# tensorlink-lab/tensorlink

Hardware: NVIDIA H100
Metric: generate tokens/sec (higher is better)
Workload: dtype bf16

## Files before the change

### include/tensorlink_b200.h

```cpp
#ifndef TENSORLINK_B200_H
#define TENSORLINK_B200_H

#include <stddef.h>
#include <stdint.h>

#ifdef __cplusplus
extern "C" {
#endif

#define TL_ABI_VERSION 1

typedef enum {
    TL_OK = 0,
    TL_ERR_INVALID = -1,
    TL_ERR_CUDA = -2,
    TL_ERR_NO_DEVICE = -3,
    TL_ERR_WORKSPACE = -4
} tl_status;

#define TL_EPI_BIAS 1
#define TL_EPI_RESIDUAL 2
#define TL_EPI_SWIGLU 4
#define TL_EPI_OUT_F32 8
#define TL_EPI_ACCUM 16
#define TL_A_MN_MAJOR 32
#define TL_B_MN_MAJOR 64

int tl_abi_version(void);
const char* tl_last_error(void);
int tl_device_info(int* sm_count, int* cc_major, int* cc_minor);

int tl_rmsnorm_fwd(const void* x, const void* w, void* y, float* rstd_out, int rows, int H, float eps, void* stream);

int tl_embed_fwd(const int64_t* ids, const void* table, void* out, int n_tokens, int H, int vocab, void* stream);

int tl_gemm_bf16(const void* A, const void* B, void* C, int M, int N, int K, int lda, int ldb, int ldc,
                 const void* bias, const void* residual, int flags, void* stream);

size_t tl_gemm_splitk_ws(int M, int N);
int tl_gemm_bf16_ws(const void* A, const void* B, void* C, int M, int N, int K, int lda, int ldb, int ldc,
                    const void* bias, const void* residual, int flags, void* workspace, size_t ws_bytes, void* stream);
int tl_gemm_bf16_ws_norm(const void* A, const void* B, void* C, int M, int N, int K, int lda, int ldb, int ldc,
                         const void* bias, const void* residual, int flags, void* workspace, size_t ws_bytes,
                         const void* norm_w, float eps, void* H_out, void* stream);

int tl_gemv_bf16(const void* x, const void* W, void* y, int M, int N, int K, const void* bias,
                 const void* residual, const void* norm_w, float eps, int flags, void* stream);
int tl_gemv_bf16_pf(const void* x, const void* W, void* y, int M, int N, int K, const void* bias,
                    const void* residual, const void* norm_w, float eps, int flags, const void* next_W,
                    size_t next_bytes, void* stream);

int tl_rope_table(const float* inv_freq, void* cos_tab, void* sin_tab, int max_pos, int half_dim, void* stream);

int tl_rope_kv_fwd(const void* qkv, void* q_out, void* k_cache, void* v_cache, const int32_t* pos0_dev,
                   const void* cos_tab, const void* sin_tab, const void* q_norm_w, const void* k_norm_w,
                   float eps, int n_tokens, int S, int n_h, int n_kv, int d, int T_max, void* stream);

int tl_attn_prefill_fwd(const void* q, const void* k_cache, const void* v_cache, void* out, float* lse, int B,
                        int S, int past_len, int n_h, int n_kv, int d, int T_max, float scale, void* stream);

size_t tl_attn_decode_ws(int B, int n_h, int d, int T_max);
int tl_attn_decode_fwd(const void* q, const void* k_cache, const void* v_cache, void* out,
                       const int32_t* kv_len_dev, void* workspace, size_t ws_bytes, int B, int n_h, int n_kv,
                       int d, int T_max, float scale, void* stream);

int tl_attn_decode_fused(const void* qkv, void* k_cache, void* v_cache, void* out, const int32_t* pos_dev,
                         const void* cos_tab, const void* sin_tab, const void* q_norm_w, const void* k_norm_w,
                         float eps, int B, int n_h, int n_kv, int d, int T_max, float scale, void* stream);

int tl_rope_kv_fwd_rows(const void* qkv, void* q_out, void* k_cache, void* v_cache, const int32_t* pos0_dev,
                        const void* cos_tab, const void* sin_tab, const void* q_norm_w, const void* k_norm_w,
                        float eps, int n_tokens, int S, int n_h, int n_kv, int d, int T_max,
                        const int32_t* kv_start_dev, void* stream);
int tl_attn_prefill_fwd_rows(const void* q, const void* k_cache, const void* v_cache, void* out, float* lse, int B,
                             int S, int past_len, int n_h, int n_kv, int d, int T_max, float scale,
                             const int32_t* kv_start_dev, void* stream);
int tl_attn_decode_fwd_rows(const void* q, const void* k_cache, const void* v_cache, void* out,
                            const int32_t* kv_len_dev, void* workspace, size_t ws_bytes, int B, int n_h, int n_kv,
                            int d, int T_max, float scale, const int32_t* kv_start_dev, void* stream);
int tl_attn_decode_fused_rows(const void* qkv, void* k_cache, void* v_cache, void* out, const int32_t* pos_dev,
                              const void* cos_tab, const void* sin_tab, const void* q_norm_w, const void* k_norm_w,
                              float eps, int B, int n_h, int n_kv, int d, int T_max, float scale,
                              const int32_t* kv_start_dev, void* stream);
int tl_attn_bwd_rows(const void* q, const void* k_cache, const void* v_cache, const void* out, const void* dout,
                     const float* lse, void* dq, void* dk, void* dv, void* workspace, size_t ws_bytes, int B, int S,
                     int n_h, int n_kv, int d, int T_max, float scale, const int32_t* kv_start_dev, void* stream);

size_t tl_lmhead_ws(int M, int V);
int tl_lmhead_argmax(const void* x, const void* W, const void* norm_w, float eps, int64_t* ids_out,
                     void* logits_out, void* workspace, size_t ws_bytes, int M, int V, int H, void* stream);

int tl_argmax_bf16(const void* logits, int64_t* ids_out, void* workspace, size_t ws_bytes, int M, int V, void* stream);

size_t tl_sample_ws(int M);
int tl_sample(const void* logits, int64_t* ids_out, int M, int V, float temperature, int top_k, float top_p,
              unsigned long long seed, int32_t* counters_dev, void* workspace, size_t ws_bytes, void* stream);

#define TL_LP_PENALTY 0
#define TL_LP_NGRAM 1
#define TL_LP_MIN_NEW 2
#define TL_LP_PROMPT 3
#define TL_LP_N_EOS 4
#define TL_LP_EOS 5
#define TL_LP_MAX_EOS 8
#define TL_LP_PARAMS (TL_LP_EOS + TL_LP_MAX_EOS)
#define TL_LP_BAN 1
size_t tl_logits_proc_ws(int M, int V);
int tl_history_fill(const int64_t* prompt, int32_t* log, int32_t* len, uint32_t* bits, int M, int S, int L, int V,
                    void* stream);
int tl_argmax_proc(const void* logits, int64_t* ids_out, int32_t* log, int32_t* len, uint32_t* bits,
                   const int32_t* params_dev, int flags, void* workspace, size_t ws_bytes, int M, int V, int L, void* stream);
int tl_sample_proc(const void* logits, int64_t* ids_out, int32_t* log, int32_t* len, uint32_t* bits,
                   const int32_t* params_dev, int flags, int M, int V, int L, float temperature, int top_k, float top_p,
                   unsigned long long seed, int32_t* counters_dev, void* workspace, size_t ws_bytes, void* stream);

int tl_advance_pos(int32_t* pos_dev, int32_t* kv_len_dev, int delta, void* stream);
int tl_append_token(const int64_t* ids, int64_t* out_tokens, int32_t* step_dev, int B, int ld, void* stream);

#define TL_JOB_GEMV 0
#define TL_JOB_ATTN 1
#define TL_ATTN_POS_PER_ROW 1
#define TL_DECODE_CHAIN_MAX_JOBS 16
#define TL_DECODE_CHAIN_SYNC_BYTES 1024
typedef struct tl_decode_job {
    int32_t type, N, K, flags;
    int32_t n_h, n_kv, d, T_max;
    float eps, scale;
    const void* W;
    const void* x;
    void* y;
    const void* bias;
    const void* residual;
    const void* norm_w;
    const void* pos_dev;
    const void* cos_tab;
    const void* sin_tab;
    const void* q_norm_w;
    const void* k_norm_w;
    void* k_cache;
    void* v_cache;
} tl_decode_job;
size_t tl_decode_chain_ws(int M, int n_h, int n_kv, int d);
int tl_decode_chain(const tl_decode_job* jobs, int n_jobs, int M, void* sync_slot, void* attn_ws, size_t attn_ws_bytes,
                    const void* pf_ptr, size_t pf_bytes, void* stream);
int tl_decode_chain_trace(void* buf, int n_slots);

int tl_peer_alloc(size_t bytes, void** ptr, unsigned char* handle64);
int tl_peer_open(const unsigned char* handle64, void** ptr);
int tl_peer_close(void* ptr);
int tl_peer_free(void* ptr);
int tl_peer_wait(const uint32_t* flag_local, uint32_t* want_dev, uint32_t* err_dev, uint64_t* wait_ns_dev,
                 uint64_t timeout_ns, int32_t* bump_dev, void* stream);
int tl_peer_signal(uint32_t* flag_peer, uint32_t* sent_dev, int32_t* bump_dev, void* stream);
int tl_peer_put(void* dst_peer, const void* src, size_t bytes, uint32_t* flag_peer, uint32_t* sent_dev, void* stream);

int tl_swiglu_fwd(const void* gu, void* h, int M, int I, void* stream);
int tl_swiglu_bwd(const void* gu, const void* dh, void* dgu, int M, int I, void* stream);
int tl_rmsnorm_bwd(const void* x, const void* w, const void* dy, const float* rstd, const void* dx_add, void* dx,
                   float* dw_accum, int rows, int H, void* stream);
int tl_rope_kv_bwd(const void* dq, const void* dk, const void* dv, void* dqkv, const void* cos_tab,
                   const void* sin_tab, int n_tokens, int S, int n_h, int n_kv, int d, int T_max, void* stream);
int tl_qk_norm_bwd(const void* qkv_pre, void* dqkv, const void* q_norm_w, const void* k_norm_w, float* dqn_accum,
                   float* dkn_accum, float eps, int n_tokens, int n_h, int n_kv, int d, void* stream);
size_t tl_attn_bwd_ws(int B, int S, int n_h);
int tl_attn_bwd(const void* q, const void* k_cache, const void* v_cache, const void* out, const void* dout,
                const float* lse, void* dq, void* dk, void* dv, void* workspace, size_t ws_bytes, int B, int S,
                int n_h, int n_kv, int d, int T_max, float scale, void* stream);
int tl_ce_fwd_bwd(const void* logits, const int64_t* labels, float* loss_sum, int32_t* n_valid, void* dlogits,
                  float grad_scale, int M, int V, void* stream);
int tl_embed_bwd(const int64_t* ids, const void* dout, void* dtable, int n_tokens, int H, int vocab, void* stream);
int tl_colsum(const void* dy, float* db_accum, int M, int N, int ld, void* stream);
int tl_f32_to_bf16_accum(const float* src, void* dst, size_t n, int accumulate, void* stream);
int tl_add_inplace(void* a, const void* b, size_t n, void* stream);
int tl_scale_add_bf16(void* a, const void* b, float scale, int accumulate, size_t n, void* stream);
int tl_scale_add_f32(float* a, const float* b, float scale, int accumulate, size_t n, void* stream);
int tl_adamw_step(void* param, const void* grad, float* exp_avg, float* exp_avg_sq, size_t n, float lr,
                  float beta1, float beta2, float eps, float weight_decay, int step, int decoupled,
                  void* stream);

#ifdef __cplusplus
}
#endif
#endif
```

### tensorlink_b200/csrc/attention.cu

```cuda
#include <stdlib.h>

#include "common.cuh"

namespace tl {

constexpr int FA_BQ = 64, FA_BKV = 64, FA_THREADS = 128;

__device__ __forceinline__ void cp_async16(void* smem_dst, const void* gsrc, bool valid) {
    const uint32_t d = smem_u32(smem_dst);
    const int sz = valid ? 16 : 0;
    asm volatile("cp.async.cg.shared.global [%0], [%1], 16, %2;" ::"r"(d), "l"(gsrc), "r"(sz) : "memory");
}
__device__ __forceinline__ void cp_async_commit() { asm volatile("cp.async.commit_group;" ::: "memory"); }
template <int N>
__device__ __forceinline__ void cp_async_wait() { asm volatile("cp.async.wait_group %0;" ::"n"(N) : "memory"); }

__device__ __forceinline__ void ldmatrix_x4(uint32_t* r, const void* p) {
    asm volatile("ldmatrix.sync.aligned.m8n8.x4.shared.b16 {%0,%1,%2,%3}, [%4];"
                 : "=r"(r[0]), "=r"(r[1]), "=r"(r[2]), "=r"(r[3]) : "r"(smem_u32(p)));
}
__device__ __forceinline__ void ldmatrix_x4_trans(uint32_t* r, const void* p) {
    asm volatile("ldmatrix.sync.aligned.m8n8.x4.trans.shared.b16 {%0,%1,%2,%3}, [%4];"
                 : "=r"(r[0]), "=r"(r[1]), "=r"(r[2]), "=r"(r[3]) : "r"(smem_u32(p)));
}
__device__ __forceinline__ void mma_bf16_16816(float* c, const uint32_t* a, uint32_t b0, uint32_t b1) {
    asm volatile(
        "mma.sync.aligned.m16n8k16.row.col.f32.bf16.bf16.f32 {%0,%1,%2,%3}, {%4,%5,%6,%7}, {%8,%9}, {%0,%1,%2,%3};"
        : "+f"(c[0]), "+f"(c[1]), "+f"(c[2]), "+f"(c[3])
        : "r"(a[0]), "r"(a[1]), "r"(a[2]), "r"(a[3]), "r"(b0), "r"(b1));
}

template <int D, bool ROWS>
__global__ void __launch_bounds__(FA_THREADS) attn_prefill_kernel(const bf16* __restrict__ q,
                                                                   const bf16* __restrict__ k_cache,
                                                                   const bf16* __restrict__ v_cache,
                                                                   bf16* __restrict__ out, float* __restrict__ lse,
                                                                   int S, int past_len, int n_h, int n_kv, int T_max,
                                                                   float scale_log2, const int32_t* __restrict__ kv_start) {
    constexpr int LDS = D + 8;
    extern __shared__ __align__(16) unsigned char smem_raw[];
    bf16* sQ = reinterpret_cast<bf16*>(smem_raw);
    bf16* sK = sQ + FA_BQ * LDS;
    bf16* sV = sK + 2 * FA_BKV * LDS;

    const int tid = threadIdx.x, warp = tid >> 5, lane = tid & 31;
    const int g = lane >> 2, t4 = lane & 3;
    const int qt = gridDim.x - 1 - blockIdx.x;
    const int h = blockIdx.y, b = blockIdx.z;
    const int kvh = h / (n_h / n_kv);
    const int q0 = qt * FA_BQ;
    const int T = past_len + S;
    const bf16* qg = q + ((size_t)b * S) * n_h * D + (size_t)h * D;
    const bf16* kg = k_cache + ((size_t)b * n_kv + kvh) * T_max * D;
    const bf16* vg = v_cache + ((size_t)b * n_kv + kvh) * T_max * D;
    constexpr int CPR = D / 8;
    int k_start = 0, t0 = 0;
    if constexpr (ROWS) {
        k_start = kv_start[b];
        if (min(T, past_len + q0 + FA_BQ) <= k_start) {
#pragma unroll
            for (int r = 0; r < 2; ++r) {
                const int row = q0 + warp * 16 + g + r * 8;
                if (row >= S) continue;
                bf16* dst = out + ((size_t)b * S + row) * n_h * D + (size_t)h * D;
#pragma unroll
                for (int i = 0; i < D / 8; ++i) *reinterpret_cast<uint32_t*>(dst + i * 8 + 2 * t4) = 0u;
                if (lse && t4 == 0) lse[((size_t)b * n_h + h) * S + row] = -INFINITY;
            }
            return;
        }
        t0 = k_start / FA_BKV;
    }

    for (int c = tid; c < FA_BQ * CPR; c += FA_THREADS) {
        const int r = c / CPR, cc = c - r * CPR;
        const bool ok = (q0 + r) < S;
        cp_async16(sQ + r * LDS + cc * 8, qg + (size_t)(ok ? q0 + r : 0) * n_h * D + cc * 8, ok);
    }
    auto load_kv = [&](int buf, int kv0) {
        for (int c = tid; c < FA_BKV * CPR; c += FA_THREADS) {
            const int r = c / CPR, cc = c - r * CPR;
            const bool ok = (kv0 + r) < T && (!ROWS || (kv0 + r) >= k_start);
            const size_t off = (size_t)(ok ? kv0 + r : 0) * D + cc * 8;
            cp_async16(sK + (buf * FA_BKV + r) * LDS + cc * 8, kg + off, ok);
            cp_async16(sV + (buf * FA_BKV + r) * LDS + cc * 8, vg + off, ok);
        }
    };
    const int kv_end = min(T, past_len + q0 + FA_BQ);
    const int n_tiles = (kv_end + FA_BKV - 1) / FA_BKV;
    load_kv(t0 & 1, t0 * FA_BKV);
    cp_async_commit();

    float o[D / 8][4];
#pragma unroll
    for (int i = 0; i < D / 8; ++i) o[i][0] = o[i][1] = o[i][2] = o[i][3] = 0.f;
    float m_run[2] = {-INFINITY, -INFINITY}, l_run[2] = {0.f, 0.f};
    uint32_t qf[D / 16][4];
    const int qrow_abs0 = past_len + q0 + warp * 16 + g;

    for (int it = t0; it < n_tiles; ++it) {
        const int buf = it & 1;
        if (it + 1 < n_tiles) load_kv(buf ^ 1, (it + 1) * FA_BKV);
        cp_async_commit();
        cp_async_wait<1>();
        __syncthreads();
        if (it == t0) {
#pragma unroll
            for (int ks = 0; ks < D / 16; ++ks)
                ldmatrix_x4(qf[ks], sQ + (warp * 16 + (lane & 15)) * LDS + ks * 16 + (lane >> 4) * 8);
        }
        const bf16* sKb = sK + buf * FA_BKV * LDS;
        const bf16* sVb = sV + buf * FA_BKV * LDS;
        float s[FA_BKV / 8][4];
#pragma unroll
        for (int i = 0; i < FA_BKV / 8; ++i) s[i][0] = s[i][1] = s[i][2] = s[i][3] = 0.f;
#pragma unroll
        for (int ks = 0; ks < D / 16; ++ks) {
#pragma unroll
            for (int np = 0; np < FA_BKV / 16; ++np) {
                uint32_t bfr[4];
                const int mi = lane >> 3;
                ldmatrix_x4(bfr, sKb + (np * 16 + (mi >> 1) * 8 + (lane & 7)) * LDS + ks * 16 + (mi & 1) * 8);
                mma_bf16_16816(s[2 * np], qf[ks], bfr[0], bfr[1]);
                mma_bf16_16816(s[2 * np + 1], qf[ks], bfr[2], bfr[3]);
            }
        }
        const int kv0 = it * FA_BKV;
        float mx[2] = {-INFINITY, -INFINITY};
#pragma unroll
        for (int i = 0; i < FA_BKV / 8; ++i) {
#pragma unroll
            for (int e = 0; e < 4; ++e) {
                const int key = kv0 + i * 8 + 2 * t4 + (e & 1);
                const int qpos = qrow_abs0 + ((e >> 1) ? 8 : 0);
                float v = s[i][e] * scale_log2;
                if (key > qpos || key >= T) v = -INFINITY;
                if constexpr (ROWS) if (key < k_start) v = -INFINITY;
                s[i][e] = v;
                mx[e >> 1] = fmaxf(mx[e >> 1], v);
            }
        }
        float alpha[2], msub[2];
#pragma unroll
        for (int r = 0; r < 2; ++r) {
            mx[r] = fmaxf(mx[r], __shfl_xor_sync(0xffffffffu, mx[r], 1));
            mx[r] = fmaxf(mx[r], __shfl_xor_sync(0xffffffffu, mx[r], 2));
            const float m_new = fmaxf(m_run[r], mx[r]);
            msub[r] = (m_new == -INFINITY) ? 0.f : m_new;
            alpha[r] = exp2f(m_run[r] - msub[r]);
            m_run[r] = m_new;
        }
        float rs[2] = {0.f, 0.f};
        uint32_t pf[FA_BKV / 16][4];
#pragma unroll
        for (int i = 0; i < FA_BKV / 8; ++i) {
            const float p0 = exp2f(s[i][0] - msub[0]), p1 = exp2f(s[i][1] - msub[0]);
            const float p2 = exp2f(s[i][2] - msub[1]), p3 = exp2f(s[i][3] - msub[1]);
            rs[0] += p0 + p1;
            rs[1] += p2 + p3;
            pf[i >> 1][(i & 1) * 2] = pack_bf16(p0, p1);
            pf[i >> 1][(i & 1) * 2 + 1] = pack_bf16(p2, p3);
        }
#pragma unroll
        for (int r = 0; r < 2; ++r) {
            rs[r] += __shfl_xor_sync(0xffffffffu, rs[r], 1);
            rs[r] += __shfl_xor_sync(0xffffffffu, rs[r], 2);
            l_run[r] = l_run[r] * alpha[r] + rs[r];
        }
#pragma unroll
        for (int i = 0; i < D / 8; ++i) {
            o[i][0] *= alpha[0];
            o[i][1] *= alpha[0];
            o[i][2] *= alpha[1];
            o[i][3] *= alpha[1];
        }
#pragma unroll
        for (int kk = 0; kk < FA_BKV / 16; ++kk) {
#pragma unroll
            for (int dp = 0; dp < D / 16; ++dp) {
                uint32_t bfr[4];
                const int mi = lane >> 3;
                ldmatrix_x4_trans(bfr, sVb + (kk * 16 + (mi & 1) * 8 + (lane & 7)) * LDS + dp * 16 + (mi >> 1) * 8);
                mma_bf16_16816(o[2 * dp], pf[kk], bfr[0], bfr[1]);
                mma_bf16_16816(o[2 * dp + 1], pf[kk], bfr[2], bfr[3]);
            }
        }
        __syncthreads();
    }
#pragma unroll
    for (int r = 0; r < 2; ++r) {
        const int row = q0 + warp * 16 + g + r * 8;
        if (row >= S) continue;
        const float inv = l_run[r] > 0.f ? 1.0f / l_run[r] : 0.f;
        bf16* dst = out + ((size_t)b * S + row) * n_h * D + (size_t)h * D;
#pragma unroll
        for (int i = 0; i < D / 8; ++i)
            *reinterpret_cast<uint32_t*>(dst + i * 8 + 2 * t4) = pack_bf16(o[i][2 * r] * inv, o[i][2 * r + 1] * inv);
        if (lse && t4 == 0)
            lse[((size_t)b * n_h + h) * S + row] = m_run[r] * 0.6931471805599453f + logf(l_run[r]);
    }
}

constexpr int DEC_CHUNK = 128, DEC_THREADS = 128, DEC_MAX_REP = 8;
constexpr int DEC_CHUNK_MMA = 256;

__host__ __device__ inline size_t dec_rec_floats(int n_rep, int D) { return (size_t)n_rep * (2 + D); }

template <int D, bool ROWS>
__global__ void __launch_bounds__(DEC_THREADS) attn_decode_split_kernel(const bf16* __restrict__ q,
                                                                        const bf16* __restrict__ k_cache,
                                                                        const bf16* __restrict__ v_cache,
                                                                        float* __restrict__ ws,
                                                                        const int32_t* __restrict__ kv_len_dev,
                                                                        int n_h, int n_kv, int T_max, int n_splits,
                                                                        float scale_log2, const int32_t* __restrict__ kv_start) {
    const int split = blockIdx.x, kvh = blockIdx.y, b = blockIdx.z;
    const int kv_len = *kv_len_dev;
    const int c0 = split * DEC_CHUNK;
    if (c0 >= kv_len) return;
    int k_start = 0;
    if constexpr (ROWS) {
        k_start = kv_start[b];
        if (c0 + DEC_CHUNK <= k_start) return;
    }
    const int n_rep = n_h / n_kv;
    const int tid = threadIdx.x, lane = tid & 31, warp = tid >> 5;
    __shared__ __align__(16) float sq[DEC_MAX_REP][D];
    __shared__ float sp[DEC_MAX_REP][DEC_CHUNK];
    __shared__ float sred[DEC_THREADS / 32][DEC_MAX_REP];
    __shared__ float sm[DEC_MAX_REP];
    __shared__ __align__(16) float so[DEC_THREADS / 32][DEC_MAX_REP][D];

    for (int i = tid; i < n_rep * D; i += DEC_THREADS) {
        const int r = i / D, dd = i - r * D;
        sq[r][dd] = bf2f(q[((size_t)b * n_h + kvh * n_rep + r) * D + dd]);
    }
    __syncthreads();
    const int key = c0 + tid;
    const bool valid = key < kv_len && (!ROWS || key >= k_start);
    float sc[DEC_MAX_REP];
#pragma unroll
    for (int r = 0; r < DEC_MAX_REP; ++r) sc[r] = 0.f;
    if (valid) {
        const uint4* kr = reinterpret_cast<const uint4*>(k_cache + (((size_t)b * n_kv + kvh) * T_max + key) * D);
#pragma unroll 4
        for (int c = 0; c < D / 8; ++c) {
            const uint4 kv4 = kr[c];
            const uint32_t* k32 = reinterpret_cast<const uint32_t*>(&kv4);
            float kf[8];
#pragma unroll
            for (int j = 0; j < 4; ++j) {
                kf[2 * j] = bf16_lo(k32[j]);
                kf[2 * j + 1] = bf16_hi(k32[j]);
            }
#pragma unroll
            for (int r = 0; r < DEC_MAX_REP; ++r) {
                if (r < n_rep) {
                    const float4 qa = *reinterpret_cast<const float4*>(&sq[r][c * 8]);
                    const float4 qb = *reinterpret_cast<const float4*>(&sq[r][c * 8 + 4]);
                    sc[r] += kf[0] * qa.x + kf[1] * qa.y + kf[2] * qa.z + kf[3] * qa.w + kf[4] * qb.x + kf[5] * qb.y +
                             kf[6] * qb.z + kf[7] * qb.w;
                }
            }
        }
    }
#pragma unroll
    for (int r = 0; r < DEC_MAX_REP; ++r) {
        sc[r] = valid ? sc[r] * scale_log2 : -INFINITY;
        const float mw = warp_max(sc[r]);
        if (lane == 0) sred[warp][r] = mw;
    }
    __syncthreads();
    if (tid < DEC_MAX_REP) {
        float m = sred[0][tid];
#pragma unroll
        for (int w = 1; w < DEC_THREADS / 32; ++w) m = fmaxf(m, sred[w][tid]);
        sm[tid] = m;
    }
    __syncthreads();
    float lsum[DEC_MAX_REP];
#pragma unroll
    for (int r = 0; r < DEC_MAX_REP; ++r) {
        const float p = (valid && r < n_rep) ? exp2f(sc[r] - sm[r]) : 0.f;
        sp[r][tid] = rbf(p);
        lsum[r] = warp_sum(p);
    }
    __syncthreads();
#pragma unroll
    for (int r = 0; r < DEC_MAX_REP; ++r)
        if (lane == 0) sred[warp][r] = lsum[r];
    constexpr int TPR = D / 8;
    constexpr int KG = DEC_THREADS / TPR;
    const int dd0 = (tid % TPR) * 8, kgi = tid / TPR;
    float acc[DEC_MAX_REP][8];
#pragma unroll
    for (int r = 0; r < DEC_MAX_REP; ++r)
#pragma unroll
        for (int j = 0; j < 8; ++j) acc[r][j] = 0.f;
    const int nk = min(DEC_CHUNK, kv_len - c0);
    const int k_lo = ROWS ? max(k_start - c0, 0) : 0;
    for (int kk = k_lo + kgi; kk < nk; kk += KG) {
        const uint4 vv = *reinterpret_cast<const uint4*>(v_cache + (((size_t)b * n_kv + kvh) * T_max + c0 + kk) * D + dd0);
        const uint32_t* v32 = reinterpret_cast<const uint32_t*>(&vv);
        float vf[8];
#pragma unroll
        for (int j = 0; j < 4; ++j) {
            vf[2 * j] = bf16_lo(v32[j]);
            vf[2 * j + 1] = bf16_hi(v32[j]);
        }
#pragma unroll
        for (int r = 0; r < DEC_MAX_REP; ++r) {
            if (r < n_rep) {
                const float p = sp[r][kk];
#pragma unroll
                for (int j = 0; j < 8; ++j) acc[r][j] = fmaf(p, vf[j], acc[r][j]);
            }
        }
    }
#pragma unroll
    for (int r = 0; r < DEC_MAX_REP; ++r)
#pragma unroll
        for (int j = 0; j < 8; ++j) {
            float v = acc[r][j];
#pragma unroll
            for (int off = TPR; off < 32; off <<= 1) v += __shfl_xor_sync(0xffffffffu, v, off);
            acc[r][j] = v;
        }
    if (lane < TPR) {
#pragma unroll
        for (int r = 0; r < DEC_MAX_REP; ++r)
            if (r < n_rep) {
#pragma unroll
                for (int j = 0; j < 8; ++j) so[warp][r][dd0 + j] = acc[r][j];
            }
    }
    __syncthreads();
    float* rec = ws + (((size_t)b * n_kv + kvh) * n_splits + split) * dec_rec_floats(n_rep, D);
    for (int i = tid; i < n_rep * D; i += DEC_THREADS) {
        const int r = i / D, dd = i - r * D;
        float v = 0.f;
#pragma unroll
        for (int w = 0; w < DEC_THREADS / 32; ++w) v += so[w][r][dd];
        rec[2 * n_rep + i] = v;
    }
    if (tid < n_rep) {
        float l = 0.f;
#pragma unroll
        for (int w = 0; w < DEC_THREADS / 32; ++w) l += sred[w][tid];
        rec[tid] = sm[tid];
        rec[n_rep + tid] = l;
    }
}

template <int D, bool ROWS>
__global__ void __launch_bounds__(FA_THREADS) attn_decode_mma_kernel(const bf16* __restrict__ q, const bf16* __restrict__ k_cache,
                                                                      const bf16* __restrict__ v_cache, float* __restrict__ ws,
                                                                      const int32_t* __restrict__ kv_len_dev, int n_h, int n_kv,
                                                                      int T_max, int n_splits, float scale_log2,
                                                                      const int32_t* __restrict__ kv_start) {
    constexpr int LDS = D + 8;
    constexpr int CPR = D / 8;
    constexpr int NT = 2;
    const int split = blockIdx.x, kvh = blockIdx.y, b = blockIdx.z;
    const int kv_len = *kv_len_dev;
    const int c0 = split * DEC_CHUNK_MMA;
    if (c0 >= kv_len) return;
    int k_start = 0, t0 = 0;
    if constexpr (ROWS) {
        k_start = kv_start[b];
        if (c0 + DEC_CHUNK_MMA <= k_start) return;
        t0 = max(k_start - c0, 0) / FA_BKV;
    }
    const int n_rep = n_h / n_kv;
    extern __shared__ __align__(16) unsigned char smem_raw[];
    bf16* sQ = reinterpret_cast<bf16*>(smem_raw);
    bf16* sK = sQ + 16 * LDS;
    bf16* sV = sK + NT * FA_BKV * LDS;
    const int tid = threadIdx.x, warp = tid >> 5, lane = tid & 31;
    const int g = lane >> 2, t4 = lane & 3;
    const bf16* kg = k_cache + ((size_t)b * n_kv + kvh) * T_max * D;
    const bf16* vg = v_cache + ((size_t)b * n_kv + kvh) * T_max * D;
    const bf16* qg = q + ((size_t)b * n_h + kvh * n_rep) * D;
    for (int c = tid; c < 16 * CPR; c += FA_THREADS) {
        const int r = c / CPR, cc = c - r * CPR;
        cp_async16(sQ + r * LDS + cc * 8, qg + (size_t)(r < n_rep ? r : 0) * D + cc * 8, r < n_rep);
    }
    const int n_tiles = min(DEC_CHUNK_MMA / FA_BKV, (kv_len - c0 + FA_BKV - 1) / FA_BKV);
    auto load_tile = [&](int t) {
        const int kv0 = c0 + t * FA_BKV, buf = t & 1;
        for (int c = tid; c < FA_BKV * CPR; c += FA_THREADS) {
            const int r = c / CPR, cc = c - r * CPR;
            const bool ok = (kv0 + r) < kv_len && (!ROWS || (kv0 + r) >= k_start);
            const size_t off = (size_t)(ok ? kv0 + r : 0) * D + cc * 8;
            cp_async16(sK + (buf * FA_BKV + r) * LDS + cc * 8, kg + off, ok);
            cp_async16(sV + (buf * FA_BKV + r) * LDS + cc * 8, vg + off, ok);
        }
        cp_async_commit();
    };
    load_tile(t0);
    if (t0 + 1 < n_tiles) load_tile(t0 + 1);
    float o[D / 8][4];
#pragma unroll
    for (int i = 0; i < D / 8; ++i) o[i][0] = o[i][1] = o[i][2] = o[i][3] = 0.f;
    float m_run[2] = {-INFINITY, -INFINITY}, l_run[2] = {0.f, 0.f};
    uint32_t qf[D / 16][4];
    for (int t = t0; t < n_tiles; ++t) {
        if (t + 1 < n_tiles) cp_async_wait<1>(); else cp_async_wait<0>();
        __syncthreads();
        if (t == t0) {
#pragma unroll
            for (int ks = 0; ks < D / 16; ++ks)
                ldmatrix_x4(qf[ks], sQ + (lane & 15) * LDS + ks * 16 + (lane >> 4) * 8);
        }
        const bf16* sKb = sK + ((t & 1) * FA_BKV + warp * 16) * LDS;
        const bf16* sVb = sV + ((t & 1) * FA_BKV + warp * 16) * LDS;
        float sc[2][4];
#pragma unroll
        for (int i = 0; i < 2; ++i) sc[i][0] = sc[i][1] = sc[i][2] = sc[i][3] = 0.f;
#pragma unroll
        for (int ks = 0; ks < D / 16; ++ks) {
            uint32_t bfr[4];
            const int mi = lane >> 3;
            ldmatrix_x4(bfr, sKb + ((mi >> 1) * 8 + (lane & 7)) * LDS + ks * 16 + (mi & 1) * 8);
            mma_bf16_16816(sc[0], qf[ks], bfr[0], bfr[1]);
            mma_bf16_16816(sc[1], qf[ks], bfr[2], bfr[3]);
        }
        const int key0 = c0 + t * FA_BKV + warp * 16;
        float mx[2] = {-INFINITY, -INFINITY};
#pragma unroll
        for (int i = 0; i < 2; ++i)
#pragma unroll
            for (int e = 0; e < 4; ++e) {
                const int key = key0 + i * 8 + 2 * t4 + (e & 1);
                const float v = (key < kv_len && (!ROWS || key >= k_start)) ? sc[i][e] * scale_log2 : -INFINITY;
                sc[i][e] = v;
                mx[e >> 1] = fmaxf(mx[e >> 1], v);
            }
        float alpha[2], msub[2];
#pragma unroll
        for (int r = 0; r < 2; ++r) {
            mx[r] = fmaxf(mx[r], __shfl_xor_sync(0xffffffffu, mx[r], 1));
            mx[r] = fmaxf(mx[r], __shfl_xor_sync(0xffffffffu, mx[r], 2));
            const float m_new = fmaxf(m_run[r], mx[r]);
            msub[r] = (m_new == -INFINITY) ? 0.f : m_new;
            alpha[r] = exp2f(m_run[r] - msub[r]);
            m_run[r] = m_new;
        }
        float rs[2] = {0.f, 0.f};
        uint32_t pf[4];
#pragma unroll
        for (int i = 0; i < 2; ++i) {
            const float p0 = exp2f(sc[i][0] - msub[0]), p1 = exp2f(sc[i][1] - msub[0]);
            const float p2 = exp2f(sc[i][2] - msub[1]), p3 = exp2f(sc[i][3] - msub[1]);
            rs[0] += p0 + p1;
            rs[1] += p2 + p3;
            pf[i * 2] = pack_bf16(p0, p1);
            pf[i * 2 + 1] = pack_bf16(p2, p3);
        }
#pragma unroll
        for (int r = 0; r < 2; ++r) {
            rs[r] += __shfl_xor_sync(0xffffffffu, rs[r], 1);
            rs[r] += __shfl_xor_sync(0xffffffffu, rs[r], 2);
            l_run[r] = l_run[r] * alpha[r] + rs[r];
        }
#pragma unroll
        for (int i = 0; i < D / 8; ++i) {
            o[i][0] *= alpha[0];
            o[i][1] *= alpha[0];
            o[i][2] *= alpha[1];
            o[i][3] *= alpha[1];
        }
#pragma unroll
        for (int dp = 0; dp < D / 16; ++dp) {
            uint32_t bfr[4];
            const int mi = lane >> 3;
            ldmatrix_x4_trans(bfr, sVb + ((mi & 1) * 8 + (lane & 7)) * LDS + dp * 16 + (mi >> 1) * 8);
            mma_bf16_16816(o[2 * dp], pf, bfr[0], bfr[1]);
            mma_bf16_16816(o[2 * dp + 1], pf, bfr[2], bfr[3]);
        }
        if (t + 2 < n_tiles) {
            __syncthreads();
            load_tile(t + 2);
        }
    }
    __syncthreads();
    float* sM = reinterpret_cast<float*>(sK);
    float* sL = sM + 64;
    float* sO = sL + 64;
#pragma unroll
    for (int r = 0; r < 2; ++r) {
        const int row = g + r * 8;
        if (t4 == 0) { sM[warp * 16 + row] = m_run[r]; sL[warp * 16 + row] = l_run[r]; }
#pragma unroll
        for (int i = 0; i < D / 8; ++i) {
            sO[(warp * 16 + row) * D + i * 8 + 2 * t4] = o[i][2 * r];
            sO[(warp * 16 + row) * D + i * 8 + 2 * t4 + 1] = o[i][2 * r + 1];
        }
    }
    __syncthreads();
    float* rec = ws + (((size_t)b * n_kv + kvh) * n_splits + split) * dec_rec_floats(n_rep, D);
    for (int i = tid; i < n_rep * D; i += FA_THREADS) {
        const int r = i / D, dd = i - r * D;
        const float m = fmaxf(fmaxf(sM[r], sM[16 + r]), fmaxf(sM[32 + r], sM[48 + r]));
        float v = 0.f;
#pragma unroll
        for (int w = 0; w < 4; ++w) {
            const float mw = sM[w * 16 + r];
            if (mw != -INFINITY) v += sO[(w * 16 + r) * D + dd] * exp2f(mw - m);
        }
        rec[2 * n_rep + i] = v;
    }
    if (tid < n_rep) {
        const int r = tid;
        const float m = fmaxf(fmaxf(sM[r], sM[16 + r]), fmaxf(sM[32 + r], sM[48 + r]));
        float l = 0.f;
#pragma unroll
        for (int w = 0; w < 4; ++w) {
            const float mw = sM[w * 16 + r];
            if (mw != -INFINITY) l += sL[w * 16 + r] * exp2f(mw - m);
        }
        rec[r] = m;
        rec[n_rep + r] = l;
    }
}

template <int D, bool ROWS>
__global__ void attn_decode_reduce_kernel(const float* __restrict__ ws, bf16* __restrict__ out,
                                          const int32_t* __restrict__ kv_len_dev, int n_h, int n_kv, int n_splits, int chunk,
                                          const int32_t* __restrict__ kv_start) {
    const int h = blockIdx.x, b = blockIdx.y, dd = threadIdx.x;
    const int n_rep = n_h / n_kv, kvh = h / n_rep, r = h - kvh * n_rep;
    const int kv_len = *kv_len_dev;
    const int ns = min(n_splits, (kv_len + chunk - 1) / chunk);
    const int s0 = ROWS ? kv_start[b] / chunk : 0;
    const float* base = ws + ((size_t)b * n_kv + kvh) * n_splits * dec_rec_floats(n_rep, D);
    float M = -INFINITY;
    for (int s = s0; s < ns; ++s) M = fmaxf(M, base[s * dec_rec_floats(n_rep, D) + r]);
    float L = 0.f, O = 0.f;
    for (int s = s0; s < ns; ++s) {
        const float* rec = base + s * dec_rec_floats(n_rep, D);
        const float w = exp2f(rec[r] - M);
        L += rec[n_rep + r] * w;
        O += rec[2 * n_rep + r * D + dd] * w;
    }
    out[((size_t)b * n_h + h) * D + dd] = f2bf(L > 0.f ? O / L : 0.f);
}

}

namespace tl {
int attn_prefill_wgmma(const void* q, const void* k_cache, const void* v_cache, void* out, float* lse, int B, int S, int past_len,
                       int n_h, int n_kv, int d, int T_max, float scale, const int32_t* kv_start, cudaStream_t st);

static int attn_prefill_launch(const void* q, const void* k_cache, const void* v_cache, void* out, float* lse, int B, int S,
                               int past_len, int n_h, int n_kv, int d, int T_max, float scale, const int32_t* kv_start,
                               cudaStream_t st, const char* what) {
    TL_REQUIRE(d == 64 || d == 128, TL_ERR_INVALID, "%s: head_dim %d not in {64,128}", what, d);
    TL_REQUIRE(n_kv > 0 && n_h % n_kv == 0, TL_ERR_INVALID, "%s: n_h %% n_kv != 0", what);
    TL_REQUIRE(past_len >= 0 && past_len + S <= T_max, TL_ERR_INVALID,
               "%s: past_len %d + S %d exceeds cache T_max %d", what, past_len, S, T_max);
    if (B == 0 || S == 0) return TL_OK;
    {
        const char* e = getenv("TL_ATTN_IMPL");
        const int impl = !e ? 0 : (e[0] == 'm' ? 1 : (e[0] == 'w' ? 2 : 0));
        if (impl == 2 || (impl == 0 && S >= FA_BQ))
            return attn_prefill_wgmma(q, k_cache, v_cache, out, lse, B, S, past_len, n_h, n_kv, d, T_max, scale, kv_start, st);
    }
    const dim3 grid((S + FA_BQ - 1) / FA_BQ, n_h, B);
    const float sl2 = scale * 1.4426950408889634f;
    const size_t smem = (size_t)(FA_BQ + 4 * FA_BKV) * (d + 8) * sizeof(bf16);
#define TL_FA_FWD(D_, ROWS_)                                                                                                \
    do {                                                                                                                    \
        static bool done = false;                                                                                           \
        if (!done) { cudaFuncSetAttribute(attn_prefill_kernel<D_, ROWS_>, cudaFuncAttributeMaxDynamicSharedMemorySize, (int)smem); done = true; } \
        attn_prefill_kernel<D_, ROWS_><<<grid, FA_THREADS, smem, st>>>((const bf16*)q, (const bf16*)k_cache, (const bf16*)v_cache, \
                                                                        (bf16*)out, lse, S, past_len, n_h, n_kv, T_max, sl2, kv_start); \
    } while (0)
    if (kv_start) {
        if (d == 64) TL_FA_FWD(64, true); else TL_FA_FWD(128, true);
    } else {
        if (d == 64) TL_FA_FWD(64, false); else TL_FA_FWD(128, false);
    }
#undef TL_FA_FWD
    return check_launch(what);
}

static int attn_decode_launch(const void* q, const void* k_cache, const void* v_cache, void* out, const int32_t* kv_len_dev,
                              void* workspace, size_t ws_bytes, int B, int n_h, int n_kv, int d, int T_max, float scale,
                              const int32_t* kv_start, cudaStream_t st, const char* what);
}

extern "C" {

int tl_attn_prefill_fwd(const void* q, const void* k_cache, const void* v_cache, void* out, float* lse, int B, int S,
                        int past_len, int n_h, int n_kv, int d, int T_max, float scale, void* stream) {
    return tl::attn_prefill_launch(q, k_cache, v_cache, out, lse, B, S, past_len, n_h, n_kv, d, T_max, scale, nullptr,
                                   (cudaStream_t)stream, "tl_attn_prefill_fwd");
}

int tl_attn_prefill_fwd_rows(const void* q, const void* k_cache, const void* v_cache, void* out, float* lse, int B, int S,
                             int past_len, int n_h, int n_kv, int d, int T_max, float scale, const int32_t* kv_start_dev,
                             void* stream) {
    using namespace tl;
    TL_REQUIRE(kv_start_dev != nullptr, TL_ERR_INVALID, "tl_attn_prefill_fwd_rows: kv_start_dev is null");
    return attn_prefill_launch(q, k_cache, v_cache, out, lse, B, S, past_len, n_h, n_kv, d, T_max, scale, kv_start_dev,
                               (cudaStream_t)stream, "tl_attn_prefill_fwd_rows");
}

size_t tl_attn_decode_ws(int B, int n_h, int d, int T_max) {
    const size_t n_splits = (size_t)(T_max + tl::DEC_CHUNK - 1) / tl::DEC_CHUNK;
    return (size_t)B * n_splits * (size_t)n_h * (2 + d) * sizeof(float);
}

int tl_attn_decode_fwd(const void* q, const void* k_cache, const void* v_cache, void* out, const int32_t* kv_len_dev,
                       void* workspace, size_t ws_bytes, int B, int n_h, int n_kv, int d, int T_max, float scale,
                       void* stream) {
    return tl::attn_decode_launch(q, k_cache, v_cache, out, kv_len_dev, workspace, ws_bytes, B, n_h, n_kv, d, T_max, scale,
                                  nullptr, (cudaStream_t)stream, "tl_attn_decode_fwd");
}

int tl_attn_decode_fwd_rows(const void* q, const void* k_cache, const void* v_cache, void* out, const int32_t* kv_len_dev,
                            void* workspace, size_t ws_bytes, int B, int n_h, int n_kv, int d, int T_max, float scale,
                            const int32_t* kv_start_dev, void* stream) {
    using namespace tl;
    TL_REQUIRE(kv_start_dev != nullptr, TL_ERR_INVALID, "tl_attn_decode_fwd_rows: kv_start_dev is null");
    return attn_decode_launch(q, k_cache, v_cache, out, kv_len_dev, workspace, ws_bytes, B, n_h, n_kv, d, T_max, scale,
                              kv_start_dev, (cudaStream_t)stream, "tl_attn_decode_fwd_rows");
}

}

namespace tl {
static int attn_decode_launch(const void* q, const void* k_cache, const void* v_cache, void* out, const int32_t* kv_len_dev,
                              void* workspace, size_t ws_bytes, int B, int n_h, int n_kv, int d, int T_max, float scale,
                              const int32_t* kv_start, cudaStream_t st, const char* what) {
    TL_REQUIRE(d == 64 || d == 128, TL_ERR_INVALID, "%s: head_dim %d not in {64,128}", what, d);
    TL_REQUIRE(n_kv > 0 && n_h % n_kv == 0 && n_h / n_kv <= DEC_MAX_REP, TL_ERR_INVALID,
               "%s: GQA group %d/%d unsupported (max %d)", what, n_h, n_kv, DEC_MAX_REP);
    TL_REQUIRE(kv_len_dev != nullptr, TL_ERR_INVALID, "%s: kv_len_dev is null", what);
    TL_REQUIRE(ws_bytes >= tl_attn_decode_ws(B, n_h, d, T_max), TL_ERR_WORKSPACE,
               "%s: workspace %zu < %zu", what, ws_bytes, tl_attn_decode_ws(B, n_h, d, T_max));
    if (B == 0) return TL_OK;
    const int n_splits = (T_max + DEC_CHUNK - 1) / DEC_CHUNK;
    const float sl2 = scale * 1.4426950408889634f;
    const dim3 g1(n_splits, n_kv, B), g2(n_h, B);
    const char* impl = getenv("TL_DECODE_ATTN");
    if (!(impl && impl[0] == 's')) {
        const int ns_m = (T_max + DEC_CHUNK_MMA - 1) / DEC_CHUNK_MMA;
        const dim3 gm(ns_m, n_kv, B);
        const size_t smem = (size_t)(16 + 4 * FA_BKV) * (d + 8) * sizeof(bf16);
#define TL_DEC_MMA(D_, ROWS_)                                                                                               \
        do {                                                                                                                \
            static bool done = false;                                                                                       \
            if (!done) { cudaFuncSetAttribute(attn_decode_mma_kernel<D_, ROWS_>, cudaFuncAttributeMaxDynamicSharedMemorySize, (int)smem); done = true; } \
            attn_decode_mma_kernel<D_, ROWS_><<<gm, FA_THREADS, smem, st>>>((const bf16*)q, (const bf16*)k_cache, (const bf16*)v_cache, \
                                                                             (float*)workspace, kv_len_dev, n_h, n_kv, T_max, ns_m, sl2, kv_start); \
            attn_decode_reduce_kernel<D_, ROWS_><<<g2, D_, 0, st>>>((const float*)workspace, (bf16*)out, kv_len_dev, n_h, n_kv, ns_m, \
                                                                     DEC_CHUNK_MMA, kv_start);                             \
        } while (0)
        if (kv_start) {
            if (d == 64) TL_DEC_MMA(64, true); else TL_DEC_MMA(128, true);
        } else {
            if (d == 64) TL_DEC_MMA(64, false); else TL_DEC_MMA(128, false);
        }
#undef TL_DEC_MMA
        return check_launch(what);
    }
#define TL_DEC_SIMT(D_, ROWS_)                                                                                              \
    do {                                                                                                                    \
        attn_decode_split_kernel<D_, ROWS_><<<g1, DEC_THREADS, 0, st>>>((const bf16*)q, (const bf16*)k_cache, (const bf16*)v_cache, \
                                                                         (float*)workspace, kv_len_dev, n_h, n_kv, T_max, n_splits, sl2, kv_start); \
        attn_decode_reduce_kernel<D_, ROWS_><<<g2, D_, 0, st>>>((const float*)workspace, (bf16*)out, kv_len_dev, n_h, n_kv, n_splits, \
                                                                 DEC_CHUNK, kv_start);                                     \
    } while (0)
    if (kv_start) {
        if (d == 64) TL_DEC_SIMT(64, true); else TL_DEC_SIMT(128, true);
    } else {
        if (d == 64) TL_DEC_SIMT(64, false); else TL_DEC_SIMT(128, false);
    }
#undef TL_DEC_SIMT
    return check_launch(what);
}
}

namespace tl {

constexpr int FD_THREADS = 128, FD_MAX_T = 2048;

template <int D, bool ROWS>
__global__ void __launch_bounds__(FD_THREADS) attn_decode_fused_kernel(
    const bf16* __restrict__ qkv, bf16* __restrict__ k_cache, bf16* __restrict__ v_cache, bf16* __restrict__ out,
    const int32_t* __restrict__ pos_dev, const bf16* __restrict__ cos_tab, const bf16* __restrict__ sin_tab,
    const bf16* __restrict__ q_norm_w, const bf16* __restrict__ k_norm_w, float eps, int n_h, int n_kv, int T_max,
    float scale_log2, const int32_t* __restrict__ kv_start) {
    constexpr int HALF = D / 2;
    asm volatile("griddepcontrol.wait;" ::: "memory");
    asm volatile("griddepcontrol.launch_dependents;");
    const int h = blockIdx.x, b = blockIdx.y, tid = threadIdx.x, lane = tid & 31, warp = tid >> 5;
    const int n_rep = n_h / n_kv, kvh = h / n_rep;
    const int pos = *pos_dev;
    int k_start = 0;
    if constexpr (ROWS) {
        k_start = kv_start[b];
        cos_tab -= (size_t)k_start * HALF;
        sin_tab -= (size_t)k_start * HALF;
    }
    const int heads = n_h + 2 * n_kv;
    __shared__ __align__(16) float sq[D], sk[D], sv[D];
    __shared__ float sscore[FD_MAX_T + 1];
    __shared__ float sred[FD_THREADS / 32];
    __shared__ float s_bc[2];
    __shared__ __align__(16) float so[FD_THREADS / 32][D];

    const bf16* row = qkv + (size_t)b * heads * D;
    float q1 = 0.f, q2 = 0.f, k1 = 0.f, k2 = 0.f;
    if (tid < HALF) {
        q1 = bf2f(row[(size_t)h * D + tid]);
        q2 = bf2f(row[(size_t)h * D + tid + HALF]);
        k1 = bf2f(row[(size_t)(n_h + kvh) * D + tid]);
        k2 = bf2f(row[(size_t)(n_h + kvh) * D + tid + HALF]);
        sv[tid] = bf2f(row[(size_t)(n_h + n_kv + kvh) * D + tid]);
        sv[tid + HALF] = bf2f(row[(size_t)(n_h + n_kv + kvh) * D + tid + HALF]);
    }
    if (q_norm_w) {
        float a = warp_sum(q1 * q1 + q2 * q2), c = warp_sum(k1 * k1 + k2 * k2);
        __shared__ float nr[2][FD_THREADS / 32];
        if (lane == 0) { nr[0][warp] = a; nr[1][warp] = c; }
        __syncthreads();
        a = c = 0.f;
#pragma unroll
        for (int w = 0; w < FD_THREADS / 32; ++w) { a += nr[0][w]; c += nr[1][w]; }
        const float rq = 1.0f / sqrtf(a / (float)D + eps), rk = 1.0f / sqrtf(c / (float)D + eps);
        if (tid < HALF) {
            q1 = rbf(bf2f(q_norm_w[tid]) * rbf(q1 * rq));
            q2 = rbf(bf2f(q_norm_w[tid + HALF]) * rbf(q2 * rq));
            k1 = rbf(bf2f(k_norm_w[tid]) * rbf(k1 * rk));
            k2 = rbf(bf2f(k_norm_w[tid + HALF]) * rbf(k2 * rk));
        }
    }
    if (tid < HALF) {
        const float c = bf2f(cos_tab[(size_t)pos * HALF + tid]), s = bf2f(sin_tab[(size_t)pos * HALF + tid]);
        sq[tid] = rbf(rbf(q1 * c) + rbf(-q2 * s));
        sq[tid + HALF] = rbf(rbf(q2 * c) + rbf(q1 * s));
        sk[tid] = rbf(rbf(k1 * c) + rbf(-k2 * s));
        sk[tid + HALF] = rbf(rbf(k2 * c) + rbf(k1 * s));
    }
    __syncthreads();
    if (h % n_rep == 0 && tid < D) {
        const size_t off = (((size_t)b * n_kv + kvh) * T_max + pos) * D + tid;
        k_cache[off] = f2bf(sk[tid]);
        v_cache[off] = f2bf(sv[tid]);
    }
    const bf16* kb = k_cache + ((size_t)b * n_kv + kvh) * T_max * D;
    const bf16* vb = v_cache + ((size_t)b * n_kv + kvh) * T_max * D;
    float mx = -INFINITY;
    for (int key = tid; key < pos; key += FD_THREADS) {
        if constexpr (ROWS) if (key < k_start) continue;
        const uint4* kr = reinterpret_cast<const uint4*>(kb + (size_t)key * D);
        float acc = 0.f;
#pragma unroll 4
        for (int c = 0; c < D / 8; ++c) {
            const uint4 kv4 = kr[c];
            const uint32_t* k32 = reinterpret_cast<const uint32_t*>(&kv4);
            const float4 qa = *reinterpret_cast<const float4*>(&sq[c * 8]);
            const float4 qb = *reinterpret_cast<const float4*>(&sq[c * 8 + 4]);
            acc += bf16_lo(k32[0]) * qa.x + bf16_hi(k32[0]) * qa.y + bf16_lo(k32[1]) * qa.z + bf16_hi(k32[1]) * qa.w +
                   bf16_lo(k32[2]) * qb.x + bf16_hi(k32[2]) * qb.y + bf16_lo(k32[3]) * qb.z + bf16_hi(k32[3]) * qb.w;
        }
        acc *= scale_log2;
        sscore[key] = acc;
        mx = fmaxf(mx, acc);
    }
    if (warp == 0) {
        float acc = 0.f;
        for (int i = lane; i < D; i += 32) acc += sq[i] * sk[i];
        acc = warp_sum(acc) * scale_log2;
        if (lane == 0) sscore[pos] = acc;
        mx = fmaxf(mx, acc);
    }
    mx = warp_max(mx);
    if (lane == 0) sred[warp] = mx;
    __syncthreads();
    if (tid == 0) {
        float m = sred[0];
#pragma unroll
        for (int w = 1; w < FD_THREADS / 32; ++w) m = fmaxf(m, sred[w]);
        s_bc[0] = m;
    }
    __syncthreads();
    const float m_all = s_bc[0];
    float lsum = 0.f;
    for (int key = tid; key <= pos; key += FD_THREADS) {
        if constexpr (ROWS) if (key < k_start) continue;
        const float p = exp2f(sscore[key] - m_all);
        lsum += p;
        sscore[key] = rbf(p);
    }
    lsum = warp_sum(lsum);
    __syncthreads();
    if (lane == 0) sred[warp] = lsum;
    __syncthreads();
    constexpr int TPR = D / 8, KG = FD_THREADS / TPR;
    const int dd0 = (tid % TPR) * 8, kgi = tid / TPR;
    float acc[8];
#pragma unroll
    for (int j = 0; j < 8; ++j) acc[j] = 0.f;
    for (int key = kgi; key < pos; key += KG) {
        if constexpr (ROWS) if (key < k_start) continue;
        const uint4 vv = *reinterpret_cast<const uint4*>(vb + (size_t)key * D + dd0);
        const uint32_t* v32 = reinterpret_cast<const uint32_t*>(&vv);
        const float p = sscore[key];
#pragma unroll
        for (int j = 0; j < 4; ++j) {
            acc[2 * j] = fmaf(p, bf16_lo(v32[j]), acc[2 * j]);
            acc[2 * j + 1] = fmaf(p, bf16_hi(v32[j]), acc[2 * j + 1]);
        }
    }
    if (kgi == 0) {
        const float p = sscore[pos];
#pragma unroll
        for (int j = 0; j < 8; ++j) acc[j] = fmaf(p, sv[dd0 + j], acc[j]);
    }
#pragma unroll
    for (int j = 0; j < 8; ++j) {
        float v = acc[j];
#pragma unroll
        for (int off = TPR; off < 32; off <<= 1) v += __shfl_xor_sync(0xffffffffu, v, off);
        acc[j] = v;
    }
    if (lane < TPR) {
#pragma unroll
        for (int j = 0; j < 8; ++j) so[warp][dd0 + j] = acc[j];
    }
    __syncthreads();
    if (tid < D) {
        float l = 0.f, o = 0.f;
#pragma unroll
        for (int w = 0; w < FD_THREADS / 32; ++w) { l += sred[w]; o += so[w][tid]; }
        out[((size_t)b * n_h + h) * D + tid] = f2bf(o / l);
    }
}

}

namespace tl {
static int attn_decode_fused_cfg(cudaLaunchConfig_t* cfg, cudaLaunchAttribute* attr, int d, int n_h, int n_kv, int T_max,
                                 const int32_t* pos_dev, int B, void* stream, const char* what) {
    TL_REQUIRE(d == 64 || d == 128, TL_ERR_INVALID, "%s: head_dim %d not in {64,128}", what, d);
    TL_REQUIRE(n_kv > 0 && n_h % n_kv == 0, TL_ERR_INVALID, "%s: n_h %% n_kv != 0", what);
    TL_REQUIRE(T_max <= FD_MAX_T, TL_ERR_INVALID, "%s: T_max %d > %d (use the split-KV path)", what, T_max, FD_MAX_T);
    TL_REQUIRE(pos_dev != nullptr, TL_ERR_INVALID, "%s: pos_dev is null", what);
    *cfg = {};
    cfg->gridDim = dim3(n_h, B);
    cfg->blockDim = dim3(FD_THREADS);
    cfg->dynamicSmemBytes = 0;
    cfg->stream = (cudaStream_t)stream;
    attr[0].id = cudaLaunchAttributeProgrammaticStreamSerialization;
    attr[0].val.programmaticStreamSerializationAllowed = 1;
    static int use_pdl = -1;
    if (use_pdl < 0) {
        const char* e = getenv("TL_PDL");
        const char* e2 = getenv("TL_PDL_ATTN");
        use_pdl = (!(e && e[0] == '0') && (e2 && e2[0] == '1')) ? 1 : 0;
    }
    cfg->attrs = attr;
    cfg->numAttrs = use_pdl ? 1 : 0;
    return TL_OK;
}
}

extern "C" int tl_attn_decode_fused(const void* qkv, void* k_cache, void* v_cache, void* out, const int32_t* pos_dev,
                                    const void* cos_tab, const void* sin_tab, const void* q_norm_w, const void* k_norm_w,
                                    float eps, int B, int n_h, int n_kv, int d, int T_max, float scale, void* stream) {
    using namespace tl;
    cudaLaunchConfig_t cfg;
    cudaLaunchAttribute attr[1];
    const int rc = attn_decode_fused_cfg(&cfg, attr, d, n_h, n_kv, T_max, pos_dev, B, stream, "tl_attn_decode_fused");
    if (rc != TL_OK || B == 0) return rc;
    const float sl2 = scale * 1.4426950408889634f;
    if (d == 64)
        cudaLaunchKernelEx(&cfg, attn_decode_fused_kernel<64, false>, (const bf16*)qkv, (bf16*)k_cache, (bf16*)v_cache, (bf16*)out,
                           pos_dev, (const bf16*)cos_tab, (const bf16*)sin_tab, (const bf16*)q_norm_w, (const bf16*)k_norm_w, eps,
                           n_h, n_kv, T_max, sl2, (const int32_t*)nullptr);
    else
        cudaLaunchKernelEx(&cfg, attn_decode_fused_kernel<128, false>, (const bf16*)qkv, (bf16*)k_cache, (bf16*)v_cache, (bf16*)out,
                           pos_dev, (const bf16*)cos_tab, (const bf16*)sin_tab, (const bf16*)q_norm_w, (const bf16*)k_norm_w, eps,
                           n_h, n_kv, T_max, sl2, (const int32_t*)nullptr);
    return check_launch("tl_attn_decode_fused");
}

extern "C" int tl_attn_decode_fused_rows(const void* qkv, void* k_cache, void* v_cache, void* out, const int32_t* pos_dev,
                                         const void* cos_tab, const void* sin_tab, const void* q_norm_w, const void* k_norm_w,
                                         float eps, int B, int n_h, int n_kv, int d, int T_max, float scale,
                                         const int32_t* kv_start_dev, void* stream) {
    using namespace tl;
    TL_REQUIRE(kv_start_dev != nullptr, TL_ERR_INVALID, "tl_attn_decode_fused_rows: kv_start_dev is null");
    cudaLaunchConfig_t cfg;
    cudaLaunchAttribute attr[1];
    const int rc = attn_decode_fused_cfg(&cfg, attr, d, n_h, n_kv, T_max, pos_dev, B, stream, "tl_attn_decode_fused_rows");
    if (rc != TL_OK || B == 0) return rc;
    const float sl2 = scale * 1.4426950408889634f;
    if (d == 64)
        cudaLaunchKernelEx(&cfg, attn_decode_fused_kernel<64, true>, (const bf16*)qkv, (bf16*)k_cache, (bf16*)v_cache, (bf16*)out,
                           pos_dev, (const bf16*)cos_tab, (const bf16*)sin_tab, (const bf16*)q_norm_w, (const bf16*)k_norm_w, eps,
                           n_h, n_kv, T_max, sl2, kv_start_dev);
    else
        cudaLaunchKernelEx(&cfg, attn_decode_fused_kernel<128, true>, (const bf16*)qkv, (bf16*)k_cache, (bf16*)v_cache, (bf16*)out,
                           pos_dev, (const bf16*)cos_tab, (const bf16*)sin_tab, (const bf16*)q_norm_w, (const bf16*)k_norm_w, eps,
                           n_h, n_kv, T_max, sl2, kv_start_dev);
    return check_launch("tl_attn_decode_fused_rows");
}
```

### tensorlink_b200/csrc/decode_chain.cu

```cuda
#include <stdlib.h>

#include "common.cuh"

namespace tl {

constexpr int DC_CW = 8;
constexpr int DC_CT = DC_CW * 32;
constexpr int DC_THREADS = DC_CT + 32;
constexpr int DC_MAX_STAGES = 24;
constexpr int DC_MAX_JOBS = 16;
constexpr int DC_MAX_M = 4;
constexpr int DC_TILE = 32;
constexpr int DC_MIN_KEYS = 128;
constexpr int DC_KT_MAX = 128 * 2 + 16;
constexpr int DC_ATTN_BYTES = 8 * 128 * 4 + 2 * 128 * 4 + 8 * DC_TILE * 4 + 2 * DC_TILE * DC_KT_MAX;
constexpr int DC_GB = 8;
constexpr int DC_JOBCTR = 64;
constexpr int DC_STAT_OFF = 2 * (DC_MAX_JOBS + 1) * 4 + DC_MAX_JOBS * 160;
constexpr unsigned long long DC_TIMEOUT_NS = 2000000000ull;

struct ChainParams {
    int n_jobs, n_stages, NW, xs_bytes;
    int dynamic, stage_bytes;
    int kc, l2_ahead;
    unsigned* sync;
    float* attn_part;
    const unsigned char* pf_ptr;
    unsigned long long pf_bytes;
    unsigned long long* trace;
    tl_decode_job jobs[DC_MAX_JOBS];
};

__device__ __forceinline__ void dc_bar(int id, int n) { asm volatile("bar.sync %0, %1;" ::"r"(id), "r"(n) : "memory"); }
__device__ __forceinline__ unsigned dc_ld_acquire(const unsigned* p) {
    unsigned v;
    asm volatile("ld.acquire.gpu.global.u32 %0, [%1];" : "=r"(v) : "l"(p) : "memory");
    return v;
}
__device__ __forceinline__ void dc_red_release(unsigned* p, unsigned v) {
    asm volatile("red.release.gpu.global.add.u32 [%0], %1;" ::"l"(p), "r"(v) : "memory");
}
__device__ __forceinline__ unsigned long long dc_timer() {
    unsigned long long t;
    asm volatile("mov.u64 %0, %%globaltimer;" : "=l"(t));
    return t;
}
__device__ __forceinline__ uint4 dc_ldcg_v4(const void* p) {
    uint4 r;
    asm volatile("ld.global.cg.v4.u32 {%0,%1,%2,%3}, [%4];" : "=r"(r.x), "=r"(r.y), "=r"(r.z), "=r"(r.w) : "l"(p));
    return r;
}
__device__ __forceinline__ float dc_ldcg_bf16(const bf16* p) {
    unsigned short v;
    asm volatile("ld.global.cg.u16 %0, [%1];" : "=h"(v) : "l"(p));
    return __uint_as_float(((uint32_t)v) << 16);
}
__device__ __forceinline__ bool dc_mbar_wait(uint64_t* bar, uint32_t parity, volatile int* dead) {
    int it = 0;
    while (!mbar_try_wait(bar, parity)) {
        if (((++it) & 0xfff) == 0 && *dead) return false;
    }
    return true;
}

struct DcGeom {
    int npairs, P, U, u_begin, u_end, KC, n_chunks;
    bool chunked;
};
__device__ __forceinline__ DcGeom dc_geom(int N, int K, int DC_STAGE, int DC_KC) {
    DcGeom g;
    g.npairs = N >> 1;
    g.chunked = K > DC_KC || (size_t)K * 4 > (size_t)DC_STAGE;
    g.P = g.chunked ? 1 : min(8, (int)(DC_STAGE / ((size_t)K * 4)));
    g.U = (g.npairs + g.P - 1) / g.P;
    g.u_begin = (int)((long long)blockIdx.x * g.U / gridDim.x);
    g.u_end = (int)((long long)(blockIdx.x + 1) * g.U / gridDim.x);
    g.KC = g.chunked ? DC_KC : K;
    g.n_chunks = (K + g.KC - 1) / g.KC;
    return g;
}

template <int M>
__global__ void __launch_bounds__(DC_THREADS, 1) decode_chain_kernel(const __grid_constant__ ChainParams p) {
    extern __shared__ __align__(128) unsigned char smem[];
    const int n_stages = p.n_stages, NW = p.NW, DC_STAGE = p.stage_bytes, DC_KC = p.kc;
    unsigned char* ring = smem;
    bf16* xs = reinterpret_cast<bf16*>(smem + (size_t)n_stages * DC_STAGE);
    unsigned char* attn_s = smem + (size_t)n_stages * DC_STAGE + (size_t)p.xs_bytes;
    uint64_t* full_bar = reinterpret_cast<uint64_t*>(attn_s + DC_ATTN_BYTES);
    uint64_t* empty_bar = full_bar + DC_MAX_STAGES;
    __shared__ float s_part[DC_CW][M];
    __shared__ int s_dead, s_last;
    __shared__ int s_gbase[DC_GB];

    const int tid = threadIdx.x, lane = tid & 31, warp = tid >> 5;
    if (tid == 0) {
        for (int s = 0; s < n_stages; ++s) {
            mbar_init(&full_bar[s], 1);
            mbar_init(&empty_bar[s], 1);
        }
        s_dead = 0;
        s_last = 0;
        fence_barrier_init();
    }
    __syncthreads();
    asm volatile("griddepcontrol.launch_dependents;");

    if (warp == DC_CW) {
        if (lane == 0) {
            int stage = 0, gseq = 0;
            uint32_t phase = 0;
            bool alive = true;
            unsigned* const tickets = p.sync + DC_JOBCTR;
            long long loaded = 0, prefetched = 0;
            int pf_job = 0;
            long long pf_off = 0;
            auto pf_range = [&](int j, const unsigned char*& base, long long& len) {
                const tl_decode_job& q = p.jobs[j];
                const DcGeom h = dc_geom(q.N, q.K, DC_STAGE, DC_KC);
                const long long r0 = (long long)h.u_begin * h.P * 2, r1 = min((long long)h.u_end * h.P * 2, (long long)q.N);
                base = reinterpret_cast<const unsigned char*>(q.W) + r0 * q.K * 2;
                len = (r1 - r0) * q.K * 2;
            };
            auto pump = [&](int max_issue) {
                if (p.dynamic || p.l2_ahead <= 0) return;
                while (max_issue-- > 0 && pf_job < p.n_jobs && prefetched < loaded + p.l2_ahead) {
                    if (p.jobs[pf_job].type != TL_JOB_GEMV) { ++pf_job; pf_off = 0; continue; }
                    const unsigned char* base;
                    long long len;
                    pf_range(pf_job, base, len);
                    if (pf_off >= len) { ++pf_job; pf_off = 0; continue; }
                    const uint32_t sz = (uint32_t)min(16384ll, len - pf_off);
                    asm volatile("cp.async.bulk.prefetch.L2.global [%0], %1;" ::"l"(base + pf_off), "r"(sz & ~15u) : "memory");
                    pf_off += sz;
                    prefetched += sz;
                }
            };
            int first_ticket = 0;
            int jn = 0;
            while (jn < p.n_jobs && p.jobs[jn].type != TL_JOB_GEMV) ++jn;
            if (p.dynamic && jn < p.n_jobs) first_ticket = (int)atomicAdd(&tickets[jn], (unsigned)NW);
            for (int j = jn; j < p.n_jobs && alive; j = jn) {
                const tl_decode_job& jb = p.jobs[j];
                jn = j + 1;
                while (jn < p.n_jobs && p.jobs[jn].type != TL_JOB_GEMV) ++jn;
                const DcGeom g = dc_geom(jb.N, jb.K, DC_STAGE, DC_KC);
                const bf16* W = reinterpret_cast<const bf16*>(jb.W);
                const int K = jb.K;
                int base = p.dynamic ? first_ticket : g.u_begin;
                const int u_end = p.dynamic ? g.U : g.u_end;
                long long pwait = 0;
                if (p.dynamic && jn < p.n_jobs) first_ticket = (int)atomicAdd(&tickets[jn], (unsigned)NW);
                for (;;) {
                    const bool term = base >= u_end;
                    int next = base + NW;
                    if (p.dynamic && !term) next = (int)atomicAdd(&tickets[j], (unsigned)NW);
                    const int n_c = term ? 1 : g.n_chunks;
                    for (int c = 0; c < n_c && alive; ++c)
                        for (int w = 0; w < NW; ++w) {
                            const int unit = base + w;
                            const long long tw0 = clock64();
                            pump(2);
                            {
                                int it = 0;
                                while (!mbar_try_wait(&empty_bar[stage], phase ^ 1)) {
                                    pump(1);
                                    if (((++it) & 0xfff) == 0 && s_dead) { alive = false; break; }
                                }
                                if (!alive) break;
                            }
                            pwait += clock64() - tw0;
                            if (c == 0 && w == 0) s_gbase[gseq & (DC_GB - 1)] = term ? -1 : base;
                            unsigned char* dst = ring + (size_t)stage * DC_STAGE;
                            if (term || unit >= u_end) {
                                mbar_expect_tx(&full_bar[stage], 0);
                            } else {
                                const int pair0 = unit * g.P;
                                const int np = min(g.P, g.npairs - pair0);
                                if (!g.chunked) {
                                    const uint32_t bytes = (uint32_t)(2 * np) * (uint32_t)K * 2u;
                                    mbar_expect_tx(&full_bar[stage], bytes);
                                    bulk_load_1d(dst, W + (size_t)(2 * pair0) * K, bytes, &full_bar[stage]);
                                    loaded += bytes;
                                } else {
                                    const int k0 = c * g.KC;
                                    const uint32_t bytes = (uint32_t)min(g.KC, K - k0) * 2u;
                                    mbar_expect_tx(&full_bar[stage], 2 * bytes);
                                    bulk_load_1d(dst, W + (size_t)(2 * pair0) * K + k0, bytes, &full_bar[stage]);
                                    bulk_load_1d(dst + (size_t)g.KC * 2, W + (size_t)(2 * pair0 + 1) * K + k0, bytes, &full_bar[stage]);
                                    loaded += 2 * bytes;
                                }
                            }
                            if (++stage == n_stages) { stage = 0; phase ^= 1; }
                        }
                    ++gseq;
                    if (term || !alive) break;
                    base = next;
                }
                if (p.trace && blockIdx.x == 0) p.trace[DC_STAT_OFF + (size_t)j * 4 + 2] = (unsigned long long)pwait;
            }
            if (alive && p.pf_bytes) {
                const unsigned long long per = ((p.pf_bytes / gridDim.x) + 4095ull) & ~4095ull;
                unsigned long long off = (unsigned long long)blockIdx.x * per;
                const unsigned long long end = off + per < p.pf_bytes ? off + per : p.pf_bytes;
                for (; off < end; off += 16384ull) {
                    const uint32_t sz = (uint32_t)(end - off < 16384ull ? end - off : 16384ull);
                    asm volatile("cp.async.bulk.prefetch.L2.global [%0], %1;" ::"l"(p.pf_ptr + off), "r"(sz) : "memory");
                }
            }
        }
        return;
    }

    unsigned* const bar_ctr = p.sync;
    unsigned* const err_word = p.sync + 2;
    unsigned* const grp_ctr = p.sync + 4;
    unsigned bar_target = 0;
    auto grid_dep = [&](bool arrive, unsigned n_arrivals) -> bool {
        dc_bar(1, DC_CT);
        if (tid == 0) {
            if (arrive) dc_red_release(bar_ctr, 1u);
            bar_target += n_arrivals;
            unsigned long long t0 = 0;
            int it = 0;
            while ((int)(dc_ld_acquire(bar_ctr) - bar_target) < 0) {
                if (((++it) & 0x3ff) == 0) {
                    const unsigned long long now = dc_timer();
                    if (!t0) t0 = now;
                    if (now - t0 > DC_TIMEOUT_NS || dc_ld_acquire(err_word)) {
                        atomicExch(err_word, 1u);
                        s_dead = 1;
                        break;
                    }
                }
            }
        }
        dc_bar(1, DC_CT);
        return s_dead == 0;
    };
    int seq = warp;
    int gseq = 0;
    const int tr_sel = blockIdx.x == 0 ? 0 : (blockIdx.x == gridDim.x - 1 ? 1 : -1);
    auto stamp = [&](int j, int k) {
        if (!p.trace || tid != 0) return;
        const unsigned long long now = dc_timer();
        if (tr_sel >= 0) p.trace[((size_t)tr_sel * (DC_MAX_JOBS + 1) + j) * 4 + k] = now;
        if (k == 2 && j < DC_MAX_JOBS) p.trace[2 * (DC_MAX_JOBS + 1) * 4 + (size_t)j * 160 + blockIdx.x] = now;
    };
    stamp(DC_MAX_JOBS, 0);

    asm volatile("griddepcontrol.wait;" ::: "memory");
    stamp(DC_MAX_JOBS, 1);

    for (int j = 0; j < p.n_jobs; ++j) {
        const tl_decode_job& jb = p.jobs[j];
        const bool last_job = j == p.n_jobs - 1;
        stamp(j, 0);
        if (jb.type == TL_JOB_GEMV) {
            const int N = jb.N, K = jb.K, flags = jb.flags;
            const bf16* x = reinterpret_cast<const bf16*>(jb.x);
            bf16* y = reinterpret_cast<bf16*>(jb.y);
            const bf16* bias = reinterpret_cast<const bf16*>(jb.bias);
            const bf16* residual = reinterpret_cast<const bf16*>(jb.residual);
            const bf16* norm_w = reinterpret_cast<const bf16*>(jb.norm_w);
            const float eps = jb.eps;
            const int nvec = K >> 3;
            if (norm_w) {
                float ss[M];
#pragma unroll
                for (int m = 0; m < M; ++m) ss[m] = 0.f;
                constexpr int TB = M == 1 ? 4 : (M == 2 ? 2 : 1);
                for (int v0 = tid; v0 < nvec; v0 += TB * DC_CT) {
                    uint4 u[M][TB];
#pragma unroll
                    for (int m = 0; m < M; ++m)
#pragma unroll
                        for (int t = 0; t < TB; ++t)
                            if (v0 + t * DC_CT < nvec) u[m][t] = dc_ldcg_v4(x + (size_t)m * K + (size_t)(v0 + t * DC_CT) * 8);
#pragma unroll
                    for (int m = 0; m < M; ++m)
#pragma unroll
                        for (int t = 0; t < TB; ++t) {
                            const int v = v0 + t * DC_CT;
                            if (v < nvec) {
                                reinterpret_cast<uint4*>(xs + (size_t)m * K)[v] = u[m][t];
                                const uint32_t* u32 = reinterpret_cast<const uint32_t*>(&u[m][t]);
#pragma unroll
                                for (int q = 0; q < 4; ++q) {
                                    const float a = bf16_lo(u32[q]), b = bf16_hi(u32[q]);
                                    ss[m] += a * a + b * b;
                                }
                            }
                        }
                }
#pragma unroll
                for (int m = 0; m < M; ++m) {
                    const float t = warp_sum(ss[m]);
                    if (lane == 0) s_part[warp][m] = t;
                }
                dc_bar(1, DC_CT);
                float rstd[M];
#pragma unroll
                for (int m = 0; m < M; ++m) {
                    float t = 0.f;
#pragma unroll
                    for (int w = 0; w < DC_CW; ++w) t += s_part[w][m];
                    rstd[m] = 1.0f / sqrtf(t / (float)K + eps);
                }
                for (int v = tid; v < nvec; v += DC_CT) {
                    const uint4 g = reinterpret_cast<const uint4*>(norm_w)[v];
                    const uint32_t* g32 = reinterpret_cast<const uint32_t*>(&g);
#pragma unroll
                    for (int m = 0; m < M; ++m) {
                        const uint4 u = reinterpret_cast<const uint4*>(xs + (size_t)m * K)[v];
                        uint4 o;
                        const uint32_t* u32 = reinterpret_cast<const uint32_t*>(&u);
                        uint32_t* o32 = reinterpret_cast<uint32_t*>(&o);
#pragma unroll
                        for (int q = 0; q < 4; ++q)
                            o32[q] = pack_bf16(bf16_lo(g32[q]) * rbf(bf16_lo(u32[q]) * rstd[m]),
                                               bf16_hi(g32[q]) * rbf(bf16_hi(u32[q]) * rstd[m]));
                        reinterpret_cast<uint4*>(xs + (size_t)m * K)[v] = o;
                    }
                }
            } else {
                const int tot = nvec * M;
                for (int v0 = tid; v0 < tot; v0 += 4 * DC_CT) {
                    uint4 u[4];
#pragma unroll
                    for (int t = 0; t < 4; ++t)
                        if (v0 + t * DC_CT < tot) u[t] = dc_ldcg_v4(x + (size_t)(v0 + t * DC_CT) * 8);
#pragma unroll
                    for (int t = 0; t < 4; ++t)
                        if (v0 + t * DC_CT < tot) reinterpret_cast<uint4*>(xs)[v0 + t * DC_CT] = u[t];
                }
            }
            dc_bar(1, DC_CT);
            stamp(j, 1);

            const DcGeom g = dc_geom(N, K, DC_STAGE, DC_KC);
            const int u_end = p.dynamic ? g.U : g.u_end;
            const bool swiglu = flags & TL_EPI_SWIGLU;
            const int n_out = swiglu ? g.npairs : N;
            auto preload = [&](int pair, float (&bs)[2], float (&rs)[M][2]) {
                bs[0] = bs[1] = 0.f;
#pragma unroll
                for (int m = 0; m < M; ++m) rs[m][0] = rs[m][1] = 0.f;
                if (lane != 0) return;
                const int r0 = 2 * pair;
                if (flags & TL_EPI_BIAS) {
                    bs[0] = bf2f(bias[r0]);
                    bs[1] = bf2f(bias[r0 + 1]);
                }
                if (flags & TL_EPI_RESIDUAL) {
#pragma unroll
                    for (int m = 0; m < M; ++m) {
                        rs[m][0] = dc_ldcg_bf16(residual + (size_t)m * N + r0);
                        rs[m][1] = dc_ldcg_bf16(residual + (size_t)m * N + r0 + 1);
                    }
                }
            };
            auto finish = [&](int pair, const float (&a0)[M], const float (&a1)[M], const float (&bs)[2], const float (&rs)[M][2]) {
                if (lane != 0) return;
                const int r0 = 2 * pair;
#pragma unroll
                for (int m = 0; m < M; ++m) {
                    float v0 = a0[m], v1 = a1[m];
                    if (flags & TL_EPI_BIAS) {
                        v0 += bs[0];
                        v1 += bs[1];
                    }
                    if (swiglu) {
                        const float gate = rbf(v0), up = rbf(v1);
                        y[(size_t)m * n_out + pair] = f2bf(rbf(silu_f(gate)) * up);
                    } else {
                        float t0 = rbf(v0), t1 = rbf(v1);
                        if (flags & TL_EPI_RESIDUAL) {
                            t0 += rs[m][0];
                            t1 += rs[m][1];
                        }
                        *reinterpret_cast<uint32_t*>(y + (size_t)m * N + r0) = pack_bf16(t0, t1);
                    }
                }
            };
            auto dot2 = [&](const uint4* r0, const uint4* r1, int k0, int vecs, float (&a0)[M], float (&a1)[M]) {
#pragma unroll 4
                for (int v = lane; v < vecs; v += 32) {
                    const uint4 w0 = r0[v], w1 = r1[v];
                    const uint32_t* a32 = reinterpret_cast<const uint32_t*>(&w0);
                    const uint32_t* b32 = reinterpret_cast<const uint32_t*>(&w1);
#pragma unroll
                    for (int m = 0; m < M; ++m) {
                        const uint4 xv = reinterpret_cast<const uint4*>(xs + (size_t)m * K + k0)[v];
                        const uint32_t* x32 = reinterpret_cast<const uint32_t*>(&xv);
#pragma unroll
                        for (int q = 0; q < 4; ++q) {
                            const float xl = bf16_lo(x32[q]), xh = bf16_hi(x32[q]);
                            a0[m] = fmaf(bf16_lo(a32[q]), xl, a0[m]);
                            a0[m] = fmaf(bf16_hi(a32[q]), xh, a0[m]);
                            a1[m] = fmaf(bf16_lo(b32[q]), xl, a1[m]);
                            a1[m] = fmaf(bf16_hi(b32[q]), xh, a1[m]);
                        }
                    }
                }
            };
            long long cwait = 0;
            const long long cjob0 = clock64();
            if (warp < NW) {
                for (;;) {
                    int stage = seq % n_stages;
                    uint32_t phase = (uint32_t)(seq / n_stages) & 1u;
                    long long tw0 = clock64();
                    mbar_wait(&full_bar[stage], phase);
                    cwait += clock64() - tw0;
                    const int base = s_gbase[gseq & (DC_GB - 1)];
                    ++gseq;
                    if (base < 0) {
                        __syncwarp();
                        if (lane == 0) mbar_arrive(&empty_bar[stage]);
                        seq += NW;
                        break;
                    }
                    const int unit = base + warp;
                    const bool valid = unit < u_end;
                    const int pair0 = unit * g.P;
                    float a0[M], a1[M];
                    float bs[2], rs[M][2];
#pragma unroll
                    for (int m = 0; m < M; ++m) a0[m] = a1[m] = 0.f;
                    if (valid) preload(pair0, bs, rs);
                    for (int c = 0; c < g.n_chunks; ++c, seq += NW) {
                        if (c) {
                            stage = seq % n_stages;
                            phase = (uint32_t)(seq / n_stages) & 1u;
                            tw0 = clock64();
                            mbar_wait(&full_bar[stage], phase);
                            cwait += clock64() - tw0;
                        }
                        const unsigned char* src = ring + (size_t)stage * DC_STAGE;
                        if (valid) {
                            if (!g.chunked) {
                                const int np = min(g.P, g.npairs - pair0);
                                for (int pp = 0; pp < np; ++pp) {
                                    float b0[M], b1[M];
                                    float bn[2], rn[M][2];
#pragma unroll
                                    for (int m = 0; m < M; ++m) b0[m] = b1[m] = 0.f;
                                    if (pp + 1 < np) preload(pair0 + pp + 1, bn, rn);
                                    dot2(reinterpret_cast<const uint4*>(src + (size_t)(2 * pp) * K * 2),
                                         reinterpret_cast<const uint4*>(src + (size_t)(2 * pp + 1) * K * 2), 0, nvec, b0, b1);
#pragma unroll
                                    for (int m = 0; m < M; ++m) { b0[m] = warp_sum(b0[m]); b1[m] = warp_sum(b1[m]); }
                                    finish(pair0 + pp, b0, b1, bs, rs);
                                    if (pp + 1 < np) {
                                        bs[0] = bn[0]; bs[1] = bn[1];
#pragma unroll
                                        for (int m = 0; m < M; ++m) { rs[m][0] = rn[m][0]; rs[m][1] = rn[m][1]; }
                                    }
                                }
                            } else {
                                const int k0 = c * g.KC;
                                dot2(reinterpret_cast<const uint4*>(src), reinterpret_cast<const uint4*>(src + (size_t)g.KC * 2), k0,
                                     min(g.KC, K - k0) >> 3, a0, a1);
                            }
                        }
                        __syncwarp();
                        if (lane == 0) mbar_arrive(&empty_bar[stage]);
                    }
                    if (valid && g.chunked) {
#pragma unroll
                        for (int m = 0; m < M; ++m) { a0[m] = warp_sum(a0[m]); a1[m] = warp_sum(a1[m]); }
                        finish(pair0, a0, a1, bs, rs);
                    }
                }
            }
            if (p.trace && blockIdx.x == 0 && tid == 0) {
                p.trace[DC_STAT_OFF + (size_t)j * 4 + 0] = (unsigned long long)cwait;
                p.trace[DC_STAT_OFF + (size_t)j * 4 + 1] = (unsigned long long)(clock64() - cjob0);
            }
            stamp(j, 2);
            if (!last_job && !grid_dep(true, gridDim.x)) break;
            stamp(j, 3);
        } else if (jb.type == TL_JOB_ATTN) {
            const int n_h = jb.n_h, n_kv = jb.n_kv, D = jb.d, T_max = jb.T_max;
            const int HALF = D >> 1, n_rep = n_h / n_kv;
            const int G = n_kv * M;
            const int cpg = (int)gridDim.x / G;
            const int grp = (int)blockIdx.x / cpg, split = (int)blockIdx.x % cpg;
            const bool in_grid = grp < G;
            const int b = in_grid ? grp / n_kv : 0, kvh = in_grid ? grp % n_kv : 0;
            const int pos = reinterpret_cast<const int32_t*>(jb.pos_dev)[(jb.flags & TL_ATTN_POS_PER_ROW) ? b : 0];
            const int n_keys = pos + 1;
            int cpg_eff = min(cpg, (n_keys + DC_MIN_KEYS - 1) / DC_MIN_KEYS);
            const int chunk = (((n_keys + cpg_eff - 1) / cpg_eff) + DC_TILE - 1) / DC_TILE * DC_TILE;
            cpg_eff = (n_keys + chunk - 1) / chunk;
            const bool active = in_grid && split < cpg_eff;
            float* sq = reinterpret_cast<float*>(attn_s);
            float* sk = sq + 8 * 128;
            float* sv = sk + 128;
            float* sp = sv + 128;
            unsigned char* kt = reinterpret_cast<unsigned char*>(sp + 8 * DC_TILE);
            unsigned char* vt = kt + DC_TILE * DC_KT_MAX;
            const int KT = D * 2 + 16;
            if (tid == 0) s_last = 0;
            if (active) {
                const int k0 = split * chunk, k1 = min(n_keys, k0 + chunk);
                const bool owns_pos = k1 == n_keys;
                const int n_tiles = (k1 - k0 + DC_TILE - 1) / DC_TILE;
                const int heads = n_h + 2 * n_kv;
                const bf16* row = reinterpret_cast<const bf16*>(jb.x) + (size_t)b * heads * D;
                const bf16* cos_tab = reinterpret_cast<const bf16*>(jb.cos_tab);
                const bf16* sin_tab = reinterpret_cast<const bf16*>(jb.sin_tab);
                const bf16* qn = reinterpret_cast<const bf16*>(jb.q_norm_w);
                const bf16* kn = reinterpret_cast<const bf16*>(jb.k_norm_w);
                bf16* k_cache = reinterpret_cast<bf16*>(jb.k_cache);
                bf16* v_cache = reinterpret_cast<bf16*>(jb.v_cache);
                const bf16* kb = k_cache + ((size_t)b * n_kv + kvh) * T_max * D;
                const bf16* vb = v_cache + ((size_t)b * n_kv + kvh) * T_max * D;
                const int vpr = D >> 3, rpp = DC_CT / vpr, n_pass = DC_TILE / rpp;
                const int l_row = tid / vpr, l_col = (tid % vpr) * 8;
                uint4 kreg[2], vreg[2];
                auto load_tile = [&](int t0) {
#pragma unroll
                    for (int ps = 0; ps < 2; ++ps) {
                        kreg[ps] = make_uint4(0u, 0u, 0u, 0u);
                        vreg[ps] = make_uint4(0u, 0u, 0u, 0u);
                        const int key = t0 + ps * rpp + l_row;
                        if (ps < n_pass && key < k1 && key < pos) {
                            kreg[ps] = *reinterpret_cast<const uint4*>(kb + (size_t)key * D + l_col);
                            vreg[ps] = *reinterpret_cast<const uint4*>(vb + (size_t)key * D + l_col);
                        }
                    }
                };
                load_tile(k0);
                for (int u = warp; u <= n_rep; u += DC_CW) {
                    const bool is_k = u == n_rep;
                    if (is_k && !owns_pos) continue;
                    const bf16* src = row + (size_t)(is_k ? n_h + kvh : kvh * n_rep + u) * D;
                    const bf16* nw = is_k ? kn : qn;
                    float* dst = is_k ? sk : sq + u * 128;
                    float x1[2], x2[2], cs[2], sn[2];
                    float ssq = 0.f;
#pragma unroll
                    for (int t = 0; t < 2; ++t) {
                        const int i = lane + 32 * t;
                        x1[t] = x2[t] = cs[t] = sn[t] = 0.f;
                        if (i < HALF) {
                            x1[t] = dc_ldcg_bf16(src + i);
                            x2[t] = dc_ldcg_bf16(src + i + HALF);
                            cs[t] = bf2f(cos_tab[(size_t)pos * HALF + i]);
                            sn[t] = bf2f(sin_tab[(size_t)pos * HALF + i]);
                        }
                    }
#pragma unroll
                    for (int t = 0; t < 2; ++t) ssq += x1[t] * x1[t] + x2[t] * x2[t];
                    if (nw) {
                        const float r = 1.0f / sqrtf(warp_sum(ssq) / (float)D + jb.eps);
#pragma unroll
                        for (int t = 0; t < 2; ++t) {
                            const int i = lane + 32 * t;
                            if (i < HALF) {
                                x1[t] = rbf(bf2f(nw[i]) * rbf(x1[t] * r));
                                x2[t] = rbf(bf2f(nw[i + HALF]) * rbf(x2[t] * r));
                            }
                        }
                    }
#pragma unroll
                    for (int t = 0; t < 2; ++t) {
                        const int i = lane + 32 * t;
                        if (i < HALF) {
                            dst[i] = rbf(rbf(x1[t] * cs[t]) + rbf(-x2[t] * sn[t]));
                            dst[i + HALF] = rbf(rbf(x2[t] * cs[t]) + rbf(x1[t] * sn[t]));
                        }
                    }
                }
                if (owns_pos && tid < D) sv[tid] = dc_ldcg_bf16(row + (size_t)(n_h + n_kv + kvh) * D + tid);
                dc_bar(1, DC_CT);
                if (owns_pos && tid < D) {
                    const size_t off = (((size_t)b * n_kv + kvh) * T_max + pos) * D + tid;
                    k_cache[off] = f2bf(sk[tid]);
                    v_cache[off] = f2bf(sv[tid]);
                }
                const float scale_log2 = jb.scale * 1.4426950408889634f;
                float m_run = -INFINITY, l_run = 0.f;
                float o[4] = {0.f, 0.f, 0.f, 0.f};
                for (int t = 0; t < n_tiles; ++t) {
                    const int t0 = k0 + t * DC_TILE;
#pragma unroll
                    for (int ps = 0; ps < 2; ++ps) {
                        if (ps < n_pass) {
                            const int r_ = ps * rpp + l_row, key = t0 + r_;
                            if (key == pos && key < k1) {
                                uint4 kk, vv;
                                uint32_t* k32 = reinterpret_cast<uint32_t*>(&kk);
                                uint32_t* v32 = reinterpret_cast<uint32_t*>(&vv);
#pragma unroll
                                for (int q = 0; q < 4; ++q) {
                                    k32[q] = pack_bf16(sk[l_col + 2 * q], sk[l_col + 2 * q + 1]);
                                    v32[q] = pack_bf16(sv[l_col + 2 * q], sv[l_col + 2 * q + 1]);
                                }
                                kreg[ps] = kk;
                                vreg[ps] = vv;
                            }
                            *reinterpret_cast<uint4*>(kt + (size_t)r_ * KT + l_col * 2) = kreg[ps];
                            *reinterpret_cast<uint4*>(vt + (size_t)r_ * KT + l_col * 2) = vreg[ps];
                        }
                    }
                    if (t + 1 < n_tiles) load_tile(t0 + DC_TILE);
                    dc_bar(1, DC_CT);
                    if (warp < n_rep) {
                        const int r = warp;
                        float acc = 0.f;
                        const unsigned char* krow = kt + (size_t)lane * KT;
                        for (int c = 0; c < (D >> 3); ++c) {
                            const uint4 kv4 = *reinterpret_cast<const uint4*>(krow + c * 16);
                            const uint32_t* k32 = reinterpret_cast<const uint32_t*>(&kv4);
                            const float4 qa = *reinterpret_cast<const float4*>(&sq[r * 128 + c * 8]);
                            const float4 qb = *reinterpret_cast<const float4*>(&sq[r * 128 + c * 8 + 4]);
                            acc += bf16_lo(k32[0]) * qa.x + bf16_hi(k32[0]) * qa.y + bf16_lo(k32[1]) * qa.z + bf16_hi(k32[1]) * qa.w +
                                   bf16_lo(k32[2]) * qb.x + bf16_hi(k32[2]) * qb.y + bf16_lo(k32[3]) * qb.z + bf16_hi(k32[3]) * qb.w;
                        }
                        const bool in_range = t0 + lane < k1;
                        const float sc_ = in_range ? acc * scale_log2 : -INFINITY;
                        const float m_new = fmaxf(m_run, warp_max(sc_));
                        const float pr = in_range ? exp2f(sc_ - m_new) : 0.f;
                        const float alpha = exp2f(m_run - m_new);
                        l_run = l_run * alpha + warp_sum(pr);
                        m_run = m_new;
                        sp[r * DC_TILE + lane] = rbf(pr);
                        __syncwarp();
#pragma unroll
                        for (int q = 0; q < 4; ++q) o[q] *= alpha;
                        if (D == 128) {
#pragma unroll 8
                            for (int key = 0; key < DC_TILE; ++key) {
                                const uint2 vv = *reinterpret_cast<const uint2*>(vt + (size_t)key * KT + lane * 8);
                                const float pk = sp[r * DC_TILE + key];
                                o[0] = fmaf(pk, bf16_lo(vv.x), o[0]);
                                o[1] = fmaf(pk, bf16_hi(vv.x), o[1]);
                                o[2] = fmaf(pk, bf16_lo(vv.y), o[2]);
                                o[3] = fmaf(pk, bf16_hi(vv.y), o[3]);
                            }
                        } else {
#pragma unroll 8
                            for (int key = 0; key < DC_TILE; ++key) {
                                const uint32_t vv = *reinterpret_cast<const uint32_t*>(vt + (size_t)key * KT + lane * 4);
                                const float pk = sp[r * DC_TILE + key];
                                o[0] = fmaf(pk, bf16_lo(vv), o[0]);
                                o[1] = fmaf(pk, bf16_hi(vv), o[1]);
                            }
                        }
                        __syncwarp();
                    }
                    if (t + 1 < n_tiles) dc_bar(1, DC_CT);
                }
                const int EPL = D >> 5;
                if (cpg_eff == 1) {
                    if (warp < n_rep) {
                        bf16* yo = reinterpret_cast<bf16*>(jb.y) + ((size_t)b * n_h + kvh * n_rep + warp) * D + lane * EPL;
                        const float inv = 1.0f / l_run;
                        *reinterpret_cast<uint32_t*>(yo) = pack_bf16(o[0] * inv, o[1] * inv);
                        if (D == 128) *reinterpret_cast<uint32_t*>(yo + 2) = pack_bf16(o[2] * inv, o[3] * inv);
                    }
                    if (tid == 0) s_last = 1;
                } else {
                    if (warp < n_rep) {
                        float* pp = p.attn_part + (((size_t)b * n_h + kvh * n_rep + warp) * cpg + split) * (D + 4);
                        if (D == 128) *reinterpret_cast<float4*>(pp + lane * 4) = make_float4(o[0], o[1], o[2], o[3]);
                        else *reinterpret_cast<float2*>(pp + lane * 2) = make_float2(o[0], o[1]);
                        if (lane == 0) { pp[D] = m_run; pp[D + 1] = l_run; }
                    }
                    dc_bar(1, DC_CT);
                    if (tid == 0) {
                        __threadfence();
                        const unsigned old = atomicAdd(&grp_ctr[grp], 1u);
                        if (old == (unsigned)(cpg_eff - 1)) {
                            __threadfence();
                            s_last = 1;
                        }
                    }
                    dc_bar(1, DC_CT);
                    if (s_last) {
                        if (warp < n_rep) {
                            const int h = kvh * n_rep + warp;
                            const float* base = p.attn_part + ((size_t)b * n_h + h) * cpg * (D + 4);
                            float mc = -INFINITY, L = 0.f, O[4] = {0.f, 0.f, 0.f, 0.f};
                            for (int s0 = 0; s0 < cpg_eff; s0 += 4) {
                                float ms[4], ls[4], os[4][4];
#pragma unroll
                                for (int q = 0; q < 4; ++q) {
                                    const int s_ = min(s0 + q, cpg_eff - 1);
                                    const float* e = base + (size_t)s_ * (D + 4);
                                    ms[q] = __ldcg(e + D);
                                    ls[q] = __ldcg(e + D + 1);
                                    if (D == 128) {
                                        const float4 t4 = __ldcg(reinterpret_cast<const float4*>(e + lane * 4));
                                        os[q][0] = t4.x; os[q][1] = t4.y; os[q][2] = t4.z; os[q][3] = t4.w;
                                    } else {
                                        const float2 t2 = __ldcg(reinterpret_cast<const float2*>(e + lane * 2));
                                        os[q][0] = t2.x; os[q][1] = t2.y; os[q][2] = os[q][3] = 0.f;
                                    }
                                }
#pragma unroll
                                for (int q = 0; q < 4; ++q) {
                                    if (s0 + q < cpg_eff) {
                                        const float mn = fmaxf(mc, ms[q]);
                                        const float a = exp2f(mc - mn), w = exp2f(ms[q] - mn);
                                        L = L * a + w * ls[q];
#pragma unroll
                                        for (int e_ = 0; e_ < 4; ++e_) O[e_] = O[e_] * a + w * os[q][e_];
                                        mc = mn;
                                    }
                                }
                            }
                            bf16* yo = reinterpret_cast<bf16*>(jb.y) + ((size_t)b * n_h + h) * D + lane * EPL;
                            const float inv = 1.0f / L;
                            *reinterpret_cast<uint32_t*>(yo) = pack_bf16(O[0] * inv, O[1] * inv);
                            if (D == 128) *reinterpret_cast<uint32_t*>(yo + 2) = pack_bf16(O[2] * inv, O[3] * inv);
                        }
                        if (tid == 0) grp_ctr[grp] = 0u;
                    }
                }
            }
            stamp(j, 2);
            if (!last_job && !grid_dep(s_last != 0, (unsigned)G)) break;
            stamp(j, 3);
        }
    }
    dc_bar(1, DC_CT);
    stamp(DC_MAX_JOBS, 2);
    if (tid == 0) {
        __threadfence();
        const unsigned prev = atomicAdd(&p.sync[1], 1u);
        if (prev == gridDim.x - 1) {
            p.sync[0] = 0;
            p.sync[1] = 0;
            for (int j = 0; j < p.n_jobs; ++j) p.sync[DC_JOBCTR + j] = 0;
            __threadfence();
        }
    }
}

}

static unsigned long long* g_chain_trace = nullptr;
static int g_chain_trace_slots = 0, g_chain_trace_next = 0;
constexpr int DC_TRACE_WORDS = tl::DC_STAT_OFF + tl::DC_MAX_JOBS * 4;

extern "C" {

int tl_decode_chain_trace(void* buf, int n_slots) {
    g_chain_trace = (unsigned long long*)buf;
    g_chain_trace_slots = buf ? n_slots : 0;
    g_chain_trace_next = 0;
    return TL_OK;
}

size_t tl_decode_chain_ws(int M, int n_h, int n_kv, int d) {
    if (M < 1 || n_h < 1 || n_kv < 1) return 0;
    const int cpg = 160 / (n_kv * M) > 0 ? 160 / (n_kv * M) : 1;
    return (size_t)M * n_h * cpg * (d + 4) * sizeof(float) + 256;
}

int tl_decode_chain(const tl_decode_job* jobs, int n_jobs, int M, void* sync_slot, void* attn_ws, size_t attn_ws_bytes,
                    const void* pf_ptr, size_t pf_bytes, void* stream) {
    using namespace tl;
    TL_REQUIRE(M >= 1 && M <= DC_MAX_M, TL_ERR_INVALID, "tl_decode_chain: M=%d outside 1..%d", M, DC_MAX_M);
    TL_REQUIRE(jobs && n_jobs > 0 && n_jobs <= DC_MAX_JOBS && sync_slot, TL_ERR_INVALID, "tl_decode_chain: bad job list (n=%d, max %d)",
               n_jobs, DC_MAX_JOBS);
    const int grid = sm_count();
    int k_max = 0, n_attn = 0;
    for (int j = 0; j < n_jobs; ++j) {
        const tl_decode_job& jb = jobs[j];
        if (jb.type == TL_JOB_GEMV) {
            TL_REQUIRE(jb.K % 8 == 0 && jb.N % 2 == 0 && jb.N > 0 && (((uintptr_t)jb.W) & 15) == 0, TL_ERR_INVALID,
                       "tl_decode_chain: job %d bad GEMV shape / alignment", j);
            if (jb.K > k_max) k_max = jb.K;
        } else if (jb.type == TL_JOB_ATTN) {
            TL_REQUIRE((jb.d == 64 || jb.d == 128) && jb.n_kv > 0 && jb.n_h % jb.n_kv == 0 && jb.n_h / jb.n_kv <= 8, TL_ERR_INVALID,
                       "tl_decode_chain: job %d attention shape unsupported (d=%d n_h=%d n_kv=%d)", j, jb.d, jb.n_h, jb.n_kv);
            const int G = jb.n_kv * M;
            TL_REQUIRE(G <= grid && G <= 60, TL_ERR_INVALID, "tl_decode_chain: %d (row, kv head) groups do not fit", G);
            const int cpg = grid / G;
            TL_REQUIRE(attn_ws && attn_ws_bytes >= (size_t)M * jb.n_h * cpg * (jb.d + 4) * sizeof(float), TL_ERR_INVALID,
                       "tl_decode_chain: attention workspace too small");
            ++n_attn;
        } else {
            TL_REQUIRE(false, TL_ERR_INVALID, "tl_decode_chain: job %d has unsupported type %d", j, jb.type);
        }
    }
    (void)n_attn;
    constexpr int SMEM_CAP = 227 * 1024 - 1024;
    const size_t xs_bytes = (((size_t)M * k_max * 2) + 127) & ~(size_t)127;
    const size_t attn_bytes = (size_t)DC_ATTN_BYTES;
    const size_t fixed = xs_bytes + attn_bytes + 2 * DC_MAX_STAGES * sizeof(uint64_t);
    static int forced_kb = -1;
    if (forced_kb < 0) {
        const char* e = getenv("TL_CHAIN_STAGE_KB");
        forced_kb = e ? atoi(e) : 0;
    }
    int DC_STAGE = 0, n_stages = 0, NW = 0;
    TL_REQUIRE(fixed + 4 * 8192 <= (size_t)SMEM_CAP, TL_ERR_INVALID, "tl_decode_chain: M*K_max too large (%zu B fixed)", fixed);
    if (!forced_kb) {
        int kb = (int)((SMEM_CAP - fixed) / 8 / 1024);
        if (kb > 24) kb = 24;
        if (kb >= 12) { DC_STAGE = kb * 1024; n_stages = 8; NW = 8; }
    }
    if (!DC_STAGE) {
        DC_STAGE = (forced_kb >= 8 ? forced_kb : 16) * 1024;
        int max_stages = (int)((SMEM_CAP - fixed) / DC_STAGE);
        if (max_stages > DC_MAX_STAGES) max_stages = DC_MAX_STAGES;
        TL_REQUIRE(max_stages >= 4, TL_ERR_INVALID, "tl_decode_chain: fewer than 4 ring slots fit");
        for (int nw = DC_CW; nw >= 4; --nw) {
            const int st_ = max_stages / nw * nw;
            if (st_ > n_stages) { n_stages = st_; NW = nw; }
        }
    }
    const int DC_KC = (DC_STAGE / 4) & ~7;
    ChainParams prm = {};
    prm.n_jobs = n_jobs;
    prm.n_stages = n_stages;
    prm.NW = NW;
    prm.xs_bytes = (int)xs_bytes;
    static int dyn = -1, l2_ahead = -1;
    if (dyn < 0) {
        const char* e = getenv("TL_CHAIN_DYNAMIC");
        dyn = (e && e[0] == '1') ? 1 : 0;
        const char* a = getenv("TL_CHAIN_L2_AHEAD_KB");
        l2_ahead = a ? atoi(a) * 1024 : 0;
        if (l2_ahead < 0) l2_ahead = 0;
    }
    prm.dynamic = dyn;
    prm.stage_bytes = DC_STAGE;
    prm.kc = DC_KC;
    prm.l2_ahead = l2_ahead;
    prm.sync = (unsigned*)sync_slot;
    prm.attn_part = (float*)attn_ws;
    prm.pf_ptr = (const unsigned char*)pf_ptr;
    prm.pf_bytes = (((uintptr_t)pf_ptr) & 15) ? 0ull : (unsigned long long)(pf_bytes & ~(size_t)15);
    prm.trace = (g_chain_trace && g_chain_trace_next < g_chain_trace_slots)
                    ? g_chain_trace + (size_t)(g_chain_trace_next++) * DC_TRACE_WORDS : nullptr;
    for (int j = 0; j < n_jobs; ++j) prm.jobs[j] = jobs[j];
    const size_t smem = (size_t)n_stages * DC_STAGE + fixed;
    cudaLaunchConfig_t cfg = {};
    cfg.gridDim = dim3(grid);
    cfg.blockDim = dim3(DC_THREADS);
    cfg.dynamicSmemBytes = smem;
    cfg.stream = (cudaStream_t)stream;
    cudaLaunchAttribute attr[1];
    attr[0].id = cudaLaunchAttributeProgrammaticStreamSerialization;
    attr[0].val.programmaticStreamSerializationAllowed = 1;
    static int use_pdl = -1;
    if (use_pdl < 0) {
        const char* e = getenv("TL_PDL");
        use_pdl = (e && e[0] == '0') ? 0 : 1;
    }
    cfg.attrs = attr;
    cfg.numAttrs = use_pdl ? 1 : 0;
#define TL_DC_LAUNCH(MM)                                                                                                   \
    {                                                                                                                      \
        static bool done = false;                                                                                          \
        if (!done) {                                                                                                       \
            if (cudaFuncSetAttribute(decode_chain_kernel<MM>, cudaFuncAttributeMaxDynamicSharedMemorySize, SMEM_CAP) != cudaSuccess) \
                return check_launch("tl_decode_chain (smem attr)");                                                      \
            done = true;                                                                                                   \
        }                                                                                                                  \
        cudaLaunchKernelEx(&cfg, decode_chain_kernel<MM>, prm);                                                            \
    }
    switch (M) {
        case 1: TL_DC_LAUNCH(1) break;
        case 2: TL_DC_LAUNCH(2) break;
        case 3: TL_DC_LAUNCH(3) break;
        default: TL_DC_LAUNCH(4) break;
    }
#undef TL_DC_LAUNCH
    return check_launch("tl_decode_chain");
}

}
```

### tensorlink_b200/ml/shard.py

```python
from __future__ import annotations

from dataclasses import dataclass
from typing import Dict, List, Optional, Sequence

import torch

from .. import native as nat
from .configs import ShardModelConfig
from .weights import init_state_dict

ALIGN = 128


_GEMV_MAX_ROWS = None


def gemv_max_rows() -> int:
    global _GEMV_MAX_ROWS
    if _GEMV_MAX_ROWS is None:
        import os
        _GEMV_MAX_ROWS = max(1, min(8, int(os.environ.get("TL_GEMV_MAX_ROWS", "3"))))
    return _GEMV_MAX_ROWS


def _rope_inv_freq(cfg: ShardModelConfig) -> torch.Tensor:
    d = cfg.head_dim
    return 1.0 / (cfg.rope_theta ** (torch.arange(0, d, 2, dtype=torch.int64).to(torch.float32) / d))


class ShardParams:

    def __init__(self, cfg: ShardModelConfig, layer_ids: Sequence[int], has_embed: bool, has_head: bool,
                 device, with_grad: bool = False):
        self.cfg, self.layer_ids = cfg, list(layer_ids)
        self.has_embed, self.has_head = has_embed, has_head
        self.device = torch.device(device)
        H, I = cfg.hidden, cfg.intermediate
        spec: List[tuple] = []
        for li in self.layer_ids:
            spec += [(f"l{li}.ln1", (H,)), (f"l{li}.wqkv", (cfg.qkv_dim, H))]
            if cfg.qkv_bias:
                spec.append((f"l{li}.bqkv", (cfg.qkv_dim,)))
            if cfg.qk_norm:
                spec += [(f"l{li}.qn", (cfg.head_dim,)), (f"l{li}.kn", (cfg.head_dim,))]
            spec += [(f"l{li}.wo", (H, cfg.q_dim)), (f"l{li}.ln2", (H,)), (f"l{li}.wgu", (2 * I, H)),
                     (f"l{li}.wd", (H, I))]
        if has_embed:
            spec.append(("embed", (cfg.vocab, H)))
        if has_head:
            spec.append(("norm", (H,)))
            if not (cfg.tied and has_embed):
                spec.append(("head", (cfg.vocab, H)))
        self.spec = spec
        self.offsets: Dict[str, tuple] = {}
        off = 0
        for name, shape in spec:
            n = 1
            for s in shape:
                n *= s
            self.offsets[name] = (off, n, shape)
            off += (n + ALIGN - 1) // ALIGN * ALIGN
        self.numel = off
        self.flat = torch.zeros(off, dtype=torch.bfloat16, device=self.device)
        self.grad: Optional[torch.Tensor] = torch.zeros_like(self.flat) if with_grad else None
        self.v: Dict[str, torch.Tensor] = {n: self.flat[o:o + k].view(shape) for n, (o, k, shape) in self.offsets.items()}
        self.g: Dict[str, torch.Tensor] = ({n: self.grad[o:o + k].view(shape) for n, (o, k, shape) in self.offsets.items()}
                                           if with_grad else {})
        if has_head and cfg.tied and has_embed:
            self.v["head"] = self.v["embed"]
            if with_grad:
                self.g["head"] = self.g["embed"]

    def load_hf_state_dict(self, sd: Dict[str, torch.Tensor]):
        cfg = self.cfg
        dev = self.device

        def put(name, t):
            self.v[name].copy_(t.to(device=dev, dtype=torch.bfloat16))

        for li in self.layer_ids:
            p = f"model.layers.{li}."
            put(f"l{li}.ln1", sd[p + "input_layernorm.weight"])
            put(f"l{li}.wqkv", torch.cat([sd[p + "self_attn.q_proj.weight"], sd[p + "self_attn.k_proj.weight"],
                                          sd[p + "self_attn.v_proj.weight"]], dim=0))
            if cfg.qkv_bias:
                put(f"l{li}.bqkv", torch.cat([sd[p + "self_attn.q_proj.bias"], sd[p + "self_attn.k_proj.bias"],
                                              sd[p + "self_attn.v_proj.bias"]], dim=0))
            if cfg.qk_norm:
                put(f"l{li}.qn", sd[p + "self_attn.q_norm.weight"])
                put(f"l{li}.kn", sd[p + "self_attn.k_norm.weight"])
            put(f"l{li}.wo", sd[p + "self_attn.o_proj.weight"])
            put(f"l{li}.ln2", sd[p + "post_attention_layernorm.weight"])
            g, u = sd[p + "mlp.gate_proj.weight"], sd[p + "mlp.up_proj.weight"]
            put(f"l{li}.wgu", torch.stack([g, u], dim=1).reshape(2 * cfg.intermediate, cfg.hidden))
            put(f"l{li}.wd", sd[p + "mlp.down_proj.weight"])
        if self.has_embed:
            put("embed", sd["model.embed_tokens.weight"])
        if self.has_head:
            put("norm", sd["model.norm.weight"])
            if not (cfg.tied and self.has_embed):
                put("head", sd["lm_head.weight"] if "lm_head.weight" in sd else sd["model.embed_tokens.weight"])

    def hf_state_dict(self, grads: bool = False) -> Dict[str, torch.Tensor]:
        cfg = self.cfg
        if grads and getattr(self, "grad_settle", None) is not None:
            self.grad_settle()
        src = self.g if grads else self.v
        out: Dict[str, torch.Tensor] = {}
        for li in self.layer_ids:
            p = f"model.layers.{li}."
            out[p + "input_layernorm.weight"] = src[f"l{li}.ln1"].clone()
            q, k, v = src[f"l{li}.wqkv"].split([cfg.q_dim, cfg.kv_dim, cfg.kv_dim], dim=0)
            out[p + "self_attn.q_proj.weight"], out[p + "self_attn.k_proj.weight"] = q.clone(), k.clone()
            out[p + "self_attn.v_proj.weight"] = v.clone()
            if cfg.qkv_bias:
                bq, bk, bv = src[f"l{li}.bqkv"].split([cfg.q_dim, cfg.kv_dim, cfg.kv_dim], dim=0)
                out[p + "self_attn.q_proj.bias"], out[p + "self_attn.k_proj.bias"] = bq.clone(), bk.clone()
                out[p + "self_attn.v_proj.bias"] = bv.clone()
            if cfg.qk_norm:
                out[p + "self_attn.q_norm.weight"] = src[f"l{li}.qn"].clone()
                out[p + "self_attn.k_norm.weight"] = src[f"l{li}.kn"].clone()
            out[p + "self_attn.o_proj.weight"] = src[f"l{li}.wo"].clone()
            out[p + "post_attention_layernorm.weight"] = src[f"l{li}.ln2"].clone()
            gu = src[f"l{li}.wgu"].view(cfg.intermediate, 2, cfg.hidden)
            out[p + "mlp.gate_proj.weight"], out[p + "mlp.up_proj.weight"] = gu[:, 0].clone(), gu[:, 1].clone()
            out[p + "mlp.down_proj.weight"] = src[f"l{li}.wd"].clone()
        if self.has_embed:
            out["model.embed_tokens.weight"] = src["embed"].clone()
        if self.has_head:
            out["model.norm.weight"] = src["norm"].clone()
            out["lm_head.weight"] = out["model.embed_tokens.weight"] if (cfg.tied and self.has_embed) else src["head"].clone()
        return out

    def init_seeded(self, seed: int = 1234):
        cfg = self.cfg
        for li in self.layer_ids:
            sd = init_state_dict(cfg, seed, torch.bfloat16, "cpu", layers=[li], with_embed=False, with_head=False)
            sub = ShardParams.__new__(ShardParams)
            sub.__dict__.update(self.__dict__)
            sub.layer_ids, sub.has_embed, sub.has_head = [li], False, False
            sub.load_hf_state_dict(sd)
        sd = init_state_dict(cfg, seed, torch.bfloat16, "cpu", layers=[], with_embed=self.has_embed or (
            self.has_head and cfg.tied), with_head=self.has_head)
        sub = ShardParams.__new__(ShardParams)
        sub.__dict__.update(self.__dict__)
        sub.layer_ids = []
        sub.load_hf_state_dict(sd)

    def init_on_device(self, seed: int = 1234, std: float = 0.02):
        g = torch.Generator(device=self.device).manual_seed(seed)
        self.flat.normal_(0.0, std, generator=g)
        for name in self.v:
            if name.endswith(("ln1", "ln2", "qn", "kn")) or name == "norm":
                self.v[name].fill_(1.0)


@dataclass
class ShardBuffers:
    x: torch.Tensor
    h: torch.Tensor
    qkv: torch.Tensor
    q: torch.Tensor
    attn: torch.Tensor
    act: torch.Tensor


class CudaLayerGroup:

    def __init__(self, cfg: ShardModelConfig, params: ShardParams, max_batch: int, max_seq: int,
                 max_tokens: Optional[int] = None):
        nat.require_device()
        self.cfg, self.p = cfg, params
        self.layer_ids = params.layer_ids
        self.num_layers = len(self.layer_ids)
        self.input_vars = ["hidden_states", "past_len", "use_cache"]
        self.output_vars = ["hidden_states"]
        self.device = params.device
        self.B_max, self.T_max = max_batch, max_seq
        dev, bf = self.device, torch.bfloat16
        self.kc = [torch.zeros(max_batch, cfg.n_kv_heads, max_seq, cfg.head_dim, dtype=bf, device=dev)
                   for _ in self.layer_ids]
        self.vc = [torch.zeros_like(k) for k in self.kc]
        self.cos, self.sin = nat.rope_table(_rope_inv_freq(cfg).to(dev), max_seq)
        self.weights_after_last_layer = (params.v.get("head") if "head" in params.v else
                                         params.v.get(f"l{self.layer_ids[0]}.wqkv") if len(self.layer_ids) else None)
        self.pos_dev = torch.zeros(1, dtype=torch.int32, device=dev)
        self.kvlen_dev = torch.zeros(1, dtype=torch.int32, device=dev)
        self.kv_start_dev = torch.zeros(max_batch, dtype=torch.int32, device=dev)
        self.ragged = False
        self.n_max = max_tokens or max_batch * max_seq
        self._alloc_bufs(min(self.n_max, 8))
        self.dbufs = self._make_bufs(max_batch)
        self.gemm_ws = (torch.empty(nat.gemm_splitk_ws(min(max_batch, 128), max(cfg.qkv_dim, cfg.hidden)), dtype=torch.uint8,
                                    device=dev) if max_batch > 1 else None)
        self.dec_ws = torch.empty(max(nat.attn_decode_ws(max_batch, cfg.n_heads, cfg.head_dim, max_seq), 16),
                                  dtype=torch.uint8, device=dev)
        self.scale = cfg.head_dim ** -0.5
        self.allow_chain = True
        self.chain_sync: Optional[torch.Tensor] = None
        self.chain_attn_ws: Optional[torch.Tensor] = None
        self._chains: Dict[tuple, list] = {}

    def _make_bufs(self, n: int) -> ShardBuffers:
        cfg, dev, bf = self.cfg, self.device, torch.bfloat16
        return ShardBuffers(
            x=torch.empty(n, cfg.hidden, dtype=bf, device=dev), h=torch.empty(n, cfg.hidden, dtype=bf, device=dev),
            qkv=torch.empty(n, cfg.qkv_dim, dtype=bf, device=dev), q=torch.empty(n, cfg.q_dim, dtype=bf, device=dev),
            attn=torch.empty(n, cfg.q_dim, dtype=bf, device=dev),
            act=torch.empty(n, cfg.intermediate, dtype=bf, device=dev))

    def _alloc_bufs(self, n: int):
        self.bufs = self._make_bufs(n)
        self.n_alloc = n

    def _dbufs(self, n: int) -> ShardBuffers:
        b = self.dbufs
        return ShardBuffers(b.x[:n], b.h[:n], b.qkv[:n], b.q[:n], b.attn[:n], b.act[:n])

    def _bufs(self, n: int) -> ShardBuffers:
        if n > self.n_alloc:
            self._alloc_bufs(n)
        b = self.bufs
        return ShardBuffers(b.x[:n], b.h[:n], b.qkv[:n], b.q[:n], b.attn[:n], b.act[:n])

    def reset_cache(self, past_len: int = 0):
        self.pos_dev.fill_(past_len)
        self.kvlen_dev.fill_(past_len)

    def _kv_start(self):
        return self.kv_start_dev if self.ragged else None

    def _layer_prefill(self, j: int, x: torch.Tensor, B: int, S: int, past_len: int, w: ShardBuffers):
        cfg, v, li = self.cfg, self.p.v, self.layer_ids[j]
        ks = self._kv_start()
        nat.rmsnorm_fwd(x, v[f"l{li}.ln1"], cfg.rms_eps, out=w.h)
        nat.gemm(w.h, v[f"l{li}.wqkv"], out=w.qkv, bias=v.get(f"l{li}.bqkv"))
        nat.rope_kv_fwd(w.qkv, w.q, self.kc[j], self.vc[j], self.pos_dev, self.cos, self.sin, v.get(f"l{li}.qn"),
                        v.get(f"l{li}.kn"), cfg.rms_eps, S, cfg.n_heads, cfg.n_kv_heads, cfg.head_dim, kv_start=ks)
        nat.attn_prefill_fwd(w.q, self.kc[j], self.vc[j], w.attn, None, B, S, past_len, cfg.n_heads, cfg.n_kv_heads,
                             cfg.head_dim, self.scale, kv_start=ks)
        nat.gemm(w.attn, v[f"l{li}.wo"], out=x, residual=x)
        nat.rmsnorm_fwd(x, v[f"l{li}.ln2"], cfg.rms_eps, out=w.h)
        nat.gemm(w.h, v[f"l{li}.wgu"], out=w.act, flags=nat.EPI_SWIGLU)
        nat.gemm(w.act, v[f"l{li}.wd"], out=x, residual=x)

    FUSED_DECODE_MAX_T = 2048

    def _decode_attention(self, j: int, li: int, B: int, w: ShardBuffers):
        cfg, v = self.cfg, self.p.v
        ks = self._kv_start()
        if self.T_max <= self.FUSED_DECODE_MAX_T and (cfg.n_heads // cfg.n_kv_heads) <= 8:
            nat.attn_decode_fused(w.qkv, self.kc[j], self.vc[j], w.attn, self.pos_dev, self.cos, self.sin,
                                  v.get(f"l{li}.qn"), v.get(f"l{li}.kn"), cfg.rms_eps, B, cfg.n_heads, cfg.n_kv_heads,
                                  cfg.head_dim, self.scale, kv_start=ks)
            return
        nat.rope_kv_fwd(w.qkv, w.q, self.kc[j], self.vc[j], self.pos_dev, self.cos, self.sin, v.get(f"l{li}.qn"),
                        v.get(f"l{li}.kn"), cfg.rms_eps, 1, cfg.n_heads, cfg.n_kv_heads, cfg.head_dim, kv_start=ks)
        nat.attn_decode_fwd(w.q, self.kc[j], self.vc[j], w.attn, self.kvlen_dev, self.dec_ws, B, cfg.n_heads,
                            cfg.n_kv_heads, cfg.head_dim, self.scale, kv_start=ks)

    def _layer_decode(self, j: int, x: torch.Tensor, B: int, w: ShardBuffers, out: Optional[torch.Tensor] = None):
        cfg, v, li = self.cfg, self.p.v, self.layer_ids[j]
        if j + 1 < self.num_layers:
            after = v[f"l{self.layer_ids[j + 1]}.wqkv"]
        else:
            after = self.weights_after_last_layer
        nat.gemv(x, v[f"l{li}.wqkv"], out=w.qkv, bias=v.get(f"l{li}.bqkv"), norm_w=v[f"l{li}.ln1"], eps=cfg.rms_eps,
                 next_w=v[f"l{li}.wo"])
        self._decode_attention(j, li, B, w)
        nat.gemv(w.attn, v[f"l{li}.wo"], out=x, residual=x, next_w=v[f"l{li}.wgu"])
        nat.gemv(x, v[f"l{li}.wgu"], out=w.act, norm_w=v[f"l{li}.ln2"], eps=cfg.rms_eps, flags=nat.EPI_SWIGLU,
                 next_w=v[f"l{li}.wd"])
        nat.gemv(w.act, v[f"l{li}.wd"], out=x if out is None else out, residual=x, next_w=after)

    def _layer_decode_batched(self, j: int, x: torch.Tensor, B: int, w: ShardBuffers, out: Optional[torch.Tensor] = None):
        cfg, v, li = self.cfg, self.p.v, self.layer_ids[j]
        ws = self.gemm_ws if B <= 128 else None
        if j == 0:
            nat.rmsnorm_fwd(x, v[f"l{li}.ln1"], cfg.rms_eps, out=w.h)
        nat.gemm(w.h, v[f"l{li}.wqkv"], out=w.qkv, bias=v.get(f"l{li}.bqkv"), ws=ws)
        self._decode_attention(j, li, B, w)
        nat.gemm(w.attn, v[f"l{li}.wo"], out=x, residual=x, ws=ws, norm_w=v[f"l{li}.ln2"], eps=cfg.rms_eps, h_out=w.h)
        nat.gemm(w.h, v[f"l{li}.wgu"], out=w.act, flags=nat.EPI_SWIGLU, ws=ws)
        if j + 1 < self.num_layers:
            nat.gemm(w.act, v[f"l{li}.wd"], out=x, residual=x, ws=ws, norm_w=v[f"l{self.layer_ids[j + 1]}.ln1"],
                     eps=cfg.rms_eps, h_out=w.h)
        else:
            nat.gemm(w.act, v[f"l{li}.wd"], out=x if out is None else out, residual=x, ws=ws)

    def prefill(self, hidden: torch.Tensor, past_len: int = 0, kv_start=None) -> torch.Tensor:
        B, S, H = hidden.shape
        if B > self.B_max or past_len + S > self.T_max:
            raise ValueError(f"shard sized for B<={self.B_max}, T<={self.T_max}; got B={B}, T={past_len + S}")
        self._set_kv_start(kv_start, B, past_len + S)
        N = B * S
        w = self._bufs(N)
        w.x.copy_(hidden.reshape(N, H))
        self.pos_dev.fill_(past_len)
        for j in range(self.num_layers):
            self._layer_prefill(j, w.x, B, S, past_len, w)
        self.pos_dev.fill_(past_len + S)
        self.kvlen_dev.fill_(past_len + S)
        return w.x.view(B, S, H)

    def _set_kv_start(self, kv_start, B: int, T: int):
        if kv_start is None:
            self.ragged = False
            return
        ks = torch.as_tensor(kv_start, dtype=torch.int32).reshape(-1).cpu()
        if ks.numel() != B or bool((ks < 0).any()) or bool((ks >= T).any()):
            raise ValueError(f"kv_start needs {B} values in [0, {T}): every row keeps at least one real token")
        self.kv_start_dev.zero_()
        self.kv_start_dev[:B].copy_(ks, non_blocking=False)
        self.ragged = bool((ks != 0).any())

    def decode_step_inplace(self, x: torch.Tensor, out: Optional[torch.Tensor] = None, advance: bool = True):
        B = x.shape[0]
        w = self._dbufs(B)
        if advance:
            nat.advance_pos(self.kvlen_dev, None, 1)
        if self.chain_ok(B) or self.dq_ok(B):
            (self._decode_step_chained if self.chain_ok(B) else self._decode_step_dq)(x, B, out)
            if advance:
                nat.advance_pos(self.pos_dev, None, 1)
            return
        for j in range(self.num_layers):
            o = out if j == self.num_layers - 1 else None
            if B <= gemv_max_rows():
                self._layer_decode(j, x, B, w, o)
            else:
                self._layer_decode_batched(j, x, B, w, o)
        if advance:
            nat.advance_pos(self.pos_dev, None, 1)

    def chain_ok(self, B: int) -> bool:
        import os
        cfg = self.cfg
        return (os.environ.get("TL_DECODE_IMPL", "kernels") == "chain" and self.allow_chain and self.num_layers > 0
                and not self.ragged
                and B <= min(4, gemv_max_rows()) and cfg.n_kv_heads * B <= 60 and cfg.n_heads // cfg.n_kv_heads <= 8
                and cfg.head_dim in (64, 128))

    def _chain_group(self) -> int:
        import os
        return max(1, min(3, int(os.environ.get("TL_CHAIN_LAYERS", "1"))))

    def _decode_chains(self, x: torch.Tensor, B: int, out: Optional[torch.Tensor]):
        key = (B, x.data_ptr(), 0 if out is None else out.data_ptr())
        if key in self._chains:
            return self._chains[key]
        cfg, v = self.cfg, self.p.v
        w = self._dbufs(B)
        J = nat.make_job
        if self.chain_sync is None:
            self.chain_sync = torch.zeros(self.num_layers + 1, nat.CHAIN_SYNC_BYTES // 4, dtype=torch.int32, device=self.device)
            self.chain_attn_ws = torch.empty(nat.decode_chain_ws(min(self.B_max, 4), cfg.n_heads, cfg.n_kv_heads, cfg.head_dim),
                                             dtype=torch.uint8, device=self.device)
        per = self._chain_group()
        launches = []
        for g0 in range(0, self.num_layers, per):
            jobs = []
            g1 = min(self.num_layers, g0 + per)
            for j in range(g0, g1):
                li = self.layer_ids[j]
                jobs.append(J(nat.JOB_ATTN, x=w.qkv, y=w.attn, k_cache=self.kc[j], v_cache=self.vc[j], pos_dev=self.pos_dev,
                              cos_tab=self.cos, sin_tab=self.sin, q_norm_w=v.get(f"l{li}.qn"), k_norm_w=v.get(f"l{li}.kn"),
                              n_h=cfg.n_heads, n_kv=cfg.n_kv_heads, d=cfg.head_dim, T_max=self.T_max, scale=self.scale,
                              eps=cfg.rms_eps))
                jobs.append(J(nat.JOB_GEMV, N=cfg.hidden, K=cfg.q_dim, flags=nat.EPI_RESIDUAL, W=v[f"l{li}.wo"], x=w.attn, y=x,
                              residual=x))
                jobs.append(J(nat.JOB_GEMV, N=2 * cfg.intermediate, K=cfg.hidden, flags=nat.EPI_SWIGLU, W=v[f"l{li}.wgu"], x=x,
                              y=w.act, norm_w=v[f"l{li}.ln2"], eps=cfg.rms_eps))
                last = j == self.num_layers - 1
                jobs.append(J(nat.JOB_GEMV, N=cfg.hidden, K=cfg.intermediate, flags=nat.EPI_RESIDUAL, W=v[f"l{li}.wd"], x=w.act,
                              y=(out if (last and out is not None) else x), residual=x))
                if not last:
                    ln = self.layer_ids[j + 1]
                    bq = v.get(f"l{ln}.bqkv")
                    jobs.append(J(nat.JOB_GEMV, N=cfg.qkv_dim, K=cfg.hidden, flags=nat.EPI_BIAS if bq is not None else 0,
                                  W=v[f"l{ln}.wqkv"], x=x, y=w.qkv, bias=bq, norm_w=v[f"l{ln}.ln1"], eps=cfg.rms_eps))
            nxt = v[f"l{self.layer_ids[g1]}.wo"] if g1 < self.num_layers else self.weights_after_last_layer
            launches.append(nat.DecodeChain(jobs, B, self.chain_sync[g0 // per], self.chain_attn_ws, nxt))
        self._chains[key] = launches
        return launches

    def _decode_step_chained(self, x: torch.Tensor, B: int, out: Optional[torch.Tensor]):
        cfg, v = self.cfg, self.p.v
        w = self._dbufs(B)
        l0 = self.layer_ids[0]
        nat.gemv(x, v[f"l{l0}.wqkv"], out=w.qkv, bias=v.get(f"l{l0}.bqkv"), norm_w=v[f"l{l0}.ln1"], eps=cfg.rms_eps,
                 next_w=v[f"l{l0}.wo"])
        for ch in self._decode_chains(x, B, out):
            ch.launch()

    def dq_ok(self, B: int) -> bool:
        import os
        return os.environ.get("TL_DECODE_IMPL", "kernels") == "dq" and self.allow_chain and self.num_layers > 1 and B <= min(4, gemv_max_rows())

    def _decode_step_dq(self, x: torch.Tensor, B: int, out: Optional[torch.Tensor]):
        cfg, v = self.cfg, self.p.v
        w = self._dbufs(B)
        key = ("dq", B, x.data_ptr(), 0 if out is None else out.data_ptr())
        if key not in self._chains:
            J = nat.make_job
            if self.chain_sync is None:
                self.chain_sync = torch.zeros(self.num_layers + 1, nat.CHAIN_SYNC_BYTES // 4, dtype=torch.int32, device=self.device)
                self.chain_attn_ws = torch.empty(nat.decode_chain_ws(min(self.B_max, 4), cfg.n_heads, cfg.n_kv_heads, cfg.head_dim),
                                                 dtype=torch.uint8, device=self.device)
            launches = []
            for j in range(self.num_layers - 1):
                li, ln = self.layer_ids[j], self.layer_ids[j + 1]
                bq = v.get(f"l{ln}.bqkv")
                jobs = [J(nat.JOB_GEMV, N=cfg.hidden, K=cfg.intermediate, flags=nat.EPI_RESIDUAL, W=v[f"l{li}.wd"], x=w.act, y=x, residual=x),
                        J(nat.JOB_GEMV, N=cfg.qkv_dim, K=cfg.hidden, flags=nat.EPI_BIAS if bq is not None else 0, W=v[f"l{ln}.wqkv"], x=x,
                          y=w.qkv, bias=bq, norm_w=v[f"l{ln}.ln1"], eps=cfg.rms_eps)]
                launches.append(nat.DecodeChain(jobs, B, self.chain_sync[j], self.chain_attn_ws, v[f"l{ln}.wo"]))
            self._chains[key] = launches
        chains = self._chains[key]
        l0 = self.layer_ids[0]
        nat.gemv(x, v[f"l{l0}.wqkv"], out=w.qkv, bias=v.get(f"l{l0}.bqkv"), norm_w=v[f"l{l0}.ln1"], eps=cfg.rms_eps, next_w=v[f"l{l0}.wo"])
        for j, li in enumerate(self.layer_ids):
            self._decode_attention(j, li, B, w)
            nat.gemv(w.attn, v[f"l{li}.wo"], out=x, residual=x, next_w=v[f"l{li}.wgu"])
            nat.gemv(x, v[f"l{li}.wgu"], out=w.act, norm_w=v[f"l{li}.ln2"], eps=cfg.rms_eps, flags=nat.EPI_SWIGLU, next_w=v[f"l{li}.wd"])
            if j + 1 < self.num_layers:
                chains[j].launch()
            else:
                nat.gemv(w.act, v[f"l{li}.wd"], out=x if out is None else out, residual=x, next_w=self.weights_after_last_layer)

    def n_chain_launches(self) -> int:
        per = self._chain_group()
        return 1 + (self.num_layers + per - 1) // per

    def check(self):
        if self.chain_sync is not None and int(self.chain_sync[:, 2].max().item()):
            self.chain_sync[:, :4].zero_()
            raise nat.NativeError("decode chain kernel timed out waiting for a dependency (co-residency of its CTAs lost?)")

    def forward(self, **kwargs) -> dict:
        hs = kwargs["hidden_states"]
        past_len = int(kwargs.get("past_len", 0) or 0)
        out = dict(kwargs)
        out["hidden_states"] = self.prefill(hs, past_len).clone()
        return out

    __call__ = forward
```

### tensorlink_b200/ml/stage.py

```python
from __future__ import annotations

from typing import Dict, List, Optional

import torch

from .. import native as nat
from .configs import ShardModelConfig
from .shard import CudaLayerGroup, ShardParams, gemv_max_rows


class CudaStage:
    def __init__(self, cfg: ShardModelConfig, layer_ids, has_embed: bool, has_head: bool, device,
                 max_batch: int, max_seq: int, n_slots: int = 1, training: bool = False,
                 state_dict: Optional[Dict[str, torch.Tensor]] = None, seed: int = 1234, init: str = "seeded",
                 max_tokens: Optional[int] = None):
        nat.require_device()
        self.cfg = cfg
        self.device = torch.device(device)
        self.has_embed, self.has_head = has_embed, has_head
        self.supports_training, self.trainer = bool(training), None
        self.supports_kv_start = True
        self.params = ShardParams(cfg, layer_ids, has_embed, has_head, self.device, with_grad=training)
        if state_dict is not None:
            self.params.load_hf_state_dict(state_dict)
        elif init == "device":
            self.params.init_on_device(seed)
        else:
            self.params.init_seeded(seed)
        self.max_batch, self.max_seq = max_batch, max_seq
        self.slots: List[CudaLayerGroup] = [CudaLayerGroup(cfg, self.params, max_batch, max_seq, max_tokens)
                                            for _ in range(n_slots)]
        dev = self.device
        self.x_dec = [torch.zeros(max_batch, cfg.hidden, dtype=torch.bfloat16, device=dev) for _ in range(n_slots)]
        self.ids_dec = [torch.zeros(max_batch, dtype=torch.int64, device=dev) for _ in range(n_slots)]
        self.graphs: Dict[tuple, torch.cuda.CUDAGraph] = {}
        if has_head:
            self.head_ws = torch.empty(max(nat.lmhead_ws(min(max_batch, 8), cfg.vocab), max_batch * 64 * 8 + 256),
                                       dtype=torch.uint8, device=dev)
            self.logits_dec = torch.empty(max_batch, cfg.vocab, dtype=torch.bfloat16, device=dev)
            self.hn = torch.empty(max_batch, cfg.hidden, dtype=torch.bfloat16, device=dev)
            self.sampling: Optional[dict] = None
            self.sample_ctr = torch.zeros(n_slots, max_batch, dtype=torch.int32, device=dev)
            self.sample_ws: Optional[torch.Tensor] = None
            self.procs: Optional[dict] = None
            self.lp_flags = 0
            self.hist_log: Optional[torch.Tensor] = None
            self.hist_len = self.hist_bits = self.lp_params = self.lp_ws = None

    def embed(self, ids: torch.Tensor) -> torch.Tensor:
        return nat.embed_fwd(ids.contiguous(), self.params.v["embed"])

    def prefill(self, hidden: torch.Tensor, past_len: int = 0, slot: int = 0, kv_start=None) -> torch.Tensor:
        return self.slots[slot].prefill(hidden, past_len, kv_start)

    def head_logits(self, hidden: torch.Tensor) -> torch.Tensor:
        cfg, v = self.cfg, self.params.v
        n = hidden.shape[0]
        if n <= gemv_max_rows():
            return nat.gemv(hidden.contiguous(), v["head"], norm_w=v["norm"], eps=cfg.rms_eps)
        hn = nat.rmsnorm_fwd(hidden.contiguous(), v["norm"], cfg.rms_eps)
        return nat.gemm(hn, v["head"])

    def set_sampling(self, sampling: Optional[dict]):
        if not self.has_head or sampling == self.sampling:
            return
        self.sampling = sampling
        self.graphs.clear()
        self.sample_ctr.zero_()
        if sampling is not None and self.sample_ws is None:
            self.sample_ws = torch.empty(nat.sample_ws(self.max_batch), dtype=torch.uint8, device=self.device)

    def set_logits_processors(self, procs: Optional[dict], length: int = 0):
        if not self.has_head:
            return
        flags = 0 if procs is None else (nat.LP_BAN if procs["ngram"] > 0 or (procs["min_new"] > 0 and procs["eos"]) else 0)
        if (procs is None) != (self.procs is None) or flags != self.lp_flags:
            self.graphs.clear()
        self.procs, self.lp_flags = procs, flags
        if procs is None:
            return
        n_slots, dev, V = len(self.slots), self.device, self.cfg.vocab
        if self.lp_ws is None:
            self.lp_ws = torch.empty(nat.logits_proc_ws(self.max_batch, V), dtype=torch.uint8, device=dev)
            self.lp_params = torch.zeros(nat.LP_PARAMS, dtype=torch.int32, device=dev)
            self.hist_len = torch.zeros(n_slots, self.max_batch, dtype=torch.int32, device=dev)
            self.hist_bits = torch.zeros(n_slots, self.max_batch, (V + 31) // 32, dtype=torch.int32, device=dev)
        if self.hist_log is None or self.hist_log.shape[2] < length:
            self.hist_log = torch.zeros(n_slots, self.max_batch, max(length, self.max_seq), dtype=torch.int32, device=dev)
            self.graphs.clear()
        self.lp_params.copy_(nat.lp_params(procs["penalty"], procs["ngram"], procs["min_new"], procs["prompt_len"],
                                           procs["eos"] if procs["min_new"] > 0 else []))

    def fill_history(self, slot: int, prompt: torch.Tensor):
        nat.history_fill(prompt.contiguous(), self.hist_log[slot], self.hist_len[slot], self.hist_bits[slot], self.cfg.vocab)

    def head_argmax(self, hidden: torch.Tensor, ids_out: torch.Tensor, slot: int = 0):
        if self.procs is not None:
            self._head_processed(hidden, ids_out, slot)
            return
        self._head_greedy(hidden, ids_out)
        if self.sampling is not None:
            B = hidden.shape[0]
            s = self.sampling
            nat.sample(self.logits_dec[:B], ids_out, self.sample_ctr[slot], self.sample_ws, s["temperature"], s["top_k"], s["top_p"],
                       s["seed"] + 0x9E3779B97F4A7C15 * slot)

    def _head_processed(self, hidden: torch.Tensor, ids_out: torch.Tensor, slot: int):
        cfg, v = self.cfg, self.params.v
        B = hidden.shape[0]
        logits = self.logits_dec[:B]
        if B <= gemv_max_rows():
            nat.gemv(hidden, v["head"], out=logits, norm_w=v["norm"], eps=cfg.rms_eps)
        else:
            nat.rmsnorm_fwd(hidden, v["norm"], cfg.rms_eps, out=self.hn[:B])
            nat.gemm(self.hn[:B], v["head"], out=logits)
        hist = (self.hist_log[slot], self.hist_len[slot], self.hist_bits[slot], self.lp_params)
        if self.sampling is None:
            nat.argmax_proc(logits, ids_out, *hist, self.lp_ws, self.lp_flags)
        else:
            s = self.sampling
            nat.sample_proc(logits, ids_out, *hist, self.sample_ctr[slot], self.lp_ws, s["temperature"], s["top_k"], s["top_p"],
                            s["seed"] + 0x9E3779B97F4A7C15 * slot, self.lp_flags)

    def _head_greedy(self, hidden: torch.Tensor, ids_out: torch.Tensor):
        cfg, v = self.cfg, self.params.v
        B = hidden.shape[0]
        if B <= gemv_max_rows():
            nat.lmhead_argmax(hidden, v["head"], v["norm"], cfg.rms_eps, ids_out, self.logits_dec[:B], self.head_ws)
        else:
            nat.rmsnorm_fwd(hidden, v["norm"], cfg.rms_eps, out=self.hn[:B])
            nat.gemm(self.hn[:B], v["head"], out=self.logits_dec[:B])
            nat.argmax_bf16(self.logits_dec[:B], ids_out, self.head_ws)

    def _decode_body_ring(self, slot: int, B: int, ring):
        grp = self.slots[slot]
        if self.has_embed:
            ring.wait_ids(slot, bump=grp.kvlen_dev)
            ring.log_token(slot, B)
            x = self.x_dec[slot][:B]
            nat.embed_fwd(ring.ids_in[slot][:B], self.params.v["embed"], out=x)
        else:
            ring.wait_x(slot, bump=grp.kvlen_dev)
            x = ring.x_in[slot][:B]
        if self.has_head:
            grp.decode_step_inplace(x, advance=False)
            self.head_argmax(x, ring.first_ids_in[slot][:B], slot)
            ring.signal_ids(slot, bump=grp.pos_dev)
        else:
            grp.decode_step_inplace(x, out=ring.next_x_in[slot][:B], advance=False)
            ring.signal_x(slot, bump=grp.pos_dev)

    def _decode_body(self, slot: int, B: int, ring=None):
        if ring is not None:
            self._decode_body_ring(slot, B, ring)
            return
        x = self.x_dec[slot][:B]
        if self.has_embed:
            nat.embed_fwd(self.ids_dec[slot][:B], self.params.v["embed"], out=x)
        self.slots[slot].decode_step_inplace(x)
        if self.has_head:
            self.head_argmax(x, self.ids_dec[slot][:B], slot)

    def decode(self, slot: int, B: int, use_graph: bool = True, ring=None):
        if not use_graph:
            self._decode_body(slot, B, ring)
            return
        ragged = self.slots[slot].ragged
        key = (slot, B, ragged) if ring is None else (slot, B, ragged, id(ring))
        g = self.graphs.get(key)
        if g is None:
            grp = self.slots[slot]
            saved = (grp.pos_dev.clone(), grp.kvlen_dev.clone(), self.ids_dec[slot].clone(), self.x_dec[slot].clone())
            ctr_saved = self.sample_ctr.clone() if self.has_head else None
            hist_saved = None
            if self.has_head and self.procs is not None:
                hist_saved = (self.hist_len.clone(), self.hist_bits.clone())
            side = torch.cuda.Stream(device=self.device)
            side.wait_stream(torch.cuda.current_stream())
            with torch.cuda.stream(side):
                self._decode_body(slot, B)
            torch.cuda.current_stream().wait_stream(side)
            grp.pos_dev.copy_(saved[0]); grp.kvlen_dev.copy_(saved[1])
            self.ids_dec[slot].copy_(saved[2]); self.x_dec[slot].copy_(saved[3])
            if ctr_saved is not None:
                self.sample_ctr.copy_(ctr_saved)
            if hist_saved is not None:
                self.hist_len.copy_(hist_saved[0]); self.hist_bits.copy_(hist_saved[1])
            torch.cuda.synchronize(self.device)
            g = torch.cuda.CUDAGraph()
            with torch.cuda.graph(g):
                self._decode_body(slot, B, ring)
            self.graphs[key] = g
        g.replay()

    def check(self):
        for g in self.slots:
            g.check()

    def n_decode_launches(self, B: int, ring: bool = False) -> int:
        fused = self.slots[0].T_max <= self.slots[0].FUSED_DECODE_MAX_T
        gemv = B <= gemv_max_rows()
        if self.slots[0].chain_ok(B):
            n = self.slots[0].n_chain_launches() + 2
        elif self.slots[0].dq_ok(B):
            n = 1 + len(self.slots[0].layer_ids) * (3 + (1 if fused else 3)) + 2
        else:
            n = len(self.slots[0].layer_ids) * ((7 if gemv else 10) - (2 if fused else 0)) + 2 + (0 if gemv else 1)
        if ring:
            n += (3 if self.has_embed else 2) - 2
        if self.has_embed:
            n += 1
        if self.has_head:
            n += 3 if B <= gemv_max_rows() else 4
        return n
```

### tensorlink_b200/native.py

```python
from __future__ import annotations

import ctypes
import os
from ctypes import POINTER, c_char_p, c_float, c_int, c_int32, c_size_t, c_void_p
from typing import Optional

import torch

_HERE = os.path.dirname(os.path.abspath(__file__))
LIB_PATH = os.path.join(_HERE, "csrc", "libtensorlink_b200.so")

EPI_BIAS, EPI_RESIDUAL, EPI_SWIGLU, EPI_OUT_F32, EPI_ACCUM, A_MN_MAJOR, B_MN_MAJOR = 1, 2, 4, 8, 16, 32, 64


class NativeError(RuntimeError):
    pass


_SIGS = {
    "tl_abi_version": (c_int, []),
    "tl_last_error": (c_char_p, []),
    "tl_device_info": (c_int, [POINTER(c_int), POINTER(c_int), POINTER(c_int)]),
    "tl_rmsnorm_fwd": (c_int, [c_void_p, c_void_p, c_void_p, c_void_p, c_int, c_int, c_float, c_void_p]),
    "tl_embed_fwd": (c_int, [c_void_p, c_void_p, c_void_p, c_int, c_int, c_int, c_void_p]),
    "tl_gemm_bf16": (c_int, [c_void_p, c_void_p, c_void_p, c_int, c_int, c_int, c_int, c_int, c_int,
                             c_void_p, c_void_p, c_int, c_void_p]),
    "tl_gemm_splitk_ws": (c_size_t, [c_int, c_int]),
    "tl_gemm_bf16_ws": (c_int, [c_void_p, c_void_p, c_void_p, c_int, c_int, c_int, c_int, c_int, c_int,
                                c_void_p, c_void_p, c_int, c_void_p, c_size_t, c_void_p]),
    "tl_gemm_bf16_ws_norm": (c_int, [c_void_p, c_void_p, c_void_p, c_int, c_int, c_int, c_int, c_int, c_int,
                                     c_void_p, c_void_p, c_int, c_void_p, c_size_t, c_void_p, c_float, c_void_p, c_void_p]),
    "tl_gemv_bf16": (c_int, [c_void_p, c_void_p, c_void_p, c_int, c_int, c_int, c_void_p, c_void_p, c_void_p,
                             c_float, c_int, c_void_p]),
    "tl_gemv_bf16_pf": (c_int, [c_void_p, c_void_p, c_void_p, c_int, c_int, c_int, c_void_p, c_void_p, c_void_p,
                                c_float, c_int, c_void_p, c_size_t, c_void_p]),
    "tl_rope_table": (c_int, [c_void_p, c_void_p, c_void_p, c_int, c_int, c_void_p]),
    "tl_rope_kv_fwd": (c_int, [c_void_p, c_void_p, c_void_p, c_void_p, c_void_p, c_void_p, c_void_p, c_void_p,
                               c_void_p, c_float, c_int, c_int, c_int, c_int, c_int, c_int, c_void_p]),
    "tl_attn_prefill_fwd": (c_int, [c_void_p, c_void_p, c_void_p, c_void_p, c_void_p, c_int, c_int, c_int, c_int,
                                    c_int, c_int, c_int, c_float, c_void_p]),
    "tl_attn_decode_ws": (c_size_t, [c_int, c_int, c_int, c_int]),
    "tl_attn_decode_fwd": (c_int, [c_void_p, c_void_p, c_void_p, c_void_p, c_void_p, c_void_p, c_size_t, c_int,
                                   c_int, c_int, c_int, c_int, c_float, c_void_p]),
    "tl_attn_decode_fused": (c_int, [c_void_p] * 9 + [c_float, c_int, c_int, c_int, c_int, c_int, c_float, c_void_p]),
    "tl_rope_kv_fwd_rows": (c_int, [c_void_p, c_void_p, c_void_p, c_void_p, c_void_p, c_void_p, c_void_p, c_void_p,
                                    c_void_p, c_float, c_int, c_int, c_int, c_int, c_int, c_int, c_void_p, c_void_p]),
    "tl_attn_prefill_fwd_rows": (c_int, [c_void_p, c_void_p, c_void_p, c_void_p, c_void_p, c_int, c_int, c_int, c_int,
                                         c_int, c_int, c_int, c_float, c_void_p, c_void_p]),
    "tl_attn_decode_fwd_rows": (c_int, [c_void_p, c_void_p, c_void_p, c_void_p, c_void_p, c_void_p, c_size_t, c_int,
                                        c_int, c_int, c_int, c_int, c_float, c_void_p, c_void_p]),
    "tl_attn_decode_fused_rows": (c_int, [c_void_p] * 9 + [c_float, c_int, c_int, c_int, c_int, c_int, c_float, c_void_p,
                                                           c_void_p]),
    "tl_decode_chain_ws": (c_size_t, [c_int, c_int, c_int, c_int]),
    "tl_decode_chain_trace": (c_int, [c_void_p, c_int]),
    "tl_decode_chain": (c_int, [c_void_p, c_int, c_int, c_void_p, c_void_p, c_size_t, c_void_p, c_size_t, c_void_p]),
    "tl_peer_alloc": (c_int, [c_size_t, POINTER(c_void_p), c_void_p]),
    "tl_peer_open": (c_int, [c_void_p, POINTER(c_void_p)]),
    "tl_peer_close": (c_int, [c_void_p]),
    "tl_peer_free": (c_int, [c_void_p]),
    "tl_peer_wait": (c_int, [c_void_p, c_void_p, c_void_p, c_void_p, ctypes.c_uint64, c_void_p, c_void_p]),
    "tl_peer_signal": (c_int, [c_void_p, c_void_p, c_void_p, c_void_p]),
    "tl_peer_put": (c_int, [c_void_p, c_void_p, c_size_t, c_void_p, c_void_p, c_void_p]),
    "tl_lmhead_ws": (c_size_t, [c_int, c_int]),
    "tl_lmhead_argmax": (c_int, [c_void_p, c_void_p, c_void_p, c_float, c_void_p, c_void_p, c_void_p, c_size_t,
                                 c_int, c_int, c_int, c_void_p]),
    "tl_argmax_bf16": (c_int, [c_void_p, c_void_p, c_void_p, c_size_t, c_int, c_int, c_void_p]),
    "tl_sample_ws": (c_size_t, [c_int]),
    "tl_sample": (c_int, [c_void_p, c_void_p, c_int, c_int, c_float, c_int, c_float, ctypes.c_uint64, c_void_p, c_void_p, c_size_t,
                          c_void_p]),
    "tl_logits_proc_ws": (c_size_t, [c_int, c_int]),
    "tl_history_fill": (c_int, [c_void_p, c_void_p, c_void_p, c_void_p, c_int, c_int, c_int, c_int, c_void_p]),
    "tl_argmax_proc": (c_int, [c_void_p] * 6 + [c_int, c_void_p, c_size_t, c_int, c_int, c_int, c_void_p]),
    "tl_sample_proc": (c_int, [c_void_p] * 6 + [c_int, c_int, c_int, c_int, c_float, c_int, c_float, ctypes.c_uint64, c_void_p,
                                                c_void_p, c_size_t, c_void_p]),
    "tl_advance_pos": (c_int, [c_void_p, c_void_p, c_int, c_void_p]),
    "tl_append_token": (c_int, [c_void_p, c_void_p, c_void_p, c_int, c_int, c_void_p]),
    "tl_swiglu_fwd": (c_int, [c_void_p, c_void_p, c_int, c_int, c_void_p]),
    "tl_swiglu_bwd": (c_int, [c_void_p, c_void_p, c_void_p, c_int, c_int, c_void_p]),
    "tl_rmsnorm_bwd": (c_int, [c_void_p, c_void_p, c_void_p, c_void_p, c_void_p, c_void_p, c_void_p, c_int, c_int,
                               c_void_p]),
    "tl_rope_kv_bwd": (c_int, [c_void_p, c_void_p, c_void_p, c_void_p, c_void_p, c_void_p, c_int, c_int, c_int, c_int,
                               c_int, c_int, c_void_p]),
    "tl_qk_norm_bwd": (c_int, [c_void_p] * 6 + [c_float, c_int, c_int, c_int, c_int, c_void_p]),
    "tl_attn_bwd_ws": (c_size_t, [c_int, c_int, c_int]),
    "tl_attn_bwd": (c_int, [c_void_p] * 10 + [c_size_t, c_int, c_int, c_int, c_int, c_int, c_int, c_float, c_void_p]),
    "tl_attn_bwd_rows": (c_int, [c_void_p] * 10 + [c_size_t, c_int, c_int, c_int, c_int, c_int, c_int, c_float, c_void_p,
                                                   c_void_p]),
    "tl_ce_fwd_bwd": (c_int, [c_void_p, c_void_p, c_void_p, c_void_p, c_void_p, c_float, c_int, c_int, c_void_p]),
    "tl_embed_bwd": (c_int, [c_void_p, c_void_p, c_void_p, c_int, c_int, c_int, c_void_p]),
    "tl_colsum": (c_int, [c_void_p, c_void_p, c_int, c_int, c_int, c_void_p]),
    "tl_f32_to_bf16_accum": (c_int, [c_void_p, c_void_p, c_size_t, c_int, c_void_p]),
    "tl_add_inplace": (c_int, [c_void_p, c_void_p, c_size_t, c_void_p]),
    "tl_scale_add_bf16": (c_int, [c_void_p, c_void_p, c_float, c_int, c_size_t, c_void_p]),
    "tl_scale_add_f32": (c_int, [c_void_p, c_void_p, c_float, c_int, c_size_t, c_void_p]),
    "tl_adamw_step": (c_int, [c_void_p, c_void_p, c_void_p, c_void_p, c_size_t, c_float, c_float, c_float, c_float,
                              c_float, c_int, c_int, c_void_p]),
}



class DecodeJob(ctypes.Structure):
    _fields_ = [("type", c_int32), ("N", c_int32), ("K", c_int32), ("flags", c_int32),
                ("n_h", c_int32), ("n_kv", c_int32), ("d", c_int32), ("T_max", c_int32),
                ("eps", c_float), ("scale", c_float),
                ("W", c_void_p), ("x", c_void_p), ("y", c_void_p), ("bias", c_void_p), ("residual", c_void_p),
                ("norm_w", c_void_p), ("pos_dev", c_void_p), ("cos_tab", c_void_p), ("sin_tab", c_void_p),
                ("q_norm_w", c_void_p), ("k_norm_w", c_void_p), ("k_cache", c_void_p), ("v_cache", c_void_p)]


JOB_GEMV, JOB_ATTN = 0, 1
ATTN_POS_PER_ROW = 1
CHAIN_MAX_JOBS, CHAIN_SYNC_BYTES = 16, 1024

_lib: Optional[ctypes.CDLL] = None


def load() -> ctypes.CDLL:
    global _lib
    if _lib is not None:
        return _lib
    if not os.path.exists(LIB_PATH):
        raise NativeError(
            f"{LIB_PATH} is missing: build it with `python -c 'import __graft_entry__ as g; g.build()'` "
            "(tensorlink_b200 has no CPU or eager fallback)")
    lib = ctypes.CDLL(LIB_PATH)
    for name, (res, args) in _SIGS.items():
        fn = getattr(lib, name)
        fn.restype = res
        fn.argtypes = args
    _lib = lib
    return lib


def exported_symbols():
    return sorted(_SIGS)


def last_error() -> str:
    return (load().tl_last_error() or b"").decode()


def _check(rc: int, what: str):
    if rc != 0:
        raise NativeError(f"{what} failed ({rc}): {last_error()}")


_device_ok = False


def require_device():
    global _device_ok
    if _device_ok:
        return
    if not torch.cuda.is_available():
        raise NativeError("no CUDA device: the tensorlink_b200 shard executor runs on sm_90a only")
    sm, ma, mi = c_int(), c_int(), c_int()
    _check(load().tl_device_info(sm, ma, mi), "tl_device_info")
    _device_ok = True


def _p(t: Optional[torch.Tensor]) -> Optional[int]:
    if t is None:
        return None
    assert t.is_cuda, "device tensor expected"
    return t.data_ptr()


_raw_stream = getattr(torch._C, "_cuda_getCurrentRawStream", None)


def _stream() -> int:
    if _raw_stream is not None:
        return _raw_stream(torch.cuda.current_device())
    return torch.cuda.current_stream().cuda_stream


def _bf16(*ts):
    for t in ts:
        if t is not None:
            assert t.dtype == torch.bfloat16 and t.is_contiguous(), (t.dtype, t.is_contiguous())


def rmsnorm_fwd(x: torch.Tensor, w: torch.Tensor, eps: float, out: Optional[torch.Tensor] = None,
                rstd: Optional[torch.Tensor] = None) -> torch.Tensor:
    require_device()
    _bf16(x, w, out)
    H = x.shape[-1]
    rows = x.numel() // H
    out = torch.empty_like(x) if out is None else out
    _check(load().tl_rmsnorm_fwd(_p(x), _p(w), _p(out), _p(rstd), rows, H, eps, _stream()), "tl_rmsnorm_fwd")
    return out


def embed_fwd(ids: torch.Tensor, table: torch.Tensor, out: Optional[torch.Tensor] = None) -> torch.Tensor:
    require_device()
    assert ids.dtype == torch.int64 and ids.is_contiguous()
    _bf16(table, out)
    V, H = table.shape
    n = ids.numel()
    out = torch.empty(*ids.shape, H, dtype=torch.bfloat16, device=table.device) if out is None else out
    _check(load().tl_embed_fwd(_p(ids), _p(table), _p(out), n, H, V, _stream()), "tl_embed_fwd")
    return out


def gemm_splitk_ws(M: int, N: int) -> int:
    return int(load().tl_gemm_splitk_ws(M, N))


def gemm(a: torch.Tensor, b: torch.Tensor, out: Optional[torch.Tensor] = None, *, bias=None, residual=None,
         flags: int = 0, M: Optional[int] = None, N: Optional[int] = None, K: Optional[int] = None,
         ws: Optional[torch.Tensor] = None, norm_w: Optional[torch.Tensor] = None, eps: float = 1e-6,
         h_out: Optional[torch.Tensor] = None) -> torch.Tensor:
    require_device()
    _bf16(a, b, bias, residual)
    a_mn, b_mn = bool(flags & A_MN_MAJOR), bool(flags & B_MN_MAJOR)
    if M is None:
        M = a.shape[1] if a_mn else a.shape[0]
    if K is None:
        K = a.shape[0] if a_mn else a.shape[1]
    if N is None:
        N = b.shape[1] if b_mn else b.shape[0]
    c_cols = N // 2 if flags & EPI_SWIGLU else N
    if out is None:
        out = torch.empty(M, c_cols, dtype=torch.float32 if flags & EPI_OUT_F32 else torch.bfloat16, device=a.device)
    if bias is not None:
        flags |= EPI_BIAS
    if residual is not None:
        flags |= EPI_RESIDUAL
    if norm_w is not None:
        assert h_out is not None and h_out.dtype == torch.bfloat16 and h_out.is_contiguous() and h_out.shape == out.shape
        _check(load().tl_gemm_bf16_ws_norm(_p(a), _p(b), _p(out), M, N, K, a.stride(0), b.stride(0), out.stride(0), _p(bias),
                                           _p(residual), flags, _p(ws), 0 if ws is None else ws.numel() * ws.element_size(),
                                           _p(norm_w), eps, _p(h_out), _stream()), "tl_gemm_bf16_ws_norm")
        return out
    if ws is not None:
        _check(load().tl_gemm_bf16_ws(_p(a), _p(b), _p(out), M, N, K, a.stride(0), b.stride(0), out.stride(0), _p(bias),
                                      _p(residual), flags, _p(ws), ws.numel() * ws.element_size(), _stream()),
               "tl_gemm_bf16_ws")
        return out
    _check(load().tl_gemm_bf16(_p(a), _p(b), _p(out), M, N, K, a.stride(0), b.stride(0), out.stride(0), _p(bias),
                               _p(residual), flags, _stream()), "tl_gemm_bf16")
    return out


_PREFETCH_BYTES = None


def prefetch_bytes() -> int:
    global _PREFETCH_BYTES
    if _PREFETCH_BYTES is None:
        _PREFETCH_BYTES = int(float(os.environ.get("TL_PREFETCH_MB", "8")) * (1 << 20))
    return _PREFETCH_BYTES


def gemv(x: torch.Tensor, w: torch.Tensor, out: Optional[torch.Tensor] = None, *, bias=None, residual=None,
         norm_w=None, eps: float = 1e-6, flags: int = 0, next_w: Optional[torch.Tensor] = None) -> torch.Tensor:
    require_device()
    _bf16(x, w, bias, residual, norm_w, out)
    M, K = x.shape
    N = w.shape[0]
    if out is None:
        out = torch.empty(M, N // 2 if flags & EPI_SWIGLU else N, dtype=torch.bfloat16, device=x.device)
    if bias is not None:
        flags |= EPI_BIAS
    if residual is not None:
        flags |= EPI_RESIDUAL
    if next_w is not None and prefetch_bytes() > 0:
        nb = min(next_w.numel() * next_w.element_size(), prefetch_bytes())
        _check(load().tl_gemv_bf16_pf(_p(x), _p(w), _p(out), M, N, K, _p(bias), _p(residual), _p(norm_w), eps, flags,
                                      _p(next_w), nb, _stream()), "tl_gemv_bf16_pf")
        return out
    _check(load().tl_gemv_bf16(_p(x), _p(w), _p(out), M, N, K, _p(bias), _p(residual), _p(norm_w), eps, flags,
                               _stream()), "tl_gemv_bf16")
    return out


def rope_table(inv_freq: torch.Tensor, max_pos: int):
    require_device()
    assert inv_freq.dtype == torch.float32 and inv_freq.is_cuda
    half = inv_freq.numel()
    cos = torch.empty(max_pos, half, dtype=torch.bfloat16, device=inv_freq.device)
    sin = torch.empty_like(cos)
    _check(load().tl_rope_table(_p(inv_freq), _p(cos), _p(sin), max_pos, half, _stream()), "tl_rope_table")
    return cos, sin


def _kv_start(kv_start, B):
    if kv_start.dtype != torch.int32 or not kv_start.is_cuda or kv_start.numel() < B or not kv_start.is_contiguous():
        raise NativeError(f"kv_start must be a contiguous int32 CUDA tensor of at least {B} rows")


def rope_kv_fwd(qkv, q_out, k_cache, v_cache, pos0_dev, cos_tab, sin_tab, q_norm_w, k_norm_w, eps, S, n_h, n_kv, d,
                kv_start=None):
    require_device()
    _bf16(qkv, q_out, k_cache, v_cache, cos_tab, sin_tab, q_norm_w, k_norm_w)
    n_tokens = qkv.shape[0]
    T_max = k_cache.shape[2]
    if kv_start is None:
        _check(load().tl_rope_kv_fwd(_p(qkv), _p(q_out), _p(k_cache), _p(v_cache), _p(pos0_dev), _p(cos_tab), _p(sin_tab),
                                     _p(q_norm_w), _p(k_norm_w), eps, n_tokens, S, n_h, n_kv, d, T_max, _stream()),
               "tl_rope_kv_fwd")
        return
    _kv_start(kv_start, n_tokens // S)
    _check(load().tl_rope_kv_fwd_rows(_p(qkv), _p(q_out), _p(k_cache), _p(v_cache), _p(pos0_dev), _p(cos_tab), _p(sin_tab),
                                      _p(q_norm_w), _p(k_norm_w), eps, n_tokens, S, n_h, n_kv, d, T_max, _p(kv_start),
                                      _stream()), "tl_rope_kv_fwd_rows")


def attn_prefill_fwd(q, k_cache, v_cache, out, lse, B, S, past_len, n_h, n_kv, d, scale, kv_start=None):
    require_device()
    _bf16(q, k_cache, v_cache, out)
    T_max = k_cache.shape[2]
    if kv_start is None:
        _check(load().tl_attn_prefill_fwd(_p(q), _p(k_cache), _p(v_cache), _p(out), _p(lse), B, S, past_len, n_h, n_kv, d,
                                          T_max, scale, _stream()), "tl_attn_prefill_fwd")
        return
    _kv_start(kv_start, B)
    _check(load().tl_attn_prefill_fwd_rows(_p(q), _p(k_cache), _p(v_cache), _p(out), _p(lse), B, S, past_len, n_h, n_kv, d,
                                           T_max, scale, _p(kv_start), _stream()), "tl_attn_prefill_fwd_rows")


def attn_decode_ws(B, n_h, d, T_max) -> int:
    return int(load().tl_attn_decode_ws(B, n_h, d, T_max))


def attn_decode_fwd(q, k_cache, v_cache, out, kv_len_dev, ws, B, n_h, n_kv, d, scale, kv_start=None):
    require_device()
    _bf16(q, k_cache, v_cache, out)
    T_max = k_cache.shape[2]
    if kv_start is None:
        _check(load().tl_attn_decode_fwd(_p(q), _p(k_cache), _p(v_cache), _p(out), _p(kv_len_dev), _p(ws),
                                         ws.numel() * ws.element_size(), B, n_h, n_kv, d, T_max, scale, _stream()),
               "tl_attn_decode_fwd")
        return
    _kv_start(kv_start, B)
    _check(load().tl_attn_decode_fwd_rows(_p(q), _p(k_cache), _p(v_cache), _p(out), _p(kv_len_dev), _p(ws),
                                          ws.numel() * ws.element_size(), B, n_h, n_kv, d, T_max, scale, _p(kv_start),
                                          _stream()), "tl_attn_decode_fwd_rows")


def lmhead_ws(M, V) -> int:
    return int(load().tl_lmhead_ws(M, V))


def lmhead_argmax(x, w, norm_w, eps, ids_out, logits_out, ws):
    require_device()
    _bf16(x, w, norm_w, logits_out)
    M, H = x.shape
    V = w.shape[0]
    assert ids_out.dtype == torch.int64
    _check(load().tl_lmhead_argmax(_p(x), _p(w), _p(norm_w), eps, _p(ids_out), _p(logits_out), _p(ws),
                                   ws.numel() * ws.element_size(), M, V, H, _stream()), "tl_lmhead_argmax")


def argmax_bf16(logits, ids_out, ws):
    require_device()
    _bf16(logits)
    M, V = logits.shape
    _check(load().tl_argmax_bf16(_p(logits), _p(ids_out), _p(ws), ws.numel() * ws.element_size(), M, V, _stream()),
           "tl_argmax_bf16")


def sample_ws(M: int) -> int:
    return int(load().tl_sample_ws(M))


def sample(logits, ids_out, counters, ws, temperature: float = 1.0, top_k: int = 0, top_p: float = 1.0, seed: int = 0):
    require_device()
    _bf16(logits)
    M, V = logits.shape
    assert ids_out.dtype == torch.int64 and counters.dtype == torch.int32 and counters.numel() >= M
    _check(load().tl_sample(_p(logits), _p(ids_out), M, V, float(temperature), int(top_k or 0), float(top_p), int(seed) & (2 ** 64 - 1),
                            _p(counters), _p(ws), ws.numel() * ws.element_size(), _stream()), "tl_sample")


LP_PENALTY, LP_NGRAM, LP_MIN_NEW, LP_PROMPT, LP_N_EOS, LP_EOS, LP_MAX_EOS = 0, 1, 2, 3, 4, 5, 8
LP_PARAMS = LP_EOS + LP_MAX_EOS
LP_BAN = 1


def logits_proc_ws(M: int, V: int) -> int:
    return int(load().tl_logits_proc_ws(M, V))


def _history(log, length, bits, M: int, V: int):
    for t in (log, length, bits):
        if t.dtype != torch.int32 or not t.is_cuda or not t.is_contiguous() or t.shape[0] < M:
            raise NativeError(f"history tensors must be contiguous int32 CUDA tensors of at least {M} rows")
    if bits.shape[1] != (V + 31) // 32:
        raise NativeError(f"history bitmap has {bits.shape[1]} words per row, V={V} needs {(V + 31) // 32}")
    return log.shape[1]


def history_fill(prompt, log, length, bits, V: int):
    require_device()
    assert prompt.dtype == torch.int64 and prompt.is_contiguous()
    M, S = prompt.shape
    L = _history(log, length, bits, M, V)
    _check(load().tl_history_fill(_p(prompt), _p(log), _p(length), _p(bits), M, S, L, V, _stream()), "tl_history_fill")


def argmax_proc(logits, ids_out, log, length, bits, params, ws, flags: int = 0):
    require_device()
    _bf16(logits)
    M, V = logits.shape
    L = _history(log, length, bits, M, V)
    assert ids_out.dtype == torch.int64 and params.dtype == torch.int32 and params.numel() >= LP_PARAMS
    _check(load().tl_argmax_proc(_p(logits), _p(ids_out), _p(log), _p(length), _p(bits), _p(params), flags, _p(ws),
                                 ws.numel() * ws.element_size(), M, V, L, _stream()), "tl_argmax_proc")


def sample_proc(logits, ids_out, log, length, bits, params, counters, ws, temperature: float = 1.0, top_k: int = 0,
                top_p: float = 1.0, seed: int = 0, flags: int = 0):
    require_device()
    _bf16(logits)
    M, V = logits.shape
    L = _history(log, length, bits, M, V)
    assert ids_out.dtype == torch.int64 and counters.dtype == torch.int32 and counters.numel() >= M
    assert params.dtype == torch.int32 and params.numel() >= LP_PARAMS
    _check(load().tl_sample_proc(_p(logits), _p(ids_out), _p(log), _p(length), _p(bits), _p(params), flags, M, V, L,
                                 float(temperature), int(top_k or 0), float(top_p), int(seed) & (2 ** 64 - 1), _p(counters),
                                 _p(ws), ws.numel() * ws.element_size(), _stream()), "tl_sample_proc")


def lp_params(penalty: float, ngram: int, min_new: int, prompt_len: int, eos_ids) -> torch.Tensor:
    import struct
    eos_ids = list(eos_ids)
    if len(eos_ids) > LP_MAX_EOS:
        raise NotImplementedError(f"min_new_tokens with more than {LP_MAX_EOS} EOS ids")
    p = [struct.unpack("<i", struct.pack("<f", float(penalty)))[0], int(ngram), int(min_new), int(prompt_len), len(eos_ids)]
    p += [int(e) for e in eos_ids] + [0] * (LP_MAX_EOS - len(eos_ids))
    return torch.tensor(p, dtype=torch.int32)


def advance_pos(pos_dev, kv_len_dev, delta: int):
    require_device()
    _check(load().tl_advance_pos(_p(pos_dev), _p(kv_len_dev), delta, _stream()), "tl_advance_pos")


def append_token(ids, out_tokens, step_dev):
    require_device()
    assert ids.dtype == torch.int64 and out_tokens.dtype == torch.int64 and out_tokens.is_contiguous()
    B, ld = out_tokens.shape
    _check(load().tl_append_token(_p(ids), _p(out_tokens), _p(step_dev), B, ld, _stream()), "tl_append_token")


class _RawCuda:

    def __init__(self, ptr: int, nbytes: int):
        self.__cuda_array_interface__ = {"shape": (nbytes,), "typestr": "|u1", "data": (ptr, False), "version": 3,
                                         "strides": None}


def tensor_from_ptr(ptr: int, nbytes: int) -> torch.Tensor:
    return torch.as_tensor(_RawCuda(ptr, nbytes))


def peer_alloc(nbytes: int):
    require_device()
    ptr, h = c_void_p(), ctypes.create_string_buffer(64)
    _check(load().tl_peer_alloc(nbytes, ctypes.byref(ptr), h), "tl_peer_alloc")
    return ptr.value, bytes(h.raw)


def peer_open(handle: bytes) -> int:
    require_device()
    ptr = c_void_p()
    _check(load().tl_peer_open(ctypes.create_string_buffer(handle, 64), ctypes.byref(ptr)), "tl_peer_open")
    return ptr.value


def peer_close(ptr: int):
    _check(load().tl_peer_close(ptr), "tl_peer_close")


def peer_free(ptr: int):
    _check(load().tl_peer_free(ptr), "tl_peer_free")


def peer_wait(flag, want, err, wait_ns=None, timeout_ns: int = 0, bump=None):
    require_device()
    _check(load().tl_peer_wait(_p(flag), _p(want), _p(err), _p(wait_ns), timeout_ns, _p(bump), _stream()), "tl_peer_wait")


def peer_signal(flag_peer, sent, bump=None):
    require_device()
    _check(load().tl_peer_signal(_p(flag_peer), _p(sent), _p(bump), _stream()), "tl_peer_signal")


def peer_put(dst_peer, src, flag_peer, sent):
    require_device()
    nbytes = src.numel() * src.element_size()
    _check(load().tl_peer_put(_p(dst_peer), _p(src), nbytes, _p(flag_peer), _p(sent), _stream()), "tl_peer_put")


def swiglu_fwd(gu, h):
    require_device(); _bf16(gu, h)
    M, I = h.shape
    _check(load().tl_swiglu_fwd(_p(gu), _p(h), M, I, _stream()), "tl_swiglu_fwd")


def swiglu_bwd(gu, dh, dgu):
    require_device(); _bf16(gu, dh, dgu)
    M, I = dh.shape
    _check(load().tl_swiglu_bwd(_p(gu), _p(dh), _p(dgu), M, I, _stream()), "tl_swiglu_bwd")


def rmsnorm_bwd(x, w, dy, rstd, dx, dw_accum, dx_add=None):
    require_device(); _bf16(x, w, dy, dx, dx_add)
    H = x.shape[-1]
    _check(load().tl_rmsnorm_bwd(_p(x), _p(w), _p(dy), _p(rstd), _p(dx_add), _p(dx), _p(dw_accum), x.numel() // H, H,
                                 _stream()), "tl_rmsnorm_bwd")


def rope_kv_bwd(dq, dk, dv, dqkv, cos_tab, sin_tab, S, n_h, n_kv, d):
    require_device(); _bf16(dq, dk, dv, dqkv)
    _check(load().tl_rope_kv_bwd(_p(dq), _p(dk), _p(dv), _p(dqkv), _p(cos_tab), _p(sin_tab), dqkv.shape[0], S, n_h, n_kv,
                                 d, dk.shape[2], _stream()), "tl_rope_kv_bwd")


def attn_bwd_ws(B, S, n_h) -> int:
    return int(load().tl_attn_bwd_ws(B, S, n_h))


def attn_bwd(q, k_cache, v_cache, out, dout, lse, dq, dk, dv, ws, B, S, n_h, n_kv, d, scale, kv_start=None):
    require_device(); _bf16(q, k_cache, v_cache, out, dout, dq, dk, dv)
    if kv_start is None:
        _check(load().tl_attn_bwd(_p(q), _p(k_cache), _p(v_cache), _p(out), _p(dout), _p(lse), _p(dq), _p(dk), _p(dv), _p(ws),
                                  ws.numel() * ws.element_size(), B, S, n_h, n_kv, d, k_cache.shape[2], scale, _stream()),
               "tl_attn_bwd")
        return
    _kv_start(kv_start, B)
    _check(load().tl_attn_bwd_rows(_p(q), _p(k_cache), _p(v_cache), _p(out), _p(dout), _p(lse), _p(dq), _p(dk), _p(dv),
                                   _p(ws), ws.numel() * ws.element_size(), B, S, n_h, n_kv, d, k_cache.shape[2], scale,
                                   _p(kv_start), _stream()), "tl_attn_bwd_rows")


def ce_fwd_bwd(logits, labels, loss_sum, n_valid, dlogits, grad_scale: float):
    require_device(); _bf16(logits, dlogits)
    M, V = logits.shape
    assert labels.dtype == torch.int64 and loss_sum.dtype == torch.float32
    _check(load().tl_ce_fwd_bwd(_p(logits), _p(labels), _p(loss_sum), _p(n_valid), _p(dlogits), grad_scale, M, V,
                                _stream()), "tl_ce_fwd_bwd")


def embed_bwd(ids, dout, dtable):
    require_device(); _bf16(dout, dtable)
    V, H = dtable.shape
    _check(load().tl_embed_bwd(_p(ids), _p(dout), _p(dtable), ids.numel(), H, V, _stream()), "tl_embed_bwd")


def colsum(dy, db_accum):
    require_device()
    assert db_accum.dtype == torch.float32
    M, N = dy.shape
    _check(load().tl_colsum(_p(dy), _p(db_accum), M, N, dy.stride(0), _stream()), "tl_colsum")


def f32_to_bf16_accum(src, dst, accumulate: bool):
    require_device()
    _check(load().tl_f32_to_bf16_accum(_p(src), _p(dst), src.numel(), int(accumulate), _stream()), "tl_f32_to_bf16_accum")


def add_inplace(a, b):
    require_device(); _bf16(a, b)
    _check(load().tl_add_inplace(_p(a), _p(b), a.numel(), _stream()), "tl_add_inplace")


def scale_add(a, b, scale: float, accumulate: bool = True):
    require_device()
    assert a.dtype == b.dtype and a.numel() == b.numel() and a.is_contiguous() and b.is_contiguous()
    if a.dtype == torch.bfloat16:
        _check(load().tl_scale_add_bf16(_p(a), _p(b), scale, int(accumulate), a.numel(), _stream()), "tl_scale_add_bf16")
    else:
        assert a.dtype == torch.float32
        _check(load().tl_scale_add_f32(_p(a), _p(b), scale, int(accumulate), a.numel(), _stream()), "tl_scale_add_f32")


def adamw_step(param, grad, m, v, lr, beta1, beta2, eps, wd, step: int, decoupled: bool):
    require_device()
    _check(load().tl_adamw_step(_p(param), _p(grad), _p(m), _p(v), param.numel(), lr, beta1, beta2, eps, wd, step,
                                int(decoupled), _stream()), "tl_adamw_step")


def attn_decode_fused(qkv, k_cache, v_cache, out, pos_dev, cos_tab, sin_tab, q_norm_w, k_norm_w, eps, B, n_h, n_kv, d, scale,
                      kv_start=None):
    require_device(); _bf16(qkv, k_cache, v_cache, out)
    if kv_start is None:
        _check(load().tl_attn_decode_fused(_p(qkv), _p(k_cache), _p(v_cache), _p(out), _p(pos_dev), _p(cos_tab), _p(sin_tab),
                                           _p(q_norm_w), _p(k_norm_w), eps, B, n_h, n_kv, d, k_cache.shape[2], scale, _stream()),
               "tl_attn_decode_fused")
        return
    _kv_start(kv_start, B)
    _check(load().tl_attn_decode_fused_rows(_p(qkv), _p(k_cache), _p(v_cache), _p(out), _p(pos_dev), _p(cos_tab), _p(sin_tab),
                                            _p(q_norm_w), _p(k_norm_w), eps, B, n_h, n_kv, d, k_cache.shape[2], scale,
                                            _p(kv_start), _stream()), "tl_attn_decode_fused_rows")


def decode_chain_ws(M: int, n_h: int, n_kv: int, d: int) -> int:
    return int(load().tl_decode_chain_ws(M, n_h, n_kv, d))


CHAIN_TRACE_WORDS = 2 * (CHAIN_MAX_JOBS + 1) * 4 + CHAIN_MAX_JOBS * 160 + CHAIN_MAX_JOBS * 4


def decode_chain_trace(buf: Optional[torch.Tensor]):
    _check(load().tl_decode_chain_trace(_p(buf), 0 if buf is None else buf.shape[0]), "tl_decode_chain_trace")


def make_job(type_, **kw) -> DecodeJob:
    j = DecodeJob()
    j.type = type_
    for k, v in kw.items():
        if isinstance(v, torch.Tensor):
            v = v.data_ptr()
        setattr(j, k, v)
    return j


class DecodeChain:

    def __init__(self, jobs, M: int, sync_slot: torch.Tensor, attn_ws: torch.Tensor, next_w: Optional[torch.Tensor] = None):
        assert 1 <= len(jobs) <= CHAIN_MAX_JOBS
        self.n, self.M = len(jobs), M
        self.host = (DecodeJob * self.n)(*jobs)
        self.sync_slot, self.attn_ws, self.next_w = sync_slot, attn_ws, next_w
        assert sync_slot.numel() * sync_slot.element_size() >= CHAIN_SYNC_BYTES

    def launch(self):
        require_device()
        nb = 0
        if self.next_w is not None and prefetch_bytes() > 0:
            nb = min(self.next_w.numel() * self.next_w.element_size(), prefetch_bytes())
        _check(load().tl_decode_chain(ctypes.cast(self.host, c_void_p), self.n, self.M, _p(self.sync_slot), _p(self.attn_ws),
                                      self.attn_ws.numel() * self.attn_ws.element_size(), _p(self.next_w) if nb else None, nb,
                                      _stream()), "tl_decode_chain")


def qk_norm_bwd(qkv_pre, dqkv, qn, kn, dqn_acc, dkn_acc, eps, n_h, n_kv, d):
    require_device(); _bf16(qkv_pre, dqkv, qn, kn)
    _check(load().tl_qk_norm_bwd(_p(qkv_pre), _p(dqkv), _p(qn), _p(kn), _p(dqn_acc), _p(dkn_acc), eps, dqkv.shape[0], n_h,
                                 n_kv, d, _stream()), "tl_qk_norm_bwd")
```

Measured before the change: 190.3.

## Run whole decode layers in device-resident persistent chains with fused attention

Moves the decode job table to device memory so a chain can hold up to 192 jobs, letting many layers, including the first QKV GEMV, run in one persistent launch. The fused decode attention is factored into a shared device function usable inside the chain, and the separate dq decode path is removed. The default weight prefetch size also drops to zero. This is meant to cut kernel launch count and per-launch overhead, at the cost of larger chain kernels and losing prefetch overlap by default.

```diff
diff --git a/include/tensorlink_b200.h b/include/tensorlink_b200.h
--- a/include/tensorlink_b200.h
+++ b/include/tensorlink_b200.h
@@ -121,6 +121,7 @@
 #define TL_JOB_ATTN 1
 #define TL_ATTN_POS_PER_ROW 1
 #define TL_DECODE_CHAIN_MAX_JOBS 16
+#define TL_DECODE_CHAIN_JOBS 192
 #define TL_DECODE_CHAIN_SYNC_BYTES 1024
 typedef struct tl_decode_job {
     int32_t type, N, K, flags;
@@ -139,10 +140,11 @@
     const void* k_norm_w;
     void* k_cache;
     void* v_cache;
+    const void* kv_start;
 } tl_decode_job;
 size_t tl_decode_chain_ws(int M, int n_h, int n_kv, int d);
-int tl_decode_chain(const tl_decode_job* jobs, int n_jobs, int M, void* sync_slot, void* attn_ws, size_t attn_ws_bytes,
-                    const void* pf_ptr, size_t pf_bytes, void* stream);
+int tl_decode_chain(const tl_decode_job* jobs, const tl_decode_job* jobs_dev, int n_jobs, int M, void* sync_slot, void* attn_ws,
+                    size_t attn_ws_bytes, const void* pf_ptr, size_t pf_bytes, void* stream);
 int tl_decode_chain_trace(void* buf, int n_slots);
 
 int tl_peer_alloc(size_t bytes, void** ptr, unsigned char* handle64);
diff --git a/tensorlink_b200/csrc/attention.cu b/tensorlink_b200/csrc/attention.cu
--- a/tensorlink_b200/csrc/attention.cu
+++ b/tensorlink_b200/csrc/attention.cu
@@ -1,5 +1,6 @@
 #include <stdlib.h>
 
+#include "attn_decode_fused.cuh"
 #include "common.cuh"
 
 namespace tl {
@@ -685,160 +686,17 @@
 
 namespace tl {
 
-constexpr int FD_THREADS = 128, FD_MAX_T = 2048;
-
 template <int D, bool ROWS>
 __global__ void __launch_bounds__(FD_THREADS) attn_decode_fused_kernel(
     const bf16* __restrict__ qkv, bf16* __restrict__ k_cache, bf16* __restrict__ v_cache, bf16* __restrict__ out,
     const int32_t* __restrict__ pos_dev, const bf16* __restrict__ cos_tab, const bf16* __restrict__ sin_tab,
     const bf16* __restrict__ q_norm_w, const bf16* __restrict__ k_norm_w, float eps, int n_h, int n_kv, int T_max,
     float scale_log2, const int32_t* __restrict__ kv_start) {
-    constexpr int HALF = D / 2;
     asm volatile("griddepcontrol.wait;" ::: "memory");
     asm volatile("griddepcontrol.launch_dependents;");
-    const int h = blockIdx.x, b = blockIdx.y, tid = threadIdx.x, lane = tid & 31, warp = tid >> 5;
-    const int n_rep = n_h / n_kv, kvh = h / n_rep;
-    const int pos = *pos_dev;
-    int k_start = 0;
-    if constexpr (ROWS) {
-        k_start = kv_start[b];
-        cos_tab -= (size_t)k_start * HALF;
-        sin_tab -= (size_t)k_start * HALF;
-    }
-    const int heads = n_h + 2 * n_kv;
-    __shared__ __align__(16) float sq[D], sk[D], sv[D];
-    __shared__ float sscore[FD_MAX_T + 1];
-    __shared__ float sred[FD_THREADS / 32];
-    __shared__ float s_bc[2];
-    __shared__ __align__(16) float so[FD_THREADS / 32][D];
-
-    const bf16* row = qkv + (size_t)b * heads * D;
-    float q1 = 0.f, q2 = 0.f, k1 = 0.f, k2 = 0.f;
-    if (tid < HALF) {
-        q1 = bf2f(row[(size_t)h * D + tid]);
-        q2 = bf2f(row[(size_t)h * D + tid + HALF]);
-        k1 = bf2f(row[(size_t)(n_h + kvh) * D + tid]);
-        k2 = bf2f(row[(size_t)(n_h + kvh) * D + tid + HALF]);
-        sv[tid] = bf2f(row[(size_t)(n_h + n_kv + kvh) * D + tid]);
-        sv[tid + HALF] = bf2f(row[(size_t)(n_h + n_kv + kvh) * D + tid + HALF]);
-    }
-    if (q_norm_w) {
-        float a = warp_sum(q1 * q1 + q2 * q2), c = warp_sum(k1 * k1 + k2 * k2);
-        __shared__ float nr[2][FD_THREADS / 32];
-        if (lane == 0) { nr[0][warp] = a; nr[1][warp] = c; }
-        __syncthreads();
-        a = c = 0.f;
-#pragma unroll
-        for (int w = 0; w < FD_THREADS / 32; ++w) { a += nr[0][w]; c += nr[1][w]; }
-        const float rq = 1.0f / sqrtf(a / (float)D + eps), rk = 1.0f / sqrtf(c / (float)D + eps);
-        if (tid < HALF) {
-            q1 = rbf(bf2f(q_norm_w[tid]) * rbf(q1 * rq));
-            q2 = rbf(bf2f(q_norm_w[tid + HALF]) * rbf(q2 * rq));
-            k1 = rbf(bf2f(k_norm_w[tid]) * rbf(k1 * rk));
-            k2 = rbf(bf2f(k_norm_w[tid + HALF]) * rbf(k2 * rk));
-        }
-    }
-    if (tid < HALF) {
-        const float c = bf2f(cos_tab[(size_t)pos * HALF + tid]), s = bf2f(sin_tab[(size_t)pos * HALF + tid]);
-        sq[tid] = rbf(rbf(q1 * c) + rbf(-q2 * s));
-        sq[tid + HALF] = rbf(rbf(q2 * c) + rbf(q1 * s));
-        sk[tid] = rbf(rbf(k1 * c) + rbf(-k2 * s));
-        sk[tid + HALF] = rbf(rbf(k2 * c) + rbf(k1 * s));
-    }
-    __syncthreads();
-    if (h % n_rep == 0 && tid < D) {
-        const size_t off = (((size_t)b * n_kv + kvh) * T_max + pos) * D + tid;
-        k_cache[off] = f2bf(sk[tid]);
-        v_cache[off] = f2bf(sv[tid]);
-    }
-    const bf16* kb = k_cache + ((size_t)b * n_kv + kvh) * T_max * D;
-    const bf16* vb = v_cache + ((size_t)b * n_kv + kvh) * T_max * D;
-    float mx = -INFINITY;
-    for (int key = tid; key < pos; key += FD_THREADS) {
-        if constexpr (ROWS) if (key < k_start) continue;
-        const uint4* kr = reinterpret_cast<const uint4*>(kb + (size_t)key * D);
-        float acc = 0.f;
-#pragma unroll 4
-        for (int c = 0; c < D / 8; ++c) {
-            const uint4 kv4 = kr[c];
-            const uint32_t* k32 = reinterpret_cast<const uint32_t*>(&kv4);
-            const float4 qa = *reinterpret_cast<const float4*>(&sq[c * 8]);
-            const float4 qb = *reinterpret_cast<const float4*>(&sq[c * 8 + 4]);
-            acc += bf16_lo(k32[0]) * qa.x + bf16_hi(k32[0]) * qa.y + bf16_lo(k32[1]) * qa.z + bf16_hi(k32[1]) * qa.w +
-                   bf16_lo(k32[2]) * qb.x + bf16_hi(k32[2]) * qb.y + bf16_lo(k32[3]) * qb.z + bf16_hi(k32[3]) * qb.w;
-        }
-        acc *= scale_log2;
-        sscore[key] = acc;
-        mx = fmaxf(mx, acc);
-    }
-    if (warp == 0) {
-        float acc = 0.f;
-        for (int i = lane; i < D; i += 32) acc += sq[i] * sk[i];
-        acc = warp_sum(acc) * scale_log2;
-        if (lane == 0) sscore[pos] = acc;
-        mx = fmaxf(mx, acc);
-    }
-    mx = warp_max(mx);
-    if (lane == 0) sred[warp] = mx;
-    __syncthreads();
-    if (tid == 0) {
-        float m = sred[0];
-#pragma unroll
-        for (int w = 1; w < FD_THREADS / 32; ++w) m = fmaxf(m, sred[w]);
-        s_bc[0] = m;
-    }
-    __syncthreads();
-    const float m_all = s_bc[0];
-    float lsum = 0.f;
-    for (int key = tid; key <= pos; key += FD_THREADS) {
-        if constexpr (ROWS) if (key < k_start) continue;
-        const float p = exp2f(sscore[key] - m_all);
-        lsum += p;
-        sscore[key] = rbf(p);
-    }
-    lsum = warp_sum(lsum);
-    __syncthreads();
-    if (lane == 0) sred[warp] = lsum;
-    __syncthreads();
-    constexpr int TPR = D / 8, KG = FD_THREADS / TPR;
-    const int dd0 = (tid % TPR) * 8, kgi = tid / TPR;
-    float acc[8];
-#pragma unroll
-    for (int j = 0; j < 8; ++j) acc[j] = 0.f;
-    for (int key = kgi; key < pos; key += KG) {
-        if constexpr (ROWS) if (key < k_start) continue;
-        const uint4 vv = *reinterpret_cast<const uint4*>(vb + (size_t)key * D + dd0);
-        const uint32_t* v32 = reinterpret_cast<const uint32_t*>(&vv);
-        const float p = sscore[key];
-#pragma unroll
-        for (int j = 0; j < 4; ++j) {
-            acc[2 * j] = fmaf(p, bf16_lo(v32[j]), acc[2 * j]);
-            acc[2 * j + 1] = fmaf(p, bf16_hi(v32[j]), acc[2 * j + 1]);
-        }
-    }
-    if (kgi == 0) {
-        const float p = sscore[pos];
-#pragma unroll
-        for (int j = 0; j < 8; ++j) acc[j] = fmaf(p, sv[dd0 + j], acc[j]);
-    }
-#pragma unroll
-    for (int j = 0; j < 8; ++j) {
-        float v = acc[j];
-#pragma unroll
-        for (int off = TPR; off < 32; off <<= 1) v += __shfl_xor_sync(0xffffffffu, v, off);
-        acc[j] = v;
-    }
-    if (lane < TPR) {
-#pragma unroll
-        for (int j = 0; j < 8; ++j) so[warp][dd0 + j] = acc[j];
-    }
-    __syncthreads();
-    if (tid < D) {
-        float l = 0.f, o = 0.f;
-#pragma unroll
-        for (int w = 0; w < FD_THREADS / 32; ++w) { l += sred[w]; o += so[w][tid]; }
-        out[((size_t)b * n_h + h) * D + tid] = f2bf(o / l);
-    }
+    __shared__ FdSmem<D> s;
+    attn_decode_fused_slice<D, ROWS, 0>(s, blockIdx.x, blockIdx.y, threadIdx.x, qkv, k_cache, v_cache, out, *pos_dev, cos_tab,
+                                        sin_tab, q_norm_w, k_norm_w, eps, n_h, n_kv, T_max, scale_log2, kv_start);
 }
 
 }
diff --git a/tensorlink_b200/csrc/attn_decode_fused.cuh b/tensorlink_b200/csrc/attn_decode_fused.cuh
--- /dev/null
+++ b/tensorlink_b200/csrc/attn_decode_fused.cuh
@@ -0,0 +1,173 @@
+#pragma once
+
+#include "common.cuh"
+
+namespace tl {
+
+constexpr int FD_THREADS = 128, FD_MAX_T = 2048;
+
+template <int D>
+struct FdSmem {
+    __align__(16) float sq[D];
+    float sk[D], sv[D];
+    float sscore[FD_MAX_T + 1];
+    float sred[FD_THREADS / 32];
+    float s_bc[2];
+    float nr[2][FD_THREADS / 32];
+    __align__(16) float so[FD_THREADS / 32][D];
+};
+
+__device__ __forceinline__ float fd_ldcg(const bf16* p) {
+    unsigned short v;
+    asm volatile("ld.global.cg.u16 %0, [%1];" : "=h"(v) : "l"(p));
+    return __uint_as_float(((uint32_t)v) << 16);
+}
+
+template <int BAR>
+__device__ __forceinline__ void fd_bar() { asm volatile("bar.sync %0, %1;" ::"n"(BAR), "n"(FD_THREADS) : "memory"); }
+
+template <int D, bool ROWS, int BAR>
+__device__ __forceinline__ void attn_decode_fused_slice(
+    FdSmem<D>& s, int h, int b, int tid, const bf16* qkv, bf16* k_cache, bf16* v_cache, bf16* out, int pos,
+    const bf16* cos_tab, const bf16* sin_tab, const bf16* q_norm_w, const bf16* k_norm_w, float eps, int n_h, int n_kv,
+    int T_max, float scale_log2, const int32_t* kv_start) {
+    constexpr int HALF = D / 2;
+    const int lane = tid & 31, warp = tid >> 5;
+    const int n_rep = n_h / n_kv, kvh = h / n_rep;
+    int k_start = 0;
+    if constexpr (ROWS) {
+        k_start = kv_start[b];
+        cos_tab -= (size_t)k_start * HALF;
+        sin_tab -= (size_t)k_start * HALF;
+    }
+    const int heads = n_h + 2 * n_kv;
+
+    const bf16* row = qkv + (size_t)b * heads * D;
+    float q1 = 0.f, q2 = 0.f, k1 = 0.f, k2 = 0.f;
+    if (tid < HALF) {
+        q1 = fd_ldcg(row + (size_t)h * D + tid);
+        q2 = fd_ldcg(row + (size_t)h * D + tid + HALF);
+        k1 = fd_ldcg(row + (size_t)(n_h + kvh) * D + tid);
+        k2 = fd_ldcg(row + (size_t)(n_h + kvh) * D + tid + HALF);
+        s.sv[tid] = fd_ldcg(row + (size_t)(n_h + n_kv + kvh) * D + tid);
+        s.sv[tid + HALF] = fd_ldcg(row + (size_t)(n_h + n_kv + kvh) * D + tid + HALF);
+    }
+    if (q_norm_w) {
+        float a = warp_sum(q1 * q1 + q2 * q2), c = warp_sum(k1 * k1 + k2 * k2);
+        if (lane == 0) { s.nr[0][warp] = a; s.nr[1][warp] = c; }
+        fd_bar<BAR>();
+        a = c = 0.f;
+#pragma unroll
+        for (int w = 0; w < FD_THREADS / 32; ++w) { a += s.nr[0][w]; c += s.nr[1][w]; }
+        const float rq = 1.0f / sqrtf(a / (float)D + eps), rk = 1.0f / sqrtf(c / (float)D + eps);
+        if (tid < HALF) {
+            q1 = rbf(bf2f(q_norm_w[tid]) * rbf(q1 * rq));
+            q2 = rbf(bf2f(q_norm_w[tid + HALF]) * rbf(q2 * rq));
+            k1 = rbf(bf2f(k_norm_w[tid]) * rbf(k1 * rk));
+            k2 = rbf(bf2f(k_norm_w[tid + HALF]) * rbf(k2 * rk));
+        }
+    }
+    if (tid < HALF) {
+        const float c = bf2f(cos_tab[(size_t)pos * HALF + tid]), sn = bf2f(sin_tab[(size_t)pos * HALF + tid]);
+        s.sq[tid] = rbf(rbf(q1 * c) + rbf(-q2 * sn));
+        s.sq[tid + HALF] = rbf(rbf(q2 * c) + rbf(q1 * sn));
+        s.sk[tid] = rbf(rbf(k1 * c) + rbf(-k2 * sn));
+        s.sk[tid + HALF] = rbf(rbf(k2 * c) + rbf(k1 * sn));
+    }
+    fd_bar<BAR>();
+    if (h % n_rep == 0 && tid < D) {
+        const size_t off = (((size_t)b * n_kv + kvh) * T_max + pos) * D + tid;
+        k_cache[off] = f2bf(s.sk[tid]);
+        v_cache[off] = f2bf(s.sv[tid]);
+    }
+    const bf16* kb = k_cache + ((size_t)b * n_kv + kvh) * T_max * D;
+    const bf16* vb = v_cache + ((size_t)b * n_kv + kvh) * T_max * D;
+    float mx = -INFINITY;
+    for (int key = tid; key < pos; key += FD_THREADS) {
+        if constexpr (ROWS) if (key < k_start) continue;
+        const uint4* kr = reinterpret_cast<const uint4*>(kb + (size_t)key * D);
+        float acc = 0.f;
+#pragma unroll 4
+        for (int c = 0; c < D / 8; ++c) {
+            const uint4 kv4 = kr[c];
+            const uint32_t* k32 = reinterpret_cast<const uint32_t*>(&kv4);
+            const float4 qa = *reinterpret_cast<const float4*>(&s.sq[c * 8]);
+            const float4 qb = *reinterpret_cast<const float4*>(&s.sq[c * 8 + 4]);
+            acc += bf16_lo(k32[0]) * qa.x + bf16_hi(k32[0]) * qa.y + bf16_lo(k32[1]) * qa.z + bf16_hi(k32[1]) * qa.w +
+                   bf16_lo(k32[2]) * qb.x + bf16_hi(k32[2]) * qb.y + bf16_lo(k32[3]) * qb.z + bf16_hi(k32[3]) * qb.w;
+        }
+        acc *= scale_log2;
+        s.sscore[key] = acc;
+        mx = fmaxf(mx, acc);
+    }
+    if (warp == 0) {
+        float acc = 0.f;
+        for (int i = lane; i < D; i += 32) acc += s.sq[i] * s.sk[i];
+        acc = warp_sum(acc) * scale_log2;
+        if (lane == 0) s.sscore[pos] = acc;
+        mx = fmaxf(mx, acc);
+    }
+    mx = warp_max(mx);
+    if (lane == 0) s.sred[warp] = mx;
+    fd_bar<BAR>();
+    if (tid == 0) {
+        float m = s.sred[0];
+#pragma unroll
+        for (int w = 1; w < FD_THREADS / 32; ++w) m = fmaxf(m, s.sred[w]);
+        s.s_bc[0] = m;
+    }
+    fd_bar<BAR>();
+    const float m_all = s.s_bc[0];
+    float lsum = 0.f;
+    for (int key = tid; key <= pos; key += FD_THREADS) {
+        if constexpr (ROWS) if (key < k_start) continue;
+        const float p = exp2f(s.sscore[key] - m_all);
+        lsum += p;
+        s.sscore[key] = rbf(p);
+    }
+    lsum = warp_sum(lsum);
+    fd_bar<BAR>();
+    if (lane == 0) s.sred[warp] = lsum;
+    fd_bar<BAR>();
+    constexpr int TPR = D / 8, KG = FD_THREADS / TPR;
+    const int dd0 = (tid % TPR) * 8, kgi = tid / TPR;
+    float acc[8];
+#pragma unroll
+    for (int j = 0; j < 8; ++j) acc[j] = 0.f;
+    for (int key = kgi; key < pos; key += KG) {
+        if constexpr (ROWS) if (key < k_start) continue;
+        const uint4 vv = *reinterpret_cast<const uint4*>(vb + (size_t)key * D + dd0);
+        const uint32_t* v32 = reinterpret_cast<const uint32_t*>(&vv);
+        const float p = s.sscore[key];
+#pragma unroll
+        for (int j = 0; j < 4; ++j) {
+            acc[2 * j] = fmaf(p, bf16_lo(v32[j]), acc[2 * j]);
+            acc[2 * j + 1] = fmaf(p, bf16_hi(v32[j]), acc[2 * j + 1]);
+        }
+    }
+    if (kgi == 0) {
+        const float p = s.sscore[pos];
+#pragma unroll
+        for (int j = 0; j < 8; ++j) acc[j] = fmaf(p, s.sv[dd0 + j], acc[j]);
+    }
+#pragma unroll
+    for (int j = 0; j < 8; ++j) {
+        float v = acc[j];
+#pragma unroll
+        for (int off = TPR; off < 32; off <<= 1) v += __shfl_xor_sync(0xffffffffu, v, off);
+        acc[j] = v;
+    }
+    if (lane < TPR) {
+#pragma unroll
+        for (int j = 0; j < 8; ++j) s.so[warp][dd0 + j] = acc[j];
+    }
+    fd_bar<BAR>();
+    if (tid < D) {
+        float l = 0.f, o = 0.f;
+#pragma unroll
+        for (int w = 0; w < FD_THREADS / 32; ++w) { l += s.sred[w]; o += s.so[w][tid]; }
+        out[((size_t)b * n_h + h) * D + tid] = f2bf(o / l);
+    }
+}
+
+}
diff --git a/tensorlink_b200/csrc/decode_chain.cu b/tensorlink_b200/csrc/decode_chain.cu
--- a/tensorlink_b200/csrc/decode_chain.cu
+++ b/tensorlink_b200/csrc/decode_chain.cu
@@ -1,5 +1,6 @@
 #include <stdlib.h>
 
+#include "attn_decode_fused.cuh"
 #include "common.cuh"
 
 namespace tl {
@@ -13,9 +14,13 @@
 constexpr int DC_TILE = 32;
 constexpr int DC_MIN_KEYS = 128;
 constexpr int DC_KT_MAX = 128 * 2 + 16;
-constexpr int DC_ATTN_BYTES = 8 * 128 * 4 + 2 * 128 * 4 + 8 * DC_TILE * 4 + 2 * DC_TILE * DC_KT_MAX;
+constexpr int DC_SPLIT_BYTES = 8 * 128 * 4 + 2 * 128 * 4 + 8 * DC_TILE * 4 + 2 * DC_TILE * DC_KT_MAX;
+constexpr int DC_ATTN_BYTES = DC_SPLIT_BYTES > (int)sizeof(FdSmem<128>) ? DC_SPLIT_BYTES : (int)sizeof(FdSmem<128>);
 constexpr int DC_GB = 8;
 constexpr int DC_JOBCTR = 64;
+constexpr int DC_CHAIN_JOBS = TL_DECODE_CHAIN_JOBS;
+static_assert(DC_JOBCTR + DC_CHAIN_JOBS <= TL_DECODE_CHAIN_SYNC_BYTES / 4, "sync slot too small");
+constexpr int DC_JOB_WORDS = (int)(sizeof(tl_decode_job) / 4);
 constexpr int DC_STAT_OFF = 2 * (DC_MAX_JOBS + 1) * 4 + DC_MAX_JOBS * 160;
 constexpr unsigned long long DC_TIMEOUT_NS = 2000000000ull;
 
@@ -28,7 +33,7 @@
     const unsigned char* pf_ptr;
     unsigned long long pf_bytes;
     unsigned long long* trace;
-    tl_decode_job jobs[DC_MAX_JOBS];
+    const tl_decode_job* jobs;
 };
 
 __device__ __forceinline__ void dc_bar(int id, int n) { asm volatile("bar.sync %0, %1;" ::"r"(id), "r"(n) : "memory"); }
@@ -242,19 +247,30 @@
     int gseq = 0;
     const int tr_sel = blockIdx.x == 0 ? 0 : (blockIdx.x == gridDim.x - 1 ? 1 : -1);
     auto stamp = [&](int j, int k) {
-        if (!p.trace || tid != 0) return;
+        if (!p.trace || tid != 0 || j >= DC_MAX_JOBS) return;
         const unsigned long long now = dc_timer();
-        if (tr_sel >= 0) p.trace[((size_t)tr_sel * (DC_MAX_JOBS + 1) + j) * 4 + k] = now;
-        if (k == 2 && j < DC_MAX_JOBS) p.trace[2 * (DC_MAX_JOBS + 1) * 4 + (size_t)j * 160 + blockIdx.x] = now;
+        const int r = j < 0 ? DC_MAX_JOBS : j;
+        if (tr_sel >= 0) p.trace[((size_t)tr_sel * (DC_MAX_JOBS + 1) + r) * 4 + k] = now;
+        if (k == 2 && j >= 0) p.trace[2 * (DC_MAX_JOBS + 1) * 4 + (size_t)j * 160 + blockIdx.x] = now;
     };
-    stamp(DC_MAX_JOBS, 0);
+    stamp(-1, 0);
+
+    __shared__ tl_decode_job s_job[2];
+    const uint32_t* const job_words = reinterpret_cast<const uint32_t*>(p.jobs);
+    if (tid < DC_JOB_WORDS) reinterpret_cast<uint32_t*>(&s_job[0])[tid] = job_words[tid];
+    dc_bar(1, DC_CT);
 
     asm volatile("griddepcontrol.wait;" ::: "memory");
-    stamp(DC_MAX_JOBS, 1);
+    stamp(-1, 1);
 
     for (int j = 0; j < p.n_jobs; ++j) {
-        const tl_decode_job& jb = p.jobs[j];
+        const tl_decode_job& jb = s_job[j & 1];
         const bool last_job = j == p.n_jobs - 1;
+        uint32_t next_word = 0;
+        if (tid < DC_JOB_WORDS && !last_job) next_word = job_words[(size_t)(j + 1) * DC_JOB_WORDS + tid];
+        auto stash_next = [&]() {
+            if (tid < DC_JOB_WORDS && !last_job) reinterpret_cast<uint32_t*>(&s_job[(j + 1) & 1])[tid] = next_word;
+        };
         stamp(j, 0);
         if (jb.type == TL_JOB_GEMV) {
             const int N = jb.N, K = jb.K, flags = jb.flags;
@@ -474,11 +490,45 @@
                     }
                 }
             }
-            if (p.trace && blockIdx.x == 0 && tid == 0) {
+            if (p.trace && blockIdx.x == 0 && tid == 0 && j < DC_MAX_JOBS) {
                 p.trace[DC_STAT_OFF + (size_t)j * 4 + 0] = (unsigned long long)cwait;
                 p.trace[DC_STAT_OFF + (size_t)j * 4 + 1] = (unsigned long long)(clock64() - cjob0);
             }
             stamp(j, 2);
+            stash_next();
+            if (!last_job && !grid_dep(true, gridDim.x)) break;
+            stamp(j, 3);
+        } else if (jb.type == TL_JOB_ATTN && jb.T_max <= FD_MAX_T) {
+            if (tid < FD_THREADS) {
+                const int n_h = jb.n_h, slices = n_h * M;
+                const float sl2 = jb.scale * 1.4426950408889634f;
+                const int32_t* pos_dev = reinterpret_cast<const int32_t*>(jb.pos_dev);
+                const int32_t* ks = reinterpret_cast<const int32_t*>(jb.kv_start);
+                const bf16* qkv = reinterpret_cast<const bf16*>(jb.x);
+                bf16* kc = reinterpret_cast<bf16*>(jb.k_cache);
+                bf16* vc = reinterpret_cast<bf16*>(jb.v_cache);
+                bf16* out = reinterpret_cast<bf16*>(jb.y);
+                const bf16* ct = reinterpret_cast<const bf16*>(jb.cos_tab);
+                const bf16* st = reinterpret_cast<const bf16*>(jb.sin_tab);
+                const bf16* qn = reinterpret_cast<const bf16*>(jb.q_norm_w);
+                const bf16* kn = reinterpret_cast<const bf16*>(jb.k_norm_w);
+                for (int sl = blockIdx.x; sl < slices; sl += gridDim.x) {
+                    const int h = sl % n_h, b = sl / n_h;
+                    const int pos = pos_dev[(jb.flags & TL_ATTN_POS_PER_ROW) ? b : 0];
+#define TL_DC_SLICE(D_, ROWS_)                                                                                             \
+    attn_decode_fused_slice<D_, ROWS_, 2>(*reinterpret_cast<FdSmem<D_>*>(attn_s), h, b, tid, qkv, kc, vc, out, pos, ct, st, qn, \
+                                          kn, jb.eps, n_h, jb.n_kv, jb.T_max, sl2, ks)
+                    if (jb.d == 64) {
+                        if (ks) TL_DC_SLICE(64, true); else TL_DC_SLICE(64, false);
+                    } else {
+                        if (ks) TL_DC_SLICE(128, true); else TL_DC_SLICE(128, false);
+                    }
+#undef TL_DC_SLICE
+                    fd_bar<2>();
+                }
+            }
+            stamp(j, 2);
+            stash_next();
             if (!last_job && !grid_dep(true, gridDim.x)) break;
             stamp(j, 3);
         } else if (jb.type == TL_JOB_ATTN) {
@@ -723,12 +773,13 @@
                 }
             }
             stamp(j, 2);
+            stash_next();
             if (!last_job && !grid_dep(s_last != 0, (unsigned)G)) break;
             stamp(j, 3);
         }
     }
     dc_bar(1, DC_CT);
-    stamp(DC_MAX_JOBS, 2);
+    stamp(-1, 2);
     if (tid == 0) {
         __threadfence();
         const unsigned prev = atomicAdd(&p.sync[1], 1u);
@@ -762,12 +813,12 @@
     return (size_t)M * n_h * cpg * (d + 4) * sizeof(float) + 256;
 }
 
-int tl_decode_chain(const tl_decode_job* jobs, int n_jobs, int M, void* sync_slot, void* attn_ws, size_t attn_ws_bytes,
-                    const void* pf_ptr, size_t pf_bytes, void* stream) {
+int tl_decode_chain(const tl_decode_job* jobs, const tl_decode_job* jobs_dev, int n_jobs, int M, void* sync_slot, void* attn_ws,
+                    size_t attn_ws_bytes, const void* pf_ptr, size_t pf_bytes, void* stream) {
     using namespace tl;
     TL_REQUIRE(M >= 1 && M <= DC_MAX_M, TL_ERR_INVALID, "tl_decode_chain: M=%d outside 1..%d", M, DC_MAX_M);
-    TL_REQUIRE(jobs && n_jobs > 0 && n_jobs <= DC_MAX_JOBS && sync_slot, TL_ERR_INVALID, "tl_decode_chain: bad job list (n=%d, max %d)",
-               n_jobs, DC_MAX_JOBS);
+    TL_REQUIRE(jobs && jobs_dev && n_jobs > 0 && n_jobs <= DC_CHAIN_JOBS && sync_slot && (((uintptr_t)jobs_dev) & 7) == 0,
+               TL_ERR_INVALID, "tl_decode_chain: bad job list (n=%d, max %d)", n_jobs, DC_CHAIN_JOBS);
     const int grid = sm_count();
     int k_max = 0, n_attn = 0;
     for (int j = 0; j < n_jobs; ++j) {
@@ -776,9 +827,14 @@
             TL_REQUIRE(jb.K % 8 == 0 && jb.N % 2 == 0 && jb.N > 0 && (((uintptr_t)jb.W) & 15) == 0, TL_ERR_INVALID,
                        "tl_decode_chain: job %d bad GEMV shape / alignment", j);
             if (jb.K > k_max) k_max = jb.K;
+        } else if (jb.type == TL_JOB_ATTN && jb.T_max <= FD_MAX_T) {
+            TL_REQUIRE((jb.d == 64 || jb.d == 128) && jb.n_kv > 0 && jb.n_h % jb.n_kv == 0 && jb.pos_dev, TL_ERR_INVALID,
+                       "tl_decode_chain: job %d attention shape unsupported (d=%d n_h=%d n_kv=%d)", j, jb.d, jb.n_h, jb.n_kv);
         } else if (jb.type == TL_JOB_ATTN) {
-            TL_REQUIRE((jb.d == 64 || jb.d == 128) && jb.n_kv > 0 && jb.n_h % jb.n_kv == 0 && jb.n_h / jb.n_kv <= 8, TL_ERR_INVALID,
-                       "tl_decode_chain: job %d attention shape unsupported (d=%d n_h=%d n_kv=%d)", j, jb.d, jb.n_h, jb.n_kv);
+            TL_REQUIRE((jb.d == 64 || jb.d == 128) && jb.n_kv > 0 && jb.n_h % jb.n_kv == 0 && jb.n_h / jb.n_kv <= 8 && jb.pos_dev,
+                       TL_ERR_INVALID, "tl_decode_chain: job %d attention shape unsupported (d=%d n_h=%d n_kv=%d)", j, jb.d,
+                       jb.n_h, jb.n_kv);
+            TL_REQUIRE(!jb.kv_start, TL_ERR_INVALID, "tl_decode_chain: job %d: per-row key starts need T_max <= %d", j, FD_MAX_T);
             const int G = jb.n_kv * M;
             TL_REQUIRE(G <= grid && G <= 60, TL_ERR_INVALID, "tl_decode_chain: %d (row, kv head) groups do not fit", G);
             const int cpg = grid / G;
@@ -840,7 +896,7 @@
     prm.pf_bytes = (((uintptr_t)pf_ptr) & 15) ? 0ull : (unsigned long long)(pf_bytes & ~(size_t)15);
     prm.trace = (g_chain_trace && g_chain_trace_next < g_chain_trace_slots)
                     ? g_chain_trace + (size_t)(g_chain_trace_next++) * DC_TRACE_WORDS : nullptr;
-    for (int j = 0; j < n_jobs; ++j) prm.jobs[j] = jobs[j];
+    prm.jobs = jobs_dev;
     const size_t smem = (size_t)n_stages * DC_STAGE + fixed;
     cudaLaunchConfig_t cfg = {};
     cfg.gridDim = dim3(grid);
diff --git a/tensorlink_b200/ml/shard.py b/tensorlink_b200/ml/shard.py
--- a/tensorlink_b200/ml/shard.py
+++ b/tensorlink_b200/ml/shard.py
@@ -319,8 +319,8 @@
         w = self._dbufs(B)
         if advance:
             nat.advance_pos(self.kvlen_dev, None, 1)
-        if self.chain_ok(B) or self.dq_ok(B):
-            (self._decode_step_chained if self.chain_ok(B) else self._decode_step_dq)(x, B, out)
+        if self.chain_ok(B):
+            self._decode_step_chained(x, B, out)
             if advance:
                 nat.advance_pos(self.pos_dev, None, 1)
             return
@@ -336,17 +336,20 @@
     def chain_ok(self, B: int) -> bool:
         import os
         cfg = self.cfg
-        return (os.environ.get("TL_DECODE_IMPL", "kernels") == "chain" and self.allow_chain and self.num_layers > 0
-                and not self.ragged
-                and B <= min(4, gemv_max_rows()) and cfg.n_kv_heads * B <= 60 and cfg.n_heads // cfg.n_kv_heads <= 8
-                and cfg.head_dim in (64, 128))
+        if os.environ.get("TL_DECODE_IMPL", "kernels") != "chain" or not self.allow_chain or self.num_layers == 0:
+            return False
+        if not (B <= min(4, gemv_max_rows()) and cfg.n_heads // cfg.n_kv_heads <= 8 and cfg.head_dim in (64, 128)):
+            return False
+        return self.T_max <= self.FUSED_DECODE_MAX_T or (not self.ragged and cfg.n_kv_heads * B <= 60)
 
     def _chain_group(self) -> int:
         import os
-        return max(1, min(3, int(os.environ.get("TL_CHAIN_LAYERS", "1"))))
+        per = int(os.environ.get("TL_CHAIN_LAYERS", "0")) or self.num_layers
+        return max(1, min(per, self.num_layers, (nat.CHAIN_JOBS - 1) // 5))
 
     def _decode_chains(self, x: torch.Tensor, B: int, out: Optional[torch.Tensor]):
-        key = (B, x.data_ptr(), 0 if out is None else out.data_ptr())
+        ks = self._kv_start()
+        key = (B, ks is not None, x.data_ptr(), 0 if out is None else out.data_ptr())
         if key in self._chains:
             return self._chains[key]
         cfg, v = self.cfg, self.p.v
@@ -356,17 +359,23 @@
             self.chain_sync = torch.zeros(self.num_layers + 1, nat.CHAIN_SYNC_BYTES // 4, dtype=torch.int32, device=self.device)
             self.chain_attn_ws = torch.empty(nat.decode_chain_ws(min(self.B_max, 4), cfg.n_heads, cfg.n_kv_heads, cfg.head_dim),
                                              dtype=torch.uint8, device=self.device)
+
+        def qkv_job(li):
+            bq = v.get(f"l{li}.bqkv")
+            return J(nat.JOB_GEMV, N=cfg.qkv_dim, K=cfg.hidden, flags=nat.EPI_BIAS if bq is not None else 0,
+                     W=v[f"l{li}.wqkv"], x=x, y=w.qkv, bias=bq, norm_w=v[f"l{li}.ln1"], eps=cfg.rms_eps)
+
         per = self._chain_group()
         launches = []
         for g0 in range(0, self.num_layers, per):
-            jobs = []
+            jobs = [qkv_job(self.layer_ids[0])] if g0 == 0 else []
             g1 = min(self.num_layers, g0 + per)
             for j in range(g0, g1):
                 li = self.layer_ids[j]
                 jobs.append(J(nat.JOB_ATTN, x=w.qkv, y=w.attn, k_cache=self.kc[j], v_cache=self.vc[j], pos_dev=self.pos_dev,
                               cos_tab=self.cos, sin_tab=self.sin, q_norm_w=v.get(f"l{li}.qn"), k_norm_w=v.get(f"l{li}.kn"),
                               n_h=cfg.n_heads, n_kv=cfg.n_kv_heads, d=cfg.head_dim, T_max=self.T_max, scale=self.scale,
-                              eps=cfg.rms_eps))
+                              eps=cfg.rms_eps, kv_start=ks))
                 jobs.append(J(nat.JOB_GEMV, N=cfg.hidden, K=cfg.q_dim, flags=nat.EPI_RESIDUAL, W=v[f"l{li}.wo"], x=w.attn, y=x,
                               residual=x))
                 jobs.append(J(nat.JOB_GEMV, N=2 * cfg.intermediate, K=cfg.hidden, flags=nat.EPI_SWIGLU, W=v[f"l{li}.wgu"], x=x,
@@ -375,62 +384,19 @@
                 jobs.append(J(nat.JOB_GEMV, N=cfg.hidden, K=cfg.intermediate, flags=nat.EPI_RESIDUAL, W=v[f"l{li}.wd"], x=w.act,
                               y=(out if (last and out is not None) else x), residual=x))
                 if not last:
-                    ln = self.layer_ids[j + 1]
-                    bq = v.get(f"l{ln}.bqkv")
-                    jobs.append(J(nat.JOB_GEMV, N=cfg.qkv_dim, K=cfg.hidden, flags=nat.EPI_BIAS if bq is not None else 0,
-                                  W=v[f"l{ln}.wqkv"], x=x, y=w.qkv, bias=bq, norm_w=v[f"l{ln}.ln1"], eps=cfg.rms_eps))
+                    jobs.append(qkv_job(self.layer_ids[j + 1]))
             nxt = v[f"l{self.layer_ids[g1]}.wo"] if g1 < self.num_layers else self.weights_after_last_layer
             launches.append(nat.DecodeChain(jobs, B, self.chain_sync[g0 // per], self.chain_attn_ws, nxt))
         self._chains[key] = launches
         return launches
 
     def _decode_step_chained(self, x: torch.Tensor, B: int, out: Optional[torch.Tensor]):
-        cfg, v = self.cfg, self.p.v
-        w = self._dbufs(B)
-        l0 = self.layer_ids[0]
-        nat.gemv(x, v[f"l{l0}.wqkv"], out=w.qkv, bias=v.get(f"l{l0}.bqkv"), norm_w=v[f"l{l0}.ln1"], eps=cfg.rms_eps,
-                 next_w=v[f"l{l0}.wo"])
         for ch in self._decode_chains(x, B, out):
             ch.launch()
 
-    def dq_ok(self, B: int) -> bool:
-        import os
-        return os.environ.get("TL_DECODE_IMPL", "kernels") == "dq" and self.allow_chain and self.num_layers > 1 and B <= min(4, gemv_max_rows())
-
-    def _decode_step_dq(self, x: torch.Tensor, B: int, out: Optional[torch.Tensor]):
-        cfg, v = self.cfg, self.p.v
-        w = self._dbufs(B)
-        key = ("dq", B, x.data_ptr(), 0 if out is None else out.data_ptr())
-        if key not in self._chains:
-            J = nat.make_job
-            if self.chain_sync is None:
-                self.chain_sync = torch.zeros(self.num_layers + 1, nat.CHAIN_SYNC_BYTES // 4, dtype=torch.int32, device=self.device)
-                self.chain_attn_ws = torch.empty(nat.decode_chain_ws(min(self.B_max, 4), cfg.n_heads, cfg.n_kv_heads, cfg.head_dim),
-                                                 dtype=torch.uint8, device=self.device)
-            launches = []
-            for j in range(self.num_layers - 1):
-                li, ln = self.layer_ids[j], self.layer_ids[j + 1]
-                bq = v.get(f"l{ln}.bqkv")
-                jobs = [J(nat.JOB_GEMV, N=cfg.hidden, K=cfg.intermediate, flags=nat.EPI_RESIDUAL, W=v[f"l{li}.wd"], x=w.act, y=x, residual=x),
-                        J(nat.JOB_GEMV, N=cfg.qkv_dim, K=cfg.hidden, flags=nat.EPI_BIAS if bq is not None else 0, W=v[f"l{ln}.wqkv"], x=x,
-                          y=w.qkv, bias=bq, norm_w=v[f"l{ln}.ln1"], eps=cfg.rms_eps)]
-                launches.append(nat.DecodeChain(jobs, B, self.chain_sync[j], self.chain_attn_ws, v[f"l{ln}.wo"]))
-            self._chains[key] = launches
-        chains = self._chains[key]
-        l0 = self.layer_ids[0]
-        nat.gemv(x, v[f"l{l0}.wqkv"], out=w.qkv, bias=v.get(f"l{l0}.bqkv"), norm_w=v[f"l{l0}.ln1"], eps=cfg.rms_eps, next_w=v[f"l{l0}.wo"])
-        for j, li in enumerate(self.layer_ids):
-            self._decode_attention(j, li, B, w)
-            nat.gemv(w.attn, v[f"l{li}.wo"], out=x, residual=x, next_w=v[f"l{li}.wgu"])
-            nat.gemv(x, v[f"l{li}.wgu"], out=w.act, norm_w=v[f"l{li}.ln2"], eps=cfg.rms_eps, flags=nat.EPI_SWIGLU, next_w=v[f"l{li}.wd"])
-            if j + 1 < self.num_layers:
-                chains[j].launch()
-            else:
-                nat.gemv(w.act, v[f"l{li}.wd"], out=x if out is None else out, residual=x, next_w=self.weights_after_last_layer)
-
     def n_chain_launches(self) -> int:
         per = self._chain_group()
-        return 1 + (self.num_layers + per - 1) // per
+        return (self.num_layers + per - 1) // per
 
     def check(self):
         if self.chain_sync is not None and int(self.chain_sync[:, 2].max().item()):
diff --git a/tensorlink_b200/ml/stage.py b/tensorlink_b200/ml/stage.py
--- a/tensorlink_b200/ml/stage.py
+++ b/tensorlink_b200/ml/stage.py
@@ -202,8 +202,6 @@
         gemv = B <= gemv_max_rows()
         if self.slots[0].chain_ok(B):
             n = self.slots[0].n_chain_launches() + 2
-        elif self.slots[0].dq_ok(B):
-            n = 1 + len(self.slots[0].layer_ids) * (3 + (1 if fused else 3)) + 2
         else:
             n = len(self.slots[0].layer_ids) * ((7 if gemv else 10) - (2 if fused else 0)) + 2 + (0 if gemv else 1)
         if ring:
diff --git a/tensorlink_b200/native.py b/tensorlink_b200/native.py
--- a/tensorlink_b200/native.py
+++ b/tensorlink_b200/native.py
@@ -53,7 +53,7 @@
                                                            c_void_p]),
     "tl_decode_chain_ws": (c_size_t, [c_int, c_int, c_int, c_int]),
     "tl_decode_chain_trace": (c_int, [c_void_p, c_int]),
-    "tl_decode_chain": (c_int, [c_void_p, c_int, c_int, c_void_p, c_void_p, c_size_t, c_void_p, c_size_t, c_void_p]),
+    "tl_decode_chain": (c_int, [c_void_p, c_void_p, c_int, c_int, c_void_p, c_void_p, c_size_t, c_void_p, c_size_t, c_void_p]),
     "tl_peer_alloc": (c_int, [c_size_t, POINTER(c_void_p), c_void_p]),
     "tl_peer_open": (c_int, [c_void_p, POINTER(c_void_p)]),
     "tl_peer_close": (c_int, [c_void_p]),
@@ -105,12 +105,13 @@
                 ("eps", c_float), ("scale", c_float),
                 ("W", c_void_p), ("x", c_void_p), ("y", c_void_p), ("bias", c_void_p), ("residual", c_void_p),
                 ("norm_w", c_void_p), ("pos_dev", c_void_p), ("cos_tab", c_void_p), ("sin_tab", c_void_p),
-                ("q_norm_w", c_void_p), ("k_norm_w", c_void_p), ("k_cache", c_void_p), ("v_cache", c_void_p)]
+                ("q_norm_w", c_void_p), ("k_norm_w", c_void_p), ("k_cache", c_void_p), ("v_cache", c_void_p),
+                ("kv_start", c_void_p)]
 
 
 JOB_GEMV, JOB_ATTN = 0, 1
 ATTN_POS_PER_ROW = 1
-CHAIN_MAX_JOBS, CHAIN_SYNC_BYTES = 16, 1024
+CHAIN_MAX_JOBS, CHAIN_JOBS, CHAIN_SYNC_BYTES = 16, 192, 1024
 
 _lib: Optional[ctypes.CDLL] = None
 
@@ -249,7 +250,7 @@
 def prefetch_bytes() -> int:
     global _PREFETCH_BYTES
     if _PREFETCH_BYTES is None:
-        _PREFETCH_BYTES = int(float(os.environ.get("TL_PREFETCH_MB", "8")) * (1 << 20))
+        _PREFETCH_BYTES = int(float(os.environ.get("TL_PREFETCH_MB", "0")) * (1 << 20))
     return _PREFETCH_BYTES
 
 
@@ -621,9 +622,10 @@
 class DecodeChain:
 
     def __init__(self, jobs, M: int, sync_slot: torch.Tensor, attn_ws: torch.Tensor, next_w: Optional[torch.Tensor] = None):
-        assert 1 <= len(jobs) <= CHAIN_MAX_JOBS
+        assert 1 <= len(jobs) <= CHAIN_JOBS
         self.n, self.M = len(jobs), M
         self.host = (DecodeJob * self.n)(*jobs)
+        self.dev = torch.frombuffer(bytearray(bytes(self.host)), dtype=torch.uint8).to(sync_slot.device)
         self.sync_slot, self.attn_ws, self.next_w = sync_slot, attn_ws, next_w
         assert sync_slot.numel() * sync_slot.element_size() >= CHAIN_SYNC_BYTES
 
@@ -632,7 +634,7 @@
         nb = 0
         if self.next_w is not None and prefetch_bytes() > 0:
             nb = min(self.next_w.numel() * self.next_w.element_size(), prefetch_bytes())
-        _check(load().tl_decode_chain(ctypes.cast(self.host, c_void_p), self.n, self.M, _p(self.sync_slot), _p(self.attn_ws),
+        _check(load().tl_decode_chain(ctypes.cast(self.host, c_void_p), _p(self.dev), self.n, self.M, _p(self.sync_slot), _p(self.attn_ws),
                                       self.attn_ws.numel() * self.attn_ws.element_size(), _p(self.next_w) if nb else None, nb,
                                       _stream()), "tl_decode_chain")
 
```

Result: no change. 191.7, median of 6 (+0.7%).
